# inferenceengine/shadernn

Measured on NVIDIA B200. Metric: frames/sec, higher is better.
Workload: dtype f32 (split-fp16 hi+lo storage for activations and weights, 3 fp16 MMAs per product, fp32 accumulate)

## Files before the change

### include/snnb.h

```cpp
#ifndef SNNB_H_
#define SNNB_H_

#include <stddef.h>
#include <stdint.h>

#ifdef __cplusplus
extern "C" {
#endif

#define SNNB_VERSION 100

typedef struct snnb_context snnb_context;
typedef struct snnb_tensor snnb_tensor;
typedef struct snnb_weights snnb_weights;
typedef struct snnb_model snnb_model;
typedef struct snnb_timer snnb_timer;

enum { SNNB_ACT_NONE = 0, SNNB_ACT_RELU = 1, SNNB_ACT_RELU6 = 2, SNNB_ACT_TANH = 3, SNNB_ACT_SIGMOID = 4, SNNB_ACT_LEAKY_RELU = 5, SNNB_ACT_SILU = 6, SNNB_ACT_SOFTMAX = 7 };
enum { SNNB_PAD_NONE = 0, SNNB_PAD_CONSTANT = 1, SNNB_PAD_REPLICATE = 2, SNNB_PAD_REFLECT = 3 };
enum { SNNB_ALGO_AUTO = 0, SNNB_ALGO_SIMT = 1, SNNB_ALGO_TCGEN05 = 2, SNNB_ALGO_TCGEN05_STREAMK = 3 };
enum { SNNB_PRECISION_FP32X3 = 0, SNNB_PRECISION_FP16W = 1, SNNB_PRECISION_FP16 = 2 };

int snnb_context_create(int device, snnb_context** out);
int snnb_context_destroy(snnb_context* ctx);
// ... 49 lines not shown
int snnb_subpixel_launch(snnb_context* ctx, int r, const snnb_tensor* in, snnb_tensor* out);

int snnb_timer_create(snnb_context* ctx, snnb_timer** out);
int snnb_timer_start(snnb_timer* t);
int snnb_timer_stop(snnb_timer* t);
int snnb_timer_elapsed_ms(snnb_timer* t, float* ms);
int snnb_timer_destroy(snnb_timer* t);

typedef struct snnb_graph snnb_graph;
int snnb_graph_capture_begin(snnb_context* ctx);
int snnb_graph_capture_end(snnb_context* ctx, snnb_graph** out);
int snnb_graph_launch(snnb_graph* g);
int snnb_graph_destroy(snnb_graph* g);

typedef struct {
    int batch;
    int input_width;
    int input_height;
    int conv_algo;
    int use_cuda_graph;
    int fuse;
    int precision;
} snnb_model_options;

int snnb_model_load_json(snnb_context* ctx, const char* json_path, const snnb_model_options* opt, snnb_model** out);
int snnb_model_destroy(snnb_model* m);
int snnb_model_num_layers(const snnb_model* m);
int snnb_model_layer_info(const snnb_model* m, int i, char* name, int name_cap, char* type, int type_cap, int* n, int* h, int* w, int* c);
int snnb_model_num_inputs(const snnb_model* m);
int snnb_model_num_outputs(const snnb_model* m);
int snnb_model_input_dims(const snnb_model* m, int idx, int* n, int* h, int* w, int* c);
int snnb_model_output_dims(const snnb_model* m, int idx, int* n, int* h, int* w, int* c);
int snnb_model_run(snnb_model* m, const float* host_input_nhwc, float* host_output, size_t out_capacity, int* classes_1based);
int snnb_model_submit(snnb_model* m, const float* host_input_nhwc, float* host_output, size_t out_capacity, int* classes_1based, int* ticket);
int snnb_model_submit_u8(snnb_model* m, const uint8_t* host_input_nhwc_u8, const float* mean4, const float* norm4, float* host_output, size_t out_capacity,
                         int* classes_1based, int* ticket);
typedef struct {
    const uint8_t* input_u8;
    int src_height, src_width;
    int linear_filter;
    float mean4[4], norm4[4];
    float* output_f32;
    size_t output_capacity;
    uint8_t* output_u8;
    float out_scale, out_offset;
    int* classes_1based;
} snnb_image_io;
int snnb_model_submit_image(snnb_model* m, const snnb_image_io* io, int* ticket);
int snnb_model_wait(snnb_model* m, int ticket);
int snnb_model_set_input(snnb_model* m, int idx, const float* host_input_nhwc);
int snnb_model_forward(snnb_model* m);
int snnb_model_get_output(snnb_model* m, int idx, float* host_output, size_t out_capacity);
int snnb_model_layer_output(snnb_model* m, int layer, float* host_nhwc, size_t capacity);
int snnb_model_dump_outputs(snnb_model* m, const char* dir);
int snnb_model_time_layers(snnb_model* m, float* times_ms, int capacity);
int snnb_model_layer_kernel(const snnb_model* m, int layer, char* name, int name_cap);
int snnb_model_launches_per_forward(const snnb_model* m);
int snnb_model_get_boxes(snnb_model* m, int n, float* rows6, int max_rows, int* count);
int snnb_model_weight_arena(snnb_model* m, void** device_ptr, size_t* bytes);

typedef struct snnb_comm snnb_comm;
int snnb_nccl_unique_id(unsigned char id128[128]);
int snnb_nccl_comm_create(snnb_context* ctx, int rank, int world_size, const unsigned char id128[128], snnb_comm** out);
int snnb_nccl_comm_destroy(snnb_comm* comm);
int snnb_bcast_weights(snnb_model* m, snnb_comm* comm, int root);

typedef struct snnb_layer_json snnb_layer_json;
int snnb_layer_json_number(const snnb_layer_json* layer, const char* key, double* out);
int snnb_layer_json_string(const snnb_layer_json* layer, const char* key, char* buf, int cap);
int snnb_layer_json_numbers(const snnb_layer_json* layer, const char* path, const double** data, size_t* count);
typedef struct {
    void* user;
    int (*output_dims)(void* user, int num_inputs, const int* in_hwc, int* out_hwc);
    int (*run)(void* user, snnb_context* ctx, int num_inputs, const snnb_tensor* const* inputs, snnb_tensor* output);
    void (*destroy)(void* user);
} snnb_layer_impl;
typedef int (*snnb_layer_creator)(void* registry_user, const snnb_layer_json* layer, snnb_layer_impl* out);
int snnb_register_layer(const char* type_name, snnb_layer_creator creator, void* registry_user);
int snnb_unregister_layer(const char* type_name);
int snnb_tensor_planes(const snnb_tensor* t, void** hi, void** lo, int* cp);
int snnb_debug_streamk_schedule(int tiles, int num_kb, int sms, int* rows, int capacity);
int snnb_debug_feed_plan(int k, int stride, int pad_x, int ic, int out[5]);
int snnb_debug_kblock_schedule(int ksize, int cblocks, int icp, int sc_cblocks, int tiles, int ksplit, int sms, int* rows, int capacity);

#ifdef __cplusplus
}
#endif
#endif
```

### shadernn_b200/_lib.py

```python
import ctypes as C
import os

HERE = os.path.dirname(os.path.abspath(__file__))
LIB_PATH = os.path.join(HERE, "libsnn_b200.so")

c_float_p = C.POINTER(C.c_float)
c_int_p = C.POINTER(C.c_int)
vp = C.c_void_p


class ConvDesc(C.Structure):
    _fields_ = [
        ("in_channels", C.c_int),
        ("out_channels", C.c_int),
        ("kernel", C.c_int),
        ("stride", C.c_int),
        ("pad_x", C.c_int),
        ("pad_y", C.c_int),
        ("pad_mode", C.c_int),
        ("activation", C.c_int),
        ("leaky_alpha", C.c_float),
        ("algo", C.c_int),
    ]

# ... 30 lines not shown
SIGNATURES = {
    "snnb_version": (C.c_int, []),
    "snnb_last_error": (C.c_char_p, []),
    "snnb_context_create": (C.c_int, [C.c_int, C.POINTER(vp)]),
    "snnb_context_destroy": (C.c_int, [vp]),
    "snnb_sync": (C.c_int, [vp]),
    "snnb_context_stream": (vp, [vp]),
    "snnb_launch_count": (C.c_uint64, [vp]),
    "snnb_context_set_precision": (C.c_int, [vp, C.c_int]),
    "snnb_tensor_alloc": (C.c_int, [vp, C.c_int, C.c_int, C.c_int, C.c_int, C.POINTER(vp)]),
    "snnb_tensor_free": (C.c_int, [vp]),
    "snnb_tensor_dims": (C.c_int, [vp, c_int_p, c_int_p, c_int_p, c_int_p]),
    "snnb_tensor_upload_nhwc": (C.c_int, [vp, vp, vp]),
    "snnb_tensor_download_nhwc": (C.c_int, [vp, vp, vp]),
    "snnb_tensor_upload_c4hw4": (C.c_int, [vp, vp, vp]),
    "snnb_tensor_download_c4hw4": (C.c_int, [vp, vp, vp]),
    "snnb_tensor_dump": (C.c_int, [vp, vp, C.c_char_p]),
    "snnb_weights_pack_conv2d": (C.c_int, [vp, C.POINTER(ConvDesc), vp, vp, vp, vp, vp, vp, C.POINTER(vp)]),
    "snnb_weights_pack_depthwise": (C.c_int, [vp, C.POINTER(ConvDesc), vp, vp, vp, vp, vp, vp, C.POINTER(vp)]),
    "snnb_weights_pack_dense": (C.c_int, [vp, C.c_int, C.c_int, vp, vp, C.POINTER(vp)]),
    "snnb_weights_pack_channels": (C.c_int, [vp, C.c_int, vp, vp, vp, vp, C.POINTER(vp)]),
    "snnb_weights_free": (C.c_int, [vp]),
    "snnb_conv2d_launch": (C.c_int, [vp, C.POINTER(ConvDesc), vp, vp, vp, vp]),
    "snnb_depthwise_launch": (C.c_int, [vp, C.POINTER(ConvDesc), vp, vp, vp]),
    "snnb_maxpool_launch": (C.c_int, [vp, C.c_int, C.c_int, vp, vp]),
    "snnb_avgpool_launch": (C.c_int, [vp, C.c_int, C.c_int, vp, vp]),
    "snnb_add_launch": (C.c_int, [vp, C.c_int, C.c_float, vp, vp, vp]),
    "snnb_batchnorm_launch": (C.c_int, [vp, vp, C.c_int, C.c_float, vp, vp]),
    "snnb_activation_launch": (C.c_int, [vp, C.c_int, C.c_float, vp, vp]),
    "snnb_dense_launch": (C.c_int, [vp, vp, C.c_int, C.c_float, vp, vp]),
    "snnb_softmax_launch": (C.c_int, [vp, vp, vp]),
    "snnb_argmax1": (C.c_int, [vp, vp, c_int_p]),
    "snnb_flatten_launch": (C.c_int, [vp, vp, vp]),
    "snnb_concat_launch": (C.c_int, [vp, vp, vp, vp]),
    "snnb_upsample_launch": (C.c_int, [vp, C.c_float, C.c_int, vp, vp]),
    "snnb_pad_launch": (C.c_int, [vp, C.c_int, C.c_int, C.c_int, vp, vp]),
    "snnb_instancenorm_launch": (C.c_int, [vp, vp, C.c_int, C.c_float, vp, vp]),
    "snnb_subpixel_launch": (C.c_int, [vp, C.c_int, vp, vp]),
    "snnb_timer_create": (C.c_int, [vp, C.POINTER(vp)]),
    "snnb_timer_start": (C.c_int, [vp]),
    "snnb_timer_stop": (C.c_int, [vp]),
    "snnb_timer_elapsed_ms": (C.c_int, [vp, c_float_p]),
    "snnb_timer_destroy": (C.c_int, [vp]),
    "snnb_model_load_json": (C.c_int, [vp, C.c_char_p, C.POINTER(ModelOptions), C.POINTER(vp)]),
    "snnb_model_destroy": (C.c_int, [vp]),
    "snnb_model_num_layers": (C.c_int, [vp]),
    "snnb_model_layer_info": (C.c_int, [vp, C.c_int, C.c_char_p, C.c_int, C.c_char_p, C.c_int, c_int_p, c_int_p, c_int_p, c_int_p]),
    "snnb_model_num_inputs": (C.c_int, [vp]),
    "snnb_model_num_outputs": (C.c_int, [vp]),
    "snnb_model_input_dims": (C.c_int, [vp, C.c_int, c_int_p, c_int_p, c_int_p, c_int_p]),
    "snnb_model_output_dims": (C.c_int, [vp, C.c_int, c_int_p, c_int_p, c_int_p, c_int_p]),
    "snnb_model_run": (C.c_int, [vp, vp, vp, C.c_size_t, vp]),
    "snnb_graph_capture_begin": (C.c_int, [vp]),
    "snnb_graph_capture_end": (C.c_int, [vp, C.POINTER(C.c_void_p)]),
    "snnb_graph_launch": (C.c_int, [vp]),
    "snnb_graph_destroy": (C.c_int, [vp]),
    "snnb_model_submit": (C.c_int, [vp, vp, vp, C.c_size_t, vp, c_int_p]),
    "snnb_model_submit_u8": (C.c_int, [vp, vp, vp, vp, vp, C.c_size_t, vp, c_int_p]),
    "snnb_model_submit_image": (C.c_int, [vp, C.POINTER(ImageIO), c_int_p]),
    "snnb_model_wait": (C.c_int, [vp, C.c_int]),
    "snnb_model_set_input": (C.c_int, [vp, C.c_int, vp]),
    "snnb_model_forward": (C.c_int, [vp]),
    "snnb_model_get_output": (C.c_int, [vp, C.c_int, vp, C.c_size_t]),
    "snnb_model_layer_output": (C.c_int, [vp, C.c_int, vp, C.c_size_t]),
    "snnb_model_dump_outputs": (C.c_int, [vp, C.c_char_p]),
    "snnb_model_time_layers": (C.c_int, [vp, c_float_p, C.c_int]),
    "snnb_model_launches_per_forward": (C.c_int, [vp]),
    "snnb_model_layer_kernel": (C.c_int, [vp, C.c_int, C.c_char_p, C.c_int]),
    "snnb_model_get_boxes": (C.c_int, [vp, C.c_int, c_float_p, C.c_int, c_int_p]),
    "snnb_model_weight_arena": (C.c_int, [vp, C.POINTER(vp), C.POINTER(C.c_size_t)]),
    "snnb_nccl_unique_id": (C.c_int, [C.c_char_p]),
    "snnb_nccl_comm_create": (C.c_int, [vp, C.c_int, C.c_int, C.c_char_p, C.POINTER(vp)]),
    "snnb_nccl_comm_destroy": (C.c_int, [vp]),
    "snnb_bcast_weights": (C.c_int, [vp, vp, C.c_int]),
    "snnb_register_layer": (C.c_int, [C.c_char_p, vp, vp]),
    "snnb_unregister_layer": (C.c_int, [C.c_char_p]),
    "snnb_layer_json_number": (C.c_int, [vp, C.c_char_p, C.POINTER(C.c_double)]),
    "snnb_layer_json_string": (C.c_int, [vp, C.c_char_p, C.c_char_p, C.c_int]),
    "snnb_layer_json_numbers": (C.c_int, [vp, C.c_char_p, C.POINTER(C.POINTER(C.c_double)), C.POINTER(C.c_size_t)]),
    "snnb_tensor_planes": (C.c_int, [vp, C.POINTER(vp), C.POINTER(vp), c_int_p]),
    "snnb_debug_streamk_schedule": (C.c_int, [C.c_int, C.c_int, C.c_int, c_int_p, C.c_int]),
    "snnb_debug_feed_plan": (C.c_int, [C.c_int, C.c_int, C.c_int, C.c_int, c_int_p]),
    "snnb_debug_kblock_schedule": (C.c_int, [C.c_int] * 7 + [c_int_p, C.c_int]),
}

_lib = None


class SnnbError(RuntimeError):
    pass


def lib():
    global _lib
    if _lib is None:
        if not os.path.exists(LIB_PATH):
            raise SnnbError(
                "%s is missing — build it with `python -m shadernn_b200._build` (or __graft_entry__.build()). "
                "shadernn_b200 has no CPU or PyTorch fallback." % LIB_PATH)
        l = C.CDLL(LIB_PATH)
        for name, (res, args) in SIGNATURES.items():
            fn = getattr(l, name)
            fn.restype = res
            fn.argtypes = args
        _lib = l
    return _lib


def check(rc, what=""):
    if rc != 0:
        msg = lib().snnb_last_error()
        raise SnnbError("%s failed (status %d): %s" % (what or "snnb call", rc, msg.decode("utf-8", "replace") if msg else "?"))
```

### shadernn_b200/csrc/capi.cpp

```cpp
#include <cstdarg>
#include <cstdlib>
#include <cstring>
#include <memory>

#include "snnb_internal.h"

namespace snnb {

static thread_local char g_err[1024] = "";
void set_error(const char* fmt, ...) {
    va_list ap;
    va_start(ap, fmt);
    vsnprintf(g_err, sizeof(g_err), fmt, ap);
    va_end(ap);
}
const char* get_error() { return g_err; }

bool pdl_enabled() {
    static const bool on = getenv("SNNB_NO_PDL") == nullptr;
    return on;
}

int ensure_stage(snnb_context* ctx, size_t bytes) {
    if (ctx->stage_dev_bytes < bytes) {
// ... 41 lines not shown
    t->feed_lo = t->lo ? t->feed_hi + plane : nullptr;
    t->feed_h = feed_h, t->feed_w = feed_w, t->feed_py = py, t->feed_px = px;
    return 0;
}

}

using namespace snnb;

#define CHECK_DIMS_EQ(a, b, what) SNNB_REQUIRE((a)->n == (b)->n && (a)->h == (b)->h && (a)->w == (b)->w && (a)->c == (b)->c, what ": tensor dims differ")

extern "C" {

int snnb_version(void) { return SNNB_VERSION; }
int snnb_context_set_precision(snnb_context* ctx, int precision) {
    SNNB_REQUIRE(ctx && (precision == SNNB_PRECISION_FP32X3 || precision == SNNB_PRECISION_FP16W), "snnb_context_set_precision: FP32X3 or FP16W (FP16 storage is a model option)");
    ctx->precision = precision;
    return 0;
}
const char* snnb_last_error(void) { return get_error(); }

int snnb_context_create(int device, snnb_context** out) {
    SNNB_REQUIRE(out, "snnb_context_create: null out");
    int count = 0;
    cudaError_t e = cudaGetDeviceCount(&count);
    if (e != cudaSuccess || count == 0) {
        set_error("snnb_context_create: no CUDA device available (%s). This library has no CPU fallback.", cudaGetErrorString(e));
        return 1;
    }
    SNNB_REQUIRE(device >= 0 && device < count, "snnb_context_create: device %d out of range (%d devices)", device, count);
    SNNB_CUDA_OK(cudaSetDevice(device));
    cudaDeviceProp prop;
    SNNB_CUDA_OK(cudaGetDeviceProperties(&prop, device));
    SNNB_REQUIRE(prop.major == 10, "snnb_context_create: device %d is sm_%d%d; this library is built for sm_100a (B200) only", device, prop.major, prop.minor);
    auto ctx      = std::make_unique<snnb_context>();
    ctx->device   = device;
    ctx->sm_count = prop.multiProcessorCount;
    SNNB_CUDA_OK(cudaStreamCreateWithFlags(&ctx->stream, cudaStreamNonBlocking));
    *out = ctx.release();
    return 0;
}

int snnb_context_destroy(snnb_context* ctx) {
    if (!ctx) return 0;
    cudaSetDevice(ctx->device);
    cudaStreamSynchronize(ctx->stream);
    if (ctx->stage_dev) cudaFree(ctx->stage_dev);
    if (ctx->stage_host) cudaFreeHost(ctx->stage_host);
    for (void* b : ctx->scratch_blocks) cudaFree(b);
    cudaStreamDestroy(ctx->stream);
    delete ctx;
    return 0;
}

int snnb_sync(snnb_context* ctx) {
    SNNB_REQUIRE(ctx, "snnb_sync: null context");
    SNNB_CUDA_OK(cudaStreamSynchronize(ctx->stream));
    return 0;
}
void* snnb_context_stream(snnb_context* ctx) { return ctx ? (void*) ctx->stream : nullptr; }
uint64_t snnb_launch_count(snnb_context* ctx) { return ctx ? ctx->launches : 0; }

int snnb_tensor_alloc(snnb_context* ctx, int n, int h, int w, int c, snnb_tensor** out) { return tensor_alloc(ctx, n, h, w, c, out); }
int snnb_tensor_free(snnb_tensor* t) {
    if (!t) return 0;
    if (t->owns && t->hi) cudaFree(t->hi);
    if (t->feed_hi) cudaFree(t->feed_hi);
    delete t;
    return 0;
}
int snnb_debug_feed_plan(int k, int stride, int pad_x, int ic, int out[5]) {
    FeedPlan fp;
    if (!out || !make_feed_plan(k, stride, pad_x, ic, fp)) return 0;
    out[0] = fp.px, out[1] = fp.d, out[2] = fp.nch, out[3] = fp.ksteps, out[4] = fp.rows_per_panel;
    return 1;
}
int snnb_debug_streamk_schedule(int tiles, int num_kb, int sms, int* rows, int capacity) {
    SNNB_REQUIRE(rows || capacity == 0, "snnb_debug_streamk_schedule: null buffer");
    return streamk_schedule(tiles, num_kb, sms, rows, capacity);
}
int snnb_debug_kblock_schedule(int ksize, int cblocks, int icp, int sc_cblocks, int tiles, int ksplit, int sms, int* rows, int capacity) {
    SNNB_REQUIRE(rows || capacity == 0, "snnb_debug_kblock_schedule: null buffer");
    return kblock_schedule(ksize, cblocks, icp, sc_cblocks, tiles, ksplit, sms, rows, capacity);
}
int snnb_tensor_planes(const snnb_tensor* t, void** hi, void** lo, int* cp) {
    SNNB_REQUIRE(t && hi && lo && cp, "snnb_tensor_planes: null argument");
    *hi = t->hi, *lo = t->lo, *cp = t->cp;
    return 0;
}
int snnb_tensor_dims(const snnb_tensor* t, int* n, int* h, int* w, int* c) {
    SNNB_REQUIRE(t, "snnb_tensor_dims: null tensor");
    if (n) *n = t->n;
    if (h) *h = t->h;
    if (w) *w = t->w;
    if (c) *c = t->c;
    return 0;
}
int snnb_tensor_upload_nhwc(snnb_context* ctx, snnb_tensor* t, const float* host) {
    SNNB_REQUIRE(ctx && t && host, "snnb_tensor_upload_nhwc: null argument");
    const size_t bytes = t->pixels() * t->c * sizeof(float);
    if (ensure_stage(ctx, bytes)) return 1;
    SNNB_CUDA_OK(cudaMemcpyAsync(ctx->stage_dev, host, bytes, cudaMemcpyHostToDevice, ctx->stream));
    if (launch_split_f32(ctx, ctx->stage_dev, t)) return 1;
    SNNB_CUDA_OK(cudaStreamSynchronize(ctx->stream));
    return 0;
}
int snnb_tensor_download_nhwc(snnb_context* ctx, const snnb_tensor* t, float* host) {
    SNNB_REQUIRE(ctx && t && host, "snnb_tensor_download_nhwc: null argument");
    const size_t bytes = t->pixels() * t->c * sizeof(float);
    if (ensure_stage(ctx, bytes)) return 1;
    if (launch_merge_f32(ctx, t, ctx->stage_dev)) return 1;
    SNNB_CUDA_OK(cudaMemcpyAsync(host, ctx->stage_dev, bytes, cudaMemcpyDeviceToHost, ctx->stream));
    SNNB_CUDA_OK(cudaStreamSynchronize(ctx->stream));
    return 0;
}

static void c4_to_nhwc(const float* c4, int N, int H, int W, int C, float* nhwc) {
    const int D = (C + 3) / 4;
    for (int n = 0; n < N; ++n)
        for (int y = 0; y < H; ++y)
            for (int x = 0; x < W; ++x)
                for (int c = 0; c < C; ++c)
                    nhwc[(((size_t) n * H + y) * W + x) * C + c] = c4[((((size_t) n * D + c / 4) * H + y) * W + x) * 4 + (c % 4)];
}
static void nhwc_to_c4(const float* nhwc, int N, int H, int W, int C, float* c4) {
    const int D = (C + 3) / 4;
    memset(c4, 0, sizeof(float) * (size_t) N * D * H * W * 4);
    for (int n = 0; n < N; ++n)
        for (int y = 0; y < H; ++y)
            for (int x = 0; x < W; ++x)
                for (int c = 0; c < C; ++c)
                    c4[((((size_t) n * D + c / 4) * H + y) * W + x) * 4 + (c % 4)] = nhwc[(((size_t) n * H + y) * W + x) * C + c];
}
int snnb_tensor_upload_c4hw4(snnb_context* ctx, snnb_tensor* t, const float* host_c4) {
    SNNB_REQUIRE(ctx && t && host_c4, "snnb_tensor_upload_c4hw4: null argument");
    std::vector<float> tmp(t->pixels() * t->c);
    c4_to_nhwc(host_c4, t->n, t->h, t->w, t->c, tmp.data());
    return snnb_tensor_upload_nhwc(ctx, t, tmp.data());
}
int snnb_tensor_download_c4hw4(snnb_context* ctx, const snnb_tensor* t, float* host_c4) {
    SNNB_REQUIRE(ctx && t && host_c4, "snnb_tensor_download_c4hw4: null argument");
    std::vector<float> tmp(t->pixels() * t->c);
    if (snnb_tensor_download_nhwc(ctx, t, tmp.data())) return 1;
    nhwc_to_c4(tmp.data(), t->n, t->h, t->w, t->c, host_c4);
    return 0;
}
int snnb_tensor_dump(snnb_context* ctx, const snnb_tensor* t, const char* path) {
    SNNB_REQUIRE(ctx && t && path, "snnb_tensor_dump: null argument");
    const int D = (t->c + 3) / 4;
    std::vector<float> c4((size_t) t->n * D * t->h * t->w * 4);
    if (snnb_tensor_download_c4hw4(ctx, t, c4.data())) return 1;
    for (int n = 0; n < t->n; ++n) {
        std::string p = path;
        if (t->n > 1) p += ".n" + std::to_string(n);
        FILE* f = fopen(p.c_str(), "wb");
        SNNB_REQUIRE(f, "snnb_tensor_dump: cannot open %s", p.c_str());
        char header[32];
        memset(header, 0, sizeof(header));
        snprintf(header, sizeof(header), "%d %d %d %d", t->w, t->h, D, t->c);
        fwrite(header, 1, sizeof(header), f);
        fwrite(c4.data() + (size_t) n * D * t->h * t->w * 4, sizeof(float), (size_t) D * t->h * t->w * 4, f);
        fclose(f);
    }
    return 0;
}

// ... 244 lines not shown
```

### shadernn_b200/csrc/engine/core.cpp

```cpp
#include <algorithm>
#include <cstring>
#include <unordered_map>
#include <unordered_set>

#include "engine.h"

using namespace snnb;

namespace snn {

using namespace dp;

MixedInferenceCore::~MixedInferenceCore() {
    if (ctx) {
        cudaSetDevice(ctx->device);
        cudaStreamSynchronize(ctx->stream);
    }
    if (cuGraphExec) cudaGraphExecDestroy(cuGraphExec);
    if (cuGraph) cudaGraphDestroy(cuGraph);
    for (auto* t : ownedTensors) snnb_tensor_free(t);
    if (arena) cudaFree(arena);
    if (scratchArena) cudaFree(scratchArena);
    if (ioStage) cudaFree(ioStage);
    if (argmaxDev) cudaFree(argmaxDev);
    if (yoloDev) cudaFree(yoloDev);
    if (yoloHost) cudaFreeHost(yoloHost);
    for (auto& sl : slots) {
        if (sl.yoloDev) cudaFree(sl.yoloDev);
        if (sl.yoloHost) cudaFreeHost(sl.yoloHost);
        if (sl.stageIn) cudaFree(sl.stageIn);
        if (sl.stageResize) cudaFree(sl.stageResize);
        if (sl.stageOut) cudaFree(sl.stageOut);
        if (sl.smallHost) cudaFreeHost(sl.smallHost);
        if (sl.argmax) cudaFree(sl.argmax);
        if (sl.h2dDone) cudaEventDestroy(sl.h2dDone);
        if (sl.stageFree) cudaEventDestroy(sl.stageFree);
        if (sl.resultReady) cudaEventDestroy(sl.resultReady);
    }
    if (copyStream) cudaStreamDestroy(copyStream);
}

std::unique_ptr<MixedInferenceCore> MixedInferenceCore::create(snnb_context* ctx, const std::string& modelFileName, const ShaderGenOptions& options,
                                                               std::string& err) {
    std::unique_ptr<MixedInferenceCore> core(new MixedInferenceCore());
    core->ctx     = ctx;
    core->options = options;
    try {
        core->layers = loadFromJsonModel(modelFileName);
        core->graph  = generateInferenceGraph(core->layers, options);
    } catch (std::exception& e) {
        err = e.what();
        return nullptr;
    }
    if (!core->init(err)) return nullptr;
    return core;
}

static bool allZeroPadding(const PaddingSpec& p) {
    uint32_t o[4];
    p.offsets(3, true, o);
    const bool keyword_same = !(p.t == "valid" || p.t == "none" || (!p.t.empty() && std::all_of(p.t.begin(), p.t.end(), ::isdigit)));
    return !keyword_same && o[0] == 0 && o[1] == 0 && o[2] == 0 && o[3] == 0;
}

bool MixedInferenceCore::init(std::string& err) {
    const int N = (int) options.batch;
    const bool twoPlanes = options.precision != SNNB_PRECISION_FP16;
    std::unordered_map<GenericModelLayer*, int> order;
    for (size_t i = 0; i < graph.sorted.size(); ++i) order[graph.sorted[i]] = (int) i;

    for (auto* L : graph.sorted) {
        if (L->isInputLayer) inputLayers.push_back(L);
        if (L->nextLayers.empty()) outputLayers.push_back(L);
        if (L->typeName == "YOLO") yolo = static_cast<YOLOLayer*>(L);
    }
    std::stable_sort(inputLayers.begin(), inputLayers.end(), [](GenericModelLayer* a, GenericModelLayer* b) {
        return static_cast<InputLayerLayer*>(a)->_desc.inputIndex < static_cast<InputLayerLayer*>(b)->_desc.inputIndex;
    });
    if (inputLayers.empty()) {
        err = "model has no InputLayer";
        return false;
    }

    std::unordered_map<GenericModelLayer*, GenericModelLayer*> alias;
    const bool shortcutFold = options.fuse && options.convAlgo != SNNB_ALGO_SIMT && getenv("SNNB_NO_SHORTCUT_FOLD") == nullptr;
    auto foldable = [&](GenericModelLayer* c2, GenericModelLayer* ds) {
        if (c2 == ds || c2->typeName != "Conv2D" || ds->typeName != "Conv2D" || c2->fusedAway || ds->fusedAway) return false;
        auto* cc = static_cast<Conv2DLayer*>(c2);
        auto* dc = static_cast<Conv2DLayer*>(ds);
        if (c2->nextLayers.size() != 1 || ds->nextLayers.size() != 1 || c2->prevLayers.size() != 1 || ds->prevLayers.size() != 1) return false;
        if (cc->_desc.activation.id != SNNB_ACT_NONE || dc->_desc.activation.id != SNNB_ACT_NONE || cc->residual || cc->fusedAct >= 0 || cc->shortcut ||
            dc->shortcut || dc->foldedInto)
            return false;
        const int dsMode = padModeId(dc->_desc.padding.mode);
        if (cc->_desc.stride != 1 || dc->_desc.kernelSize != 1 || !(dsMode == SNNB_PAD_NONE || dsMode == SNNB_PAD_CONSTANT)) return false;
        GenericModelLayer* x = ds->prevLayers[0];
        if (order[x] >= order[c2]) return false;
        const Dims &dc2 = graph.outputDims[order[c2]], &dds = graph.outputDims[order[ds]];
        if (dc2.width != dds.width || dc2.height != dds.height || dc2.depth != dds.depth || graph.outputDims[order[x]].depth != ds->numInputPlanes) return false;
        auto stand_in = [&](GenericModelLayer* X) {
            snnb_tensor t;
            const Dims& d = graph.outputDims[order[X]];
            t.n = N, t.h = (int) d.height, t.w = (int) d.width, t.c = (int) d.depth, t.cp = round_up(t.c, 8);
            t.hi = reinterpret_cast<__half*>(1), t.lo = twoPlanes ? t.hi : nullptr;
            return t;
        };
        const snnb_tensor in = stand_in(c2->prevLayers[0]), sc = stand_in(x), out = stand_in(c2);
        snnb_weights probe;
        probe.w_hi = probe.w_lo = probe.w_row_hi = probe.w_row_lo = reinterpret_cast<__half*>(1);
        uint32_t offs[4];
        cc->_desc.padding.offsets((int) cc->_desc.kernelSize, true, offs);
        ConvArgs a;
        a.in = &in, a.residual = nullptr, a.out = const_cast<snnb_tensor*>(&out), a.w = &probe;
        a.k = (int) cc->_desc.kernelSize, a.stride = 1;
        a.pad_x = a.k == 1 ? 0 : (int) offs[0], a.pad_y = a.k == 1 ? 0 : (int) offs[2], a.pad_mode = padModeId(cc->_desc.padding.mode);
        probe.row_stride = 1, probe.row_pad = a.pad_x;
        a.act = SNNB_ACT_NONE, a.alpha = 0.0f, a.precision = options.precision;
        a.shortcut = &sc, a.sc_stride = (int) dc->_desc.stride;
        return conv2d_umma_fold_supported(ctx, a);
    };
    if (options.fuse) {
        for (auto* L : graph.sorted) {
            if (L->typeName == "Pad" && L->nextLayers.size() == 1 && L->prevLayers.size() == 1) {
                auto* pad  = static_cast<PadLayer*>(L);
                auto* next = L->nextLayers[0];
                PaddingSpec* np = nullptr;
                if (next->typeName == "Conv2D" && static_cast<Conv2DLayer*>(next)->_desc.kernelSize > 1) np = &static_cast<Conv2DLayer*>(next)->_desc.padding;
                if (next->typeName == "SeparableConv2D" && pad->mode == "constant") np = &static_cast<SeparableConv2DLayer*>(next)->_desc.padding;
                if (np && allZeroPadding(*np)) {
                    uint32_t o[4];
                    pad->padding.offsets(0, false, o);
                    np->t = std::to_string(o[0]), np->b = std::to_string(o[1]), np->l = std::to_string(o[2]), np->r = std::to_string(o[3]);
                    np->mode       = pad->mode;
                    L->fusedAway   = true;
                    alias[L]       = L->prevLayers[0];
                }
            }
            if (shortcutFold && L->typeName == "Add" && L->prevLayers.size() == 2) {
                auto* add = static_cast<AddLayer*>(L);
                for (int o = 0; o < 2; ++o) {
                    GenericModelLayer* c2 = L->prevLayers[o];
                    GenericModelLayer* ds = L->prevLayers[1 - o];
                    if (!foldable(c2, ds)) continue;
                    auto* cc       = static_cast<Conv2DLayer*>(c2);
                    cc->fusedAct   = add->activation.id;
                    cc->fusedAlpha = add->activation.alpha;
                    cc->shortcut   = static_cast<Conv2DLayer*>(ds);
                    cc->shortcut->foldedInto = cc;
                    ds->fusedAway  = true;
                    L->fusedAway   = true;
                    alias[c2]      = L;
                    break;
                }
            }
            if (L->typeName == "Add" && L->prevLayers.size() == 2 && !L->fusedAway) {
                auto* add = static_cast<AddLayer*>(L);
                GenericModelLayer* a = L->prevLayers[0];
                GenericModelLayer* b = L->prevLayers[1];
                auto fusable = [&](GenericModelLayer* c, GenericModelLayer* other) {
                    if (c->typeName != "Conv2D" || c->nextLayers.size() != 1 || c->fusedAway) return false;
                    auto* conv = static_cast<Conv2DLayer*>(c);
                    if (conv->_desc.activation.id != SNNB_ACT_NONE || conv->residual || conv->fusedAct >= 0) return false;
                    return order[other] < order[c] && c != other;
                };
                GenericModelLayer* conv = nullptr;
                GenericModelLayer* other = nullptr;
                if (fusable(b, a))
                    conv = b, other = a;
                else if (fusable(a, b))
                    conv = a, other = b;
                if (conv) {
                    conv->fusedAct   = add->activation.id;
                    conv->fusedAlpha = add->activation.alpha;
                    conv->prevLayers.push_back(other);
                    L->fusedAway     = true;
                    alias[conv]      = L;
                }
            }
            if (L->typeName == "Dense" && L->prevLayers.size() == 1) {
                GenericModelLayer* f = L->prevLayers[0];
                GenericModelLayer* pool = (f->typeName == "Flatten" && f->prevLayers.size() == 1 && f->nextLayers.size() == 1 &&
                                           static_cast<FlattenLayer*>(f)->activation.id == SNNB_ACT_NONE)
                                              ? f->prevLayers[0]
                                              : f;
                auto dimsOf = [&](GenericModelLayer* x) { return graph.outputDims[order[x]]; };
                if (pool->typeName == "AveragePooling2D" && static_cast<PoolingLayer*>(pool)->isAvg && pool->nextLayers.size() == 1 && pool->prevLayers.size() == 1 &&
                    !pool->fusedAway && dimsOf(pool).width * dimsOf(pool).height == 1 && static_cast<DenseLayer*>(L)->units <= 256 &&
                    dimsOf(pool->prevLayers[0]).width * dimsOf(pool->prevLayers[0]).height >= 4 && dimsOf(pool->prevLayers[0]).depth <= 4096 &&
                    static_cast<PoolingLayer*>(pool)->_desc.kernelSize >= dimsOf(pool->prevLayers[0]).width &&
                    static_cast<PoolingLayer*>(pool)->_desc.kernelSize >= dimsOf(pool->prevLayers[0]).height) {
                    static_cast<DenseLayer*>(L)->gapSource = pool->prevLayers[0];
                    pool->fusedAway = true;
                }
            }
            if (L->typeName == "Flatten" && L->inputDims.size() == 1 && L->inputDims[0].width * L->inputDims[0].height == 1 &&
                static_cast<FlattenLayer*>(L)->activation.id == SNNB_ACT_NONE) {
                L->fusedAway = true;
                alias[L]     = L->prevLayers[0];
            }
        }
    }

    std::unordered_map<GenericModelLayer*, snnb_tensor*> outOf;
    auto resolve = [&](GenericModelLayer* L) -> GenericModelLayer* {
        std::unordered_set<GenericModelLayer*> seen;
        while (alias.count(L) && !seen.count(L)) {
            seen.insert(L);
            L = alias[L];
        }
        return L;
    };
    for (size_t i = 0; i < graph.sorted.size(); ++i) {
        GenericModelLayer* L = graph.sorted[i];
        if (L->typeName == "YOLO") continue;
        GenericModelLayer* owner = resolve(L);
        if (owner != L && !(L->typeName == "Conv2D")) continue;
        if (L->typeName == "Conv2D" && static_cast<Conv2DLayer*>(L)->foldedInto) continue;
        if (outOf.count(owner)) continue;
        const Dims& d = graph.outputDims[order[owner]];
        snnb_tensor* t = nullptr;
        if (tensor_alloc(ctx, N, (int) d.height, (int) d.width, (int) d.depth, &t, twoPlanes)) {
            err = get_error();
            return false;
        }
        ownedTensors.push_back(t);
        outOf[owner] = t;
    }
    for (auto* L : graph.sorted) {
        if (L->typeName == "YOLO") {
            for (auto* p : L->prevLayers) L->inputs.push_back(outOf.at(resolve(p)));
            continue;
        }
        GenericModelLayer* owner = resolve(L);
        L->output                = outOf.count(owner) ? outOf[owner] : nullptr;
        if (L->fusedAway) continue;
        size_t nin = L->prevLayers.size();
        if (L->typeName == "Conv2D" && static_cast<Conv2DLayer*>(L)->fusedAct >= 0 && !static_cast<Conv2DLayer*>(L)->shortcut) {
            nin -= 1;
            L->residual = outOf.at(resolve(L->prevLayers.back()));
        }
        for (size_t k = 0; k < nin; ++k) L->inputs.push_back(outOf.at(resolve(L->prevLayers[k])));
        if (L->typeName == "Conv2D") {
            auto* cl  = static_cast<Conv2DLayer*>(L);
            cl->algo = options.convAlgo;
            if (cl->shortcut) cl->shortcutIn = outOf.at(resolve(cl->shortcut->prevLayers[0]));
            int ph = 0, pw = 0;
            snnb_weights probe_w;
            probe_w.w_hi = probe_w.w_lo = reinterpret_cast<__half*>(1);
            probe_w.w_row_hi = probe_w.w_row_lo = reinterpret_cast<__half*>(1);
            probe_w.row_stride = (int) cl->_desc.stride, probe_w.row_pad = 0;
            std::swap(cl->weights, probe_w);
            const bool prepad = cl->wantsPrepad(L->inputs[0], L->output, options.convAlgo, ph, pw);
            std::swap(cl->weights, probe_w);
            if (prepad) {
                if (tensor_alloc(ctx, N, ph, pw, L->inputs[0]->c, &cl->prepadded, twoPlanes)) {
                    err = get_error();
                    return false;
                }
                ownedTensors.push_back(cl->prepadded);
            }
            {
                static const bool noFeed = getenv("SNNB_NO_FEED") != nullptr;
                GenericModelLayer* src   = resolve(L->prevLayers[0]);
                snnb_tensor* in          = L->inputs[0];
                const int mode           = padModeId(cl->_desc.padding.mode);
                uint32_t offs[4];
                cl->_desc.padding.offsets((int) cl->_desc.kernelSize, true, offs);
                const int k = (int) cl->_desc.kernelSize, padX = (int) offs[0], padY = (int) offs[2];
                FeedPlan fp;
                if (!noFeed && !prepad && src->isInputLayer && !in->feed_hi && options.convAlgo != SNNB_ALGO_SIMT && !L->residual && !cl->shortcut && L->output->c <= 64 &&
                    (mode == SNNB_PAD_NONE || mode == SNNB_PAD_CONSTANT) && make_feed_plan(k, (int) cl->_desc.stride, padX, in->c, fp)) {
                    const int tilesX = (L->output->w + 127) / 128;
                    const int needW  = 2 * (tilesX * 128 - 1) + 2 * fp.nch;
                    const int needH  = 2 * (L->output->h - 1) + k - padY + padY;
                    const int feedW  = (std::max(in->w + fp.px, needW) + 1) & ~1;
                    const int feedH  = std::max(in->h + padY, needH);
                    if (tensor_alloc_feed(in, feedH, feedW, padY, fp.px)) {
                        err = get_error();
                        return false;
                    }
                    cl->feedInput = true;
                }
            }
        }
        if (L->typeName == "Dense") {
            auto* dl = static_cast<DenseLayer*>(L);
            if (L->inputs[0]->h * L->inputs[0]->w != 1) {
                if (tensor_alloc(ctx, N, 1, 1, (int) dl->numInputPlanes, &dl->flat, twoPlanes)) {
                    err = get_error();
                    return false;
                }
                ownedTensors.push_back(dl->flat);
            }
            if ((uint32_t) (L->inputs[0]->h * L->inputs[0]->w * L->inputs[0]->c) != dl->numInputPlanes) {
                err = L->name + ": Dense expects " + std::to_string(dl->numInputPlanes) + " inputs, graph provides " +
                      std::to_string(L->inputs[0]->h * L->inputs[0]->w * L->inputs[0]->c);
                return false;
            }
        }
        if ((L->typeName == "Add" || L->typeName == "Concatenate") && L->inputs.size() != 2) {
            err = L->name + ": expects exactly two inputs";
            return false;
        }
        auto dimsStr = [](const snnb_tensor* t) { return std::to_string(t->h) + "x" + std::to_string(t->w) + "x" + std::to_string(t->c); };
        if (L->typeName == "Conv2D" || L->typeName == "SeparableConv2D" || L->typeName == "BatchNormalization" || L->typeName == "InstanceNorm") {
            if (L->inputs.empty() || !L->output) {
                err = L->name + ": layer has no input";
                return false;
            }
            if ((uint32_t) L->inputs[0]->c != L->numInputPlanes) {
                err = L->name + ": inputPlanes " + std::to_string(L->numInputPlanes) + " but the producing layer has " + std::to_string(L->inputs[0]->c) + " channels";
                return false;
            }
            const uint32_t wantOut = (L->typeName == "Conv2D") ? L->numOutputPlanes : L->numInputPlanes;
            if ((uint32_t) L->output->c != wantOut) {
                err = L->name + ": output tensor has " + std::to_string(L->output->c) + " channels, weights are packed for " + std::to_string(wantOut);
                return false;
            }
        }
        if (L->typeName == "Add") {
            for (auto* in : L->inputs)
                if (in->h != L->output->h || in->w != L->output->w || in->c != L->output->c) {
                    err = L->name + ": Add operand " + dimsStr(in) + " does not match the output " + dimsStr(L->output);
                    return false;
                }
        }
        if (L->typeName == "Conv2D" && L->residual &&
            (L->residual->h != L->output->h || L->residual->w != L->output->w || L->residual->c != L->output->c)) {
            err = L->name + ": fused Add operand " + dimsStr(L->residual) + " does not match the output " + dimsStr(L->output);
            return false;
        }
        if (L->typeName == "Concatenate") {
            if (L->inputs[0]->h != L->inputs[1]->h || L->inputs[0]->w != L->inputs[1]->w || L->inputs[0]->c + L->inputs[1]->c != L->output->c ||
                L->inputs[0]->h != L->output->h || L->inputs[0]->w != L->output->w) {
                err = L->name + ": Concatenate operands " + dimsStr(L->inputs[0]) + " and " + dimsStr(L->inputs[1]) + " do not stack into " + dimsStr(L->output);
                return false;
            }
        }
    }

    for (auto* in : inputLayers) {
        snnb_tensor* t = in->output;
        if (!t || !t->feed_hi || getenv("SNNB_NO_FEED_ONLY")) continue;
        bool only = true;
        int readers = 0;
        for (auto* L : graph.sorted) {
            if (L->fusedAway || L->isInputLayer) continue;
            const bool reads = std::find(L->inputs.begin(), L->inputs.end(), t) != L->inputs.end() || L->residual == t ||
                               (L->typeName == "Conv2D" && static_cast<Conv2DLayer*>(L)->shortcutIn == t);
            if (!reads) continue;
            ++readers;
            only = only && L->typeName == "Conv2D" && static_cast<Conv2DLayer*>(L)->feedInput && L->inputs.size() >= 1 && L->inputs[0] == t && L->residual != t &&
                   std::count(L->inputs.begin(), L->inputs.end(), t) == 1;
        }
        for (auto* o : outputLayers) only = only && o->output != t;
        t->feed_only = only && readers > 0;
    }

    std::vector<std::pair<GenericModelLayer*, PackedHost>> packed;
    size_t total = 0, scratchTotal = 0;
    for (auto* L : graph.sorted) {
        PackedHost p;
        try {
            L->packWeights(p);
// ... 239 lines not shown
            sl.stageResizeBytes = inBytes;
        }
        stage = sl.stageResize;
    }
    if (sl.everUsed) SNNB_CUDA_OK(cudaStreamWaitEvent(copyStream, sl.stageFree, 0));
    SNNB_CUDA_OK(cudaMemcpyAsync(stage, hostInput, inBytes, cudaMemcpyHostToDevice, copyStream));
    SNNB_CUDA_OK(cudaEventRecord(sl.h2dDone, copyStream));
    SNNB_CUDA_OK(cudaStreamWaitEvent(ctx->stream, sl.h2dDone, 0));
    if (resize) {
        if (launch_resize_u8(ctx, reinterpret_cast<const uint8_t*>(stage), io->src_height, io->src_width, in, mean, norm, io->linear_filter != 0)) return 1;
    } else if (u8 ? launch_split_u8(ctx, reinterpret_cast<const uint8_t*>(sl.stageIn), in, mean, norm) : launch_split_f32(ctx, sl.stageIn, in)) {
        return 1;
    }
    SNNB_CUDA_OK(cudaEventRecord(sl.stageFree, ctx->stream));
    if (forward()) return 1;
    sl.userOut = nullptr, sl.userClasses = nullptr, sl.userFloats = 0;
    static const bool noSmall = getenv("SNNB_NO_SMALL_RESULT") != nullptr;
    const bool small = !noSmall && isClassifier && !(io && io->output_u8) && (hostOutput || classes1) &&
                       outFloats * sizeof(float) + options.batch * sizeof(int) <= SMALL_RESULT_BYTES;
    if (small) {
        float* vals = static_cast<float*>(sl.smallDev);
        int* cls    = reinterpret_cast<int*>(static_cast<char*>(sl.smallDev) + outFloats * sizeof(float));
        if (launch_result_small(ctx, out, hostOutput ? vals : nullptr, classes1 ? cls : nullptr)) return 1;
        sl.userOut = hostOutput, sl.userClasses = classes1, sl.userFloats = outFloats;
        hostOutput = nullptr, classes1 = nullptr;
    }
    if (hostOutput) {
        if (launch_merge_f32(ctx, out, sl.stageOut)) return 1;
        SNNB_CUDA_OK(cudaMemcpyAsync(hostOutput, sl.stageOut, outFloats * sizeof(float), cudaMemcpyDeviceToHost, ctx->stream));
    }
    if (io && io->output_u8) {
        if (launch_merge_u8(ctx, out, reinterpret_cast<uint8_t*>(sl.stageOut), io->out_scale, io->out_offset)) return 1;
        SNNB_CUDA_OK(cudaMemcpyAsync(io->output_u8, sl.stageOut, outFloats, cudaMemcpyDeviceToHost, ctx->stream));
    }
    sl.classesHost = nullptr;
    if (classes1 && isClassifier) {
        if (launch_argmax(ctx, out, sl.argmax)) return 1;
        SNNB_CUDA_OK(cudaMemcpyAsync(classes1, sl.argmax, sizeof(int) * options.batch, cudaMemcpyDeviceToHost, ctx->stream));
        sl.classesHost = classes1;
    }
    if (yolo && decodeYolo(sl.yoloDev, sl.yoloHost, false)) return 1;
    SNNB_CUDA_OK(cudaEventRecord(sl.resultReady, ctx->stream));
    sl.busy = sl.everUsed = true;
    *ticket = nextTicket++;
    return 0;
}

int MixedInferenceCore::wait(int ticket) {
    SNNB_REQUIRE(ticket >= 0 && ticket < nextTicket && ticket >= nextTicket - 2, "wait: ticket %d is not in flight", ticket);
    Slot& sl = slots[ticket & 1];
    SNNB_REQUIRE(sl.busy, "wait: ticket %d was already waited for", ticket);
    SNNB_CUDA_OK(cudaEventSynchronize(sl.resultReady));
    if (sl.userOut) std::memcpy(sl.userOut, sl.smallHost, sl.userFloats * sizeof(float));
    if (sl.userClasses) {
        const int* cls = reinterpret_cast<const int*>(static_cast<const char*>(sl.smallHost) + sl.userFloats * sizeof(float));
        for (uint32_t i = 0; i < options.batch; ++i) sl.userClasses[i] = cls[i] + 1;
    }
    sl.userOut = nullptr, sl.userClasses = nullptr;
    if (sl.classesHost)
        for (uint32_t i = 0; i < options.batch; ++i) sl.classesHost[i] += 1;
    sl.busy = false;
    if (yolo) {
        const int rc = yolo->finishDecode(sl.yoloHost, sl.yoloDev, boxes);
        SNNB_REQUIRE(rc >= 0, "wait: corrupt detection candidate list");
        return rc;
    }
    return 0;
}

int MixedInferenceCore::layerOutput(int layerId, float* host, size_t capacityFloats) {
    SNNB_REQUIRE(layerId >= 0 && layerId < (int) layers.size() && host, "layerOutput: bad argument");
    GenericModelLayer* L = layers[layerId].get();
    SNNB_REQUIRE(!(L->typeName == "Conv2D" && static_cast<Conv2DLayer*>(L)->foldedInto),
                 "layerOutput: layer %d (%s) was fused into the K loop of the convolution it is added to; load the model with fuse=0 to observe it", layerId,
                 L->name.c_str());
    SNNB_REQUIRE(L->output, "layerOutput: layer %d (%s) has no device tensor", layerId, L->name.c_str());
    SNNB_REQUIRE(!(L->typeName == "Conv2D" && static_cast<Conv2DLayer*>(L)->fusedAct >= 0),
                 "layerOutput: layer %d (%s) was fused into its Add; load the model with fuse=0 to observe it", layerId, L->name.c_str());
    SNNB_REQUIRE(!(L->fusedAway && L->typeName == "AveragePooling2D"),
                 "layerOutput: layer %d (%s) was fused into the classifier head (pool + Dense in one launch); load the model with fuse=0 to observe it", layerId,
                 L->name.c_str());
    const size_t floats = L->output->pixels() * L->output->c;
    SNNB_REQUIRE(capacityFloats >= floats, "layerOutput: buffer too small (%zu < %zu floats)", capacityFloats, floats);
    return snnb_tensor_download_nhwc(ctx, L->output, host);
}

int MixedInferenceCore::timeLayers(std::vector<float>& ms) {
    ms.assign(layers.size(), 0.0f);
    std::vector<cudaEvent_t> ev(graph.sorted.size() + 1);
    for (auto& e : ev) SNNB_CUDA_OK(cudaEventCreate(&e));
    ExecOptions eo;
    eo.convAlgo = options.convAlgo, eo.precision = options.precision;
    SNNB_CUDA_OK(cudaEventRecord(ev[0], ctx->stream));
    layerKernels.assign(layers.size(), std::string());
    for (size_t i = 0; i < graph.sorted.size(); ++i) {
        GenericModelLayer* L = graph.sorted[i];
        if (!(L->fusedAway || L->isInputLayer || L->typeName == "YOLO")) {
            ctx->last_kernel = nullptr;
            if (int rc = L->run(ctx, eo)) return rc;
            layerKernels[L->layerId] = ctx->last_kernel ? ctx->last_kernel : (L->typeName + " kernels");
        }
        SNNB_CUDA_OK(cudaEventRecord(ev[i + 1], ctx->stream));
    }
    SNNB_CUDA_OK(cudaStreamSynchronize(ctx->stream));
    for (size_t i = 0; i < graph.sorted.size(); ++i) {
        float t = 0;
        SNNB_CUDA_OK(cudaEventElapsedTime(&t, ev[i], ev[i + 1]));
        ms[graph.sorted[i]->layerId] = t;
    }
    for (auto& e : ev) cudaEventDestroy(e);
    return 0;
}

int MixedInferenceCore::dumpOutputs(const std::string& dir) {
    for (auto& l : layers) {
        if (!l->output || l->fusedAway) continue;
        SNNB_REQUIRE(!(l->typeName == "Conv2D" && l->fusedAct >= 0), "dumpOutputs: %s was fused into its Add; load the model with fuse=0 to dump every layer", l->name.c_str());
        std::string path = dir + "/" + l->name + " pass[0].dump";
        if (snnb_tensor_dump(ctx, l->output, path.c_str())) return 1;
    }
    return 0;
}

}
```

### shadernn_b200/csrc/engine/engine.h

```cpp
#pragma once

#include <algorithm>
#include <map>
#include <memory>
#include <string>
#include <vector>

#include "../snnb_internal.h"
#include "json.h"

namespace snn {

struct SNNModelOutputBoxes {
    std::vector<std::vector<float>> rows;
};

namespace dp {

class ModelParser {
public:
    explicit ModelParser(const std::string& fileName);
    ~ModelParser();
    int getLayerCount() const;
    std::string getLayerName(int layerId) const;
    int getNumInbound(int layerId) const;
    std::vector<int> getInboundLayerId(int layerId) const;
    int getInputPlanes(int layerId) const;
    int getOutputPlanes(int layerId) const;
    bool isInputRange01() const;
    const json::Value& layer(int layerId) const;
    bool isBinWeight() const { return binFile != nullptr; }
    void readBin(float* dst, size_t count);
    const std::string& fileName() const { return _fileName; }

private:
    std::string _fileName;
    json::ValuePtr _root;
    FILE* binFile = nullptr;
};

int padModeId(const std::string& mode);
struct PaddingSpec {
    std::string t = "valid", b = "valid", l = "valid", r = "valid";
    std::string mode;
    void parse(const json::Value& layerObj, bool readMode);
    void offsets(int kernelSize, bool evenKernelTopLeftMinusOne, uint32_t (&offs)[4]) const;
    bool validLike() const { return t == "0" || t == "valid" || t == "none"; }
};

struct Dims {
    uint32_t width = 0, height = 0, depth = 0;
};

struct ActivationSpec {
    int id      = SNNB_ACT_NONE;
    float alpha = 0.0f;
    static int fromString(const std::string& s);
};

struct ExecOptions;

class GenericModelLayer {
public:
    virtual ~GenericModelLayer() {}
    std::string name;
    std::string typeName;
    int layerId = -1;
    std::vector<GenericModelLayer*> prevLayers, nextLayers;
    std::vector<Dims> inputDims;
    uint32_t numInputPlanes = 0, numOutputPlanes = 0;
    bool isInputLayer = false;

    virtual void getOutputDims(uint32_t& width, uint32_t& height, uint32_t& depth) const;
    struct Transform { float scaleW = 1, scaleH = 1, transW = 0, transH = 0; };
    virtual Transform getOutputScaleDimAdjustment() const { return Transform(); }

    virtual void packWeights(snnb::PackedHost&) {}
    snnb_weights weights;
    std::vector<snnb_tensor*> inputs;
    snnb_tensor* output = nullptr;
    virtual int run(snnb_context* ctx, const ExecOptions& opt) = 0;
    bool fusedAway          = false;
    snnb_tensor* residual   = nullptr;
    int fusedAct            = -1;
    float fusedAlpha        = 0.0f;
    float* scratch          = nullptr;
    size_t scratchBytes() const { return _scratchBytes; }

protected:
    size_t _scratchBytes = 0;
};

class PluginLayer : public GenericModelLayer {
public:
    snnb_layer_impl impl {};
    ~PluginLayer() override {
        if (impl.destroy) impl.destroy(impl.user);
    }
    void getOutputDims(uint32_t& w, uint32_t& h, uint32_t& d) const override;
    int run(snnb_context* ctx, const ExecOptions& opt) override;
};

typedef GenericModelLayer* (*LayerCreator)(ModelParser&, int);
void initLayerRegisty();
void registerLayer(const std::string& layerName, LayerCreator creator);
GenericModelLayer* createLayerInstance(std::string layerName, ModelParser& parser, int i);

struct InputLayerDesc {
    uint32_t inputWidth = 0, inputHeight = 0, inputChannels = 0, inputIndex = 0;
    void parse(ModelParser& parser, int layerId);
};
class InputLayerLayer : public GenericModelLayer {
public:
    InputLayerDesc _desc;
    void getOutputDims(uint32_t& w, uint32_t& h, uint32_t& d) const override;
    int run(snnb_context*, const ExecOptions&) override { return 0; }
};

struct GenericConvDesc {
    uint32_t kernelSize = 1, stride = 1;
    PaddingSpec padding;
    ActivationSpec activation;
    std::string activationName;
    std::vector<float> weights;
    std::vector<float> biases;
    bool useBatchNormalization = false;
    std::map<std::string, std::vector<float>> batchNormalization;
};
struct Conv2DDesc : GenericConvDesc {
    void parse(ModelParser& parser, int layerId);
};
class Conv2DLayer : public GenericModelLayer {
public:
    Conv2DDesc _desc;
    int algo = SNNB_ALGO_AUTO;
    snnb_tensor* prepadded = nullptr;
    bool feedInput = false;
    Conv2DLayer* shortcut    = nullptr;
    Conv2DLayer* foldedInto  = nullptr;
    snnb_tensor* shortcutIn  = nullptr;
    bool wantsPrepad(const snnb_tensor* in, const snnb_tensor* out, int convAlgo, int& ph, int& pw) const;
    Transform getOutputScaleDimAdjustment() const override;
    void getOutputDims(uint32_t& w, uint32_t& h, uint32_t& d) const override;
    void packWeights(snnb::PackedHost& p) override;
    int run(snnb_context* ctx, const ExecOptions& opt) override;
};
struct SeparableConv2DDesc : GenericConvDesc {
    void parse(ModelParser& parser, int layerId);
};
class SeparableConv2DLayer : public GenericModelLayer {
public:
    SeparableConv2DDesc _desc;
    void getOutputDims(uint32_t& w, uint32_t& h, uint32_t& d) const override;
    void packWeights(snnb::PackedHost& p) override;
    int run(snnb_context* ctx, const ExecOptions& opt) override;
};
struct PoolDesc {
    uint32_t kernelSize = 1, stride = 1;
    PaddingSpec padding;
    void parseMax(ModelParser& parser, int layerId);
    void parseAvg(ModelParser& parser, int layerId);
};
class PoolingLayer : public GenericModelLayer {
public:
    PoolDesc _desc;
    bool isAvg = false;
    Transform getOutputScaleDimAdjustment() const override;
    int run(snnb_context* ctx, const ExecOptions& opt) override;
};
class AdaptiveAvgPool2dLayer : public GenericModelLayer {
public:
    uint32_t poolSize = 1;
    void getOutputDims(uint32_t& w, uint32_t& h, uint32_t& d) const override;
    int run(snnb_context* ctx, const ExecOptions& opt) override;
};
class AddLayer : public GenericModelLayer {
public:
    ActivationSpec activation;
    int run(snnb_context* ctx, const ExecOptions& opt) override;
};
class BatchNormalizationLayer : public GenericModelLayer {
public:
    std::map<std::string, std::vector<float>> batchNormalization;
    ActivationSpec activation;
    void packWeights(snnb::PackedHost& p) override;
    int run(snnb_context* ctx, const ExecOptions& opt) override;
};
class InstanceNormLayer : public GenericModelLayer {
public:
    std::vector<float> gamma, beta;
    ActivationSpec activation;
    void packWeights(snnb::PackedHost& p) override;
    int run(snnb_context* ctx, const ExecOptions& opt) override;
    void setScratch() { _scratchBytes = 0; }
    void computeScratch(int n) { _scratchBytes = snnb::instnorm_scratch_floats(n, snnb::round_up((int) numOutputPlanes, 8)) * sizeof(float); }
};
class ActivationLayer : public GenericModelLayer {
public:
    ActivationSpec activation;
    int run(snnb_context* ctx, const ExecOptions& opt) override;
};
class DenseLayer : public GenericModelLayer {
public:
    std::vector<float> kernel;
    std::vector<float> biases;
    ActivationSpec activation;
    uint32_t units = 0;
    void getOutputDims(uint32_t& w, uint32_t& h, uint32_t& d) const override;
    void packWeights(snnb::PackedHost& p) override;
    int run(snnb_context* ctx, const ExecOptions& opt) override;
    snnb_tensor* flat = nullptr;
    GenericModelLayer* gapSource = nullptr;
};
class FlattenLayer : public GenericModelLayer {
public:
    ActivationSpec activation;
    void getOutputDims(uint32_t& w, uint32_t& h, uint32_t& d) const override;
    int run(snnb_context* ctx, const ExecOptions& opt) override;
};
class ConcatenateLayer : public GenericModelLayer {
public:
    void getOutputDims(uint32_t& w, uint32_t& h, uint32_t& d) const override;
    int run(snnb_context* ctx, const ExecOptions& opt) override;
};
class UpSampling2DLayer : public GenericModelLayer {
public:
    float scale = 1.0f;
    std::string interpolationType = "nearest";
    Transform getOutputScaleDimAdjustment() const override { return Transform {scale, scale, 0.0f, 0.0f}; }
    int run(snnb_context* ctx, const ExecOptions& opt) override;
};
class PadLayer : public GenericModelLayer {
public:
    PaddingSpec padding;
    std::string mode = "constant";
    Transform getOutputScaleDimAdjustment() const override;
    int run(snnb_context* ctx, const ExecOptions& opt) override;
};
class SubpixelLayer : public GenericModelLayer {
public:
    uint32_t kernelSize = 2;
    void getOutputDims(uint32_t& w, uint32_t& h, uint32_t& d) const override;
    int run(snnb_context* ctx, const ExecOptions& opt) override;
};
class YOLOLayer : public GenericModelLayer {
public:
    void getOutputDims(uint32_t& w, uint32_t& h, uint32_t& d) const override;
    int run(snnb_context*, const ExecOptions&) override { return 0; }
    int decode(snnb_context* ctx, std::vector<SNNModelOutputBoxes>& perImage);
    static constexpr int YOLO_HEAD_ROWS = 2048;
    int maxCand() const { return inputs.size() < 2 ? 0 : inputs[0]->n * (inputs[0]->h * inputs[0]->w + inputs[1]->h * inputs[1]->w) * 3; }
    size_t candidateBytes() const { return 32 + (size_t) maxCand() * 8 * sizeof(float); }
    size_t headBytes() const { return 32 + (size_t) std::min(maxCand(), YOLO_HEAD_ROWS) * 8 * sizeof(float); }
    int enqueueCandidates(snnb_context* ctx, void* devBuf);
    int finishDecode(const void* hostBuf, const void* devBuf, std::vector<SNNModelOutputBoxes>& perImage) const;
};

struct ShaderGenOptions {
    uint32_t desiredInputWidth = 0, desiredInputHeight = 0;
    uint32_t batch             = 1;
    int convAlgo               = SNNB_ALGO_AUTO;
    bool fuse                  = false;
    bool useCudaGraph          = false;
    int precision              = SNNB_PRECISION_FP32X3;
};
struct ExecOptions {
    int convAlgo  = SNNB_ALGO_AUTO;
    int precision = SNNB_PRECISION_FP32X3;
};

std::vector<std::shared_ptr<GenericModelLayer>> loadFromJsonModel(const std::string& fileName);
struct InferenceGraph {
    std::vector<GenericModelLayer*> sorted;
    std::vector<Dims> outputDims;
};
InferenceGraph generateInferenceGraph(const std::vector<std::shared_ptr<GenericModelLayer>>& layers, const ShaderGenOptions& options);

}

class MixedInferenceCore {
public:
    ~MixedInferenceCore();
    static std::unique_ptr<MixedInferenceCore> create(snnb_context* ctx, const std::string& modelFileName, const dp::ShaderGenOptions& options,
                                                      std::string& err);
    int forward();
    int setInput(int idx, const float* hostNHWC);
    int getOutput(int idx, float* host, size_t capacityFloats);
    int run(const float* hostInput, float* hostOutput, size_t capacityFloats, int* classes1);
    int submit(const float* hostInput, float* hostOutput, size_t capacityFloats, int* classes1, int* ticket);
    int submitU8(const uint8_t* hostInput, const float mean[4], const float norm[4], float* hostOutput, size_t capacityFloats, int* classes1, int* ticket);
    int submitImpl(const void* hostInput, bool u8, const float* mean, const float* norm, float* hostOutput, size_t capacityFloats, int* classes1, int* ticket,
                   const snnb_image_io* io = nullptr);
    int submitImage(const snnb_image_io& io, int* ticket);
    int wait(int ticket);
    int layerOutput(int layerId, float* host, size_t capacityFloats);
    int timeLayers(std::vector<float>& ms);
    int dumpOutputs(const std::string& dir);

    snnb_context* ctx = nullptr;
    dp::ShaderGenOptions options;
    std::vector<std::shared_ptr<dp::GenericModelLayer>> layers;
    dp::InferenceGraph graph;
    std::vector<dp::GenericModelLayer*> inputLayers, outputLayers;
    std::vector<SNNModelOutputBoxes> boxes;
    void* arena       = nullptr;
    size_t arenaBytes = 0;
    int launchesPerForward = 0;
    bool isClassifier = false;
    std::vector<std::string> layerKernels;

private:
    bool init(std::string& err);
    int enqueueForward(bool countOnly);
    std::vector<snnb_tensor*> ownedTensors;
    void* scratchArena = nullptr;
    cudaGraph_t cuGraph         = nullptr;
    cudaGraphExec_t cuGraphExec = nullptr;
    float* ioStage   = nullptr;
    size_t ioStageBytes = 0;
    int* argmaxDev   = nullptr;
    dp::YOLOLayer* yolo = nullptr;
    void* yoloDev  = nullptr;
    void* yoloHost = nullptr;
    int decodeYolo(void* dev, void* host, bool sync);
    static constexpr size_t SMALL_RESULT_BYTES = 64 * 1024;
    struct Slot {
        void* stageResize = nullptr;
        size_t stageResizeBytes = 0;
        float* stageIn = nullptr;
        float* stageOut = nullptr;
        int* argmax = nullptr;
        cudaEvent_t h2dDone = nullptr, stageFree = nullptr, resultReady = nullptr;
        int* classesHost = nullptr;
        void* smallHost = nullptr;
        void* smallDev  = nullptr;
        float* userOut = nullptr;
        int* userClasses = nullptr;
        size_t userFloats = 0;
        void* yoloDev = nullptr;
        void* yoloHost = nullptr;
        bool busy = false, everUsed = false;
    } slots[2];
    cudaStream_t copyStream = nullptr;
    int nextTicket = 0;
    int ensureStreaming();
};

}
```

### shadernn_b200/csrc/engine/layers.cpp

```cpp
#include <algorithm>
#include <cmath>

#include <cstring>
#include <thread>

#include "engine.h"

using namespace snnb;

namespace snn {
namespace dp {

void GenericModelLayer::getOutputDims(uint32_t& width, uint32_t& height, uint32_t& depth) const {
    width = height = depth = 0U;
    float accSW = 0, accSH = 0, accTW = 0, accTH = 0;
    const Transform t = getOutputScaleDimAdjustment();
    for (auto& dim : inputDims) {
        accSW  = std::max(accSW, t.scaleW * dim.width);
        accTW  = std::max(accTW, t.transW);
        accSH  = std::max(accSH, t.scaleH * dim.height);
        accTH  = std::max(accTH, t.transH);
        width  = (uint32_t) (accSW + accTW);
        height = (uint32_t) (accSH + accTH);
        depth  = std::max(depth, dim.depth);
    }
}

void InputLayerLayer::getOutputDims(uint32_t& w, uint32_t& h, uint32_t& d) const {
    w = inputDims.empty() ? _desc.inputWidth : inputDims[0].width;
    h = inputDims.empty() ? _desc.inputHeight : inputDims[0].height;
    d = _desc.inputChannels;
}

GenericModelLayer::Transform Conv2DLayer::getOutputScaleDimAdjustment() const {
    uint32_t offset[4];
    _desc.padding.offsets((int) _desc.kernelSize, true, offset);
    float scale       = 1 / static_cast<float>(_desc.stride);
    float translation = 0.0f;
    if (_desc.kernelSize % 2 != 0) {
        translation = 1 + (static_cast<float>(offset[0] + offset[1]) - static_cast<float>(_desc.kernelSize)) / static_cast<float>(_desc.stride);
    } else {
        translation = 1 + (static_cast<float>(offset[0] + offset[1] - 1) - static_cast<float>(_desc.kernelSize)) / static_cast<float>(_desc.stride);
    }
    return Transform {scale, scale, translation, translation};
}
void Conv2DLayer::getOutputDims(uint32_t& w, uint32_t& h, uint32_t& d) const {
    GenericModelLayer::getOutputDims(w, h, d);
    d = numOutputPlanes;
}
int padModeId(const std::string& m) {
    if (m == "constant") return SNNB_PAD_CONSTANT;
    if (m == "replicate") return SNNB_PAD_REPLICATE;
    if (m == "reflect") return SNNB_PAD_REFLECT;
    return SNNB_PAD_NONE;
}
static const float* bnv(const std::map<std::string, std::vector<float>>& bn, const char* key) {
    auto it = bn.find(key);
    return (it == bn.end() || it->second.empty()) ? nullptr : it->second.data();
}
void Conv2DLayer::packWeights(PackedHost& p) {
    if (foldedInto) return;
    const auto& bn = _desc.batchNormalization;
    const bool use = _desc.useBatchNormalization;
    pack_conv2d_host((int) numInputPlanes, (int) numOutputPlanes, (int) _desc.kernelSize, _desc.weights.data(), _desc.biases.empty() ? nullptr : _desc.biases.data(),
                     use ? bnv(bn, "gamma") : nullptr, use ? bnv(bn, "beta") : nullptr, use ? bnv(bn, "movingMean") : nullptr,
                     use ? bnv(bn, "movingVariance") : nullptr, p);
    {
        uint32_t offs[4];
        _desc.padding.offsets((int) _desc.kernelSize, true, offs);
        const int mode = padModeId(_desc.padding.mode);
        if (mode == SNNB_PAD_NONE || mode == SNNB_PAD_CONSTANT) {
            pack_rowwin_host(p, (int) _desc.stride, _desc.kernelSize == 1 ? 0 : (int) offs[0]);
            if (feedInput) pack_feed_host(p, (int) _desc.stride, _desc.kernelSize == 1 ? 0 : (int) offs[0]);
        } else {
            pack_rowwin_host(p, (int) _desc.stride, 0);
        }
    }
    if (shortcut) {
        const auto& sd = shortcut->_desc;
        const bool sbn = sd.useBatchNormalization;
        pack_shortcut_host((int) shortcut->numInputPlanes, sd.weights.data(), sd.biases.empty() ? nullptr : sd.biases.data(),
                           sbn ? bnv(sd.batchNormalization, "gamma") : nullptr, sbn ? bnv(sd.batchNormalization, "beta") : nullptr,
                           sbn ? bnv(sd.batchNormalization, "movingMean") : nullptr, sbn ? bnv(sd.batchNormalization, "movingVariance") : nullptr, p);
        std::vector<float>().swap(shortcut->_desc.weights);
    }
    std::vector<float>().swap(_desc.weights);
}
bool Conv2DLayer::wantsPrepad(const snnb_tensor* in, const snnb_tensor* out, int convAlgo, int& ph, int& pw) const {
    const int mode = padModeId(_desc.padding.mode);
    if (!(mode == SNNB_PAD_REPLICATE || mode == SNNB_PAD_REFLECT) || _desc.kernelSize <= 1 || convAlgo == SNNB_ALGO_SIMT) return false;
    ConvArgs probe {in, nullptr, const_cast<snnb_tensor*>(out), &weights, (int) _desc.kernelSize, (int) _desc.stride, 0, 0, SNNB_PAD_CONSTANT, 0, 0.0f};
    if (!conv2d_umma_supported(probe)) return false;
    ph = (out->h - 1) * (int) _desc.stride + (int) _desc.kernelSize;
    pw = (out->w - 1) * (int) _desc.stride + (int) _desc.kernelSize;
    return true;
}

int Conv2DLayer::run(snnb_context* ctx, const ExecOptions& opt) {
    uint32_t offs[4];
    _desc.padding.offsets((int) _desc.kernelSize, true, offs);
    if (prepadded) {
        if (launch_pad(ctx, inputs[0], prepadded, (int) offs[0], (int) offs[2], padModeId(_desc.padding.mode))) return 1;
        ConvArgs a {prepadded, residual, output, &weights, (int) _desc.kernelSize, (int) _desc.stride, 0, 0, SNNB_PAD_CONSTANT,
                    fusedAct >= 0 ? fusedAct : _desc.activation.id, fusedAct >= 0 ? fusedAlpha : _desc.activation.alpha};
        a.precision = opt.precision;
        return launch_conv2d_umma(ctx, a);
    }
    ConvArgs a;
    a.in = inputs[0], a.residual = residual, a.out = output, a.w = &weights;
    a.k = (int) _desc.kernelSize, a.stride = (int) _desc.stride;
    a.pad_x = _desc.kernelSize == 1 ? 0 : (int) offs[0];
    a.pad_y = _desc.kernelSize == 1 ? 0 : (int) offs[2];
    a.pad_mode = padModeId(_desc.padding.mode);
    a.act      = fusedAct >= 0 ? fusedAct : _desc.activation.id;
    a.alpha    = fusedAct >= 0 ? fusedAlpha : _desc.activation.alpha;
    a.precision = opt.precision;
    a.shortcut = shortcutIn, a.sc_stride = shortcut ? (int) shortcut->_desc.stride : 1;
    const int want = algo != SNNB_ALGO_AUTO ? algo : opt.convAlgo;
    if (want != SNNB_ALGO_SIMT && conv2d_umma_supported(a)) return launch_conv2d_umma(ctx, a);
    if (shortcut) {
        set_error("%s: a folded projection shortcut runs on the tensor-core kernel only; load the model with fuse=0 for another algorithm", name.c_str());
        return 2;
    }
    if (want == SNNB_ALGO_TCGEN05) {
        set_error("%s: tcgen05 path requested but unsupported for this shape", name.c_str());
        return 2;
    }
    return launch_conv2d_simt(ctx, a);
}

void SeparableConv2DLayer::getOutputDims(uint32_t& width, uint32_t& height, uint32_t& depth) const {
    uint32_t po[4];
    _desc.padding.offsets((int) _desc.kernelSize, true, po);
    width = height = depth = 0;
    for (auto& dim : inputDims) {
        width  = (dim.width - _desc.kernelSize + po[0] + po[2]) / _desc.stride + 1;
        height = (dim.height - _desc.kernelSize + po[1] + po[3]) / _desc.stride + 1;
        depth  = dim.depth;
        break;
    }
}
void SeparableConv2DLayer::packWeights(PackedHost& p) {
    const auto& bn = _desc.batchNormalization;
    const bool use = _desc.useBatchNormalization;
    pack_depthwise_host((int) numInputPlanes, (int) _desc.kernelSize, _desc.weights.data(), _desc.biases.empty() ? nullptr : _desc.biases.data(),
                        use ? bnv(bn, "gamma") : nullptr, use ? bnv(bn, "beta") : nullptr, use ? bnv(bn, "movingMean") : nullptr,
                        use ? bnv(bn, "movingVariance") : nullptr, p);
}
int SeparableConv2DLayer::run(snnb_context* ctx, const ExecOptions&) {
    uint32_t offs[4];
    _desc.padding.offsets((int) _desc.kernelSize, true, offs);
    ConvArgs a;
    a.in = inputs[0], a.residual = nullptr, a.out = output, a.w = &weights;
    a.k = (int) _desc.kernelSize, a.stride = (int) _desc.stride;
    a.pad_x = (int) offs[0], a.pad_y = (int) offs[2];
    a.pad_mode = SNNB_PAD_CONSTANT, a.act = _desc.activation.id, a.alpha = _desc.activation.alpha;
    return launch_depthwise(ctx, a);
}

GenericModelLayer::Transform PoolingLayer::getOutputScaleDimAdjustment() const {
    float scale = 1.0f / _desc.stride, translation;
    if (_desc.padding.validLike())
        translation = 1.0f - (static_cast<float>(_desc.kernelSize) / static_cast<float>(_desc.stride));
    else
        translation = 1.0f - 1.0f / static_cast<float>(_desc.stride);
    return Transform {scale, scale, translation, translation};
}
int PoolingLayer::run(snnb_context* ctx, const ExecOptions&) { return launch_pool(ctx, inputs[0], output, (int) _desc.kernelSize, (int) _desc.stride, isAvg); }

void AdaptiveAvgPool2dLayer::getOutputDims(uint32_t& w, uint32_t& h, uint32_t& d) const {
    w = h = poolSize;
    d     = inputDims.empty() ? numOutputPlanes : inputDims[0].depth;
}
int AdaptiveAvgPool2dLayer::run(snnb_context* ctx, const ExecOptions&) {
    const snnb_tensor* in = inputs[0];
    if (in->h % (int) poolSize || in->w % (int) poolSize || in->h / (int) poolSize != in->w / (int) poolSize) {
        set_error("%s: AdaptiveAvgPool2d needs H and W divisible by pool (%d x %d -> %u)", name.c_str(), in->h, in->w, poolSize);
        return 2;
    }
    const int k = in->h / (int) poolSize;
    return launch_pool(ctx, in, output, k, k, true);
}

int AddLayer::run(snnb_context* ctx, const ExecOptions&) { return launch_add(ctx, inputs[0], inputs[1], output, activation.id, activation.alpha); }
void BatchNormalizationLayer::packWeights(PackedHost& p) {
    pack_channels_host((int) numOutputPlanes, bnv(batchNormalization, "gamma"), bnv(batchNormalization, "beta"), bnv(batchNormalization, "movingMean"),
                       bnv(batchNormalization, "movingVariance"), p);
}
int BatchNormalizationLayer::run(snnb_context* ctx, const ExecOptions&) { return launch_batchnorm(ctx, inputs[0], output, &weights, activation.id, activation.alpha); }
void InstanceNormLayer::packWeights(PackedHost& p) { pack_channels_host((int) numOutputPlanes, gamma.data(), beta.data(), nullptr, nullptr, p); }
int InstanceNormLayer::run(snnb_context* ctx, const ExecOptions&) {
    return launch_instancenorm(ctx, inputs[0], output, &weights, activation.id, activation.alpha, scratch);
}
int ActivationLayer::run(snnb_context* ctx, const ExecOptions&) { return launch_activation(ctx, inputs[0], output, activation.id, activation.alpha); }

void DenseLayer::getOutputDims(uint32_t& w, uint32_t& h, uint32_t& d) const {
    w = h = 1;
    d     = units;
}
void DenseLayer::packWeights(PackedHost& p) {
    pack_conv2d_host((int) numInputPlanes, (int) units, 1, kernel.data(), biases.empty() ? nullptr : biases.data(), nullptr, nullptr, nullptr, nullptr, p);
    p.kind = 3;
    std::vector<float>().swap(kernel);
}
// ... 229 lines not shown
```

### shadernn_b200/csrc/kernels_umma.cu

```cuda
#include <cuda.h>

#include <algorithm>
#include <vector>
#include <cstdlib>

#include "snnb_internal.h"

namespace snnb {

constexpr int UM_BLOCK_M     = 128;
constexpr int UM_BLOCK_K     = 64;
constexpr int UM_MAX_N       = 128;
constexpr int UM_MAX_N2      = 256;
constexpr int UM_STAGES      = 3;
constexpr int UM_A_BYTES     = UM_BLOCK_M * 128;
constexpr int UM_B_BYTES     = UM_MAX_N * 128;
constexpr int UM_STAGE_BYTES = 2 * UM_A_BYTES + 2 * UM_B_BYTES;
constexpr int UM_EPI_WARPS   = 8;
constexpr int UM_THREADS     = 64 + 32 * UM_EPI_WARPS;
constexpr int UM_ACC_COLS    = 2 * UM_MAX_N;
constexpr int UM_TMEM_COLS   = 2 * UM_ACC_COLS;
constexpr int UM_STG_BYTES   = 2 * UM_BLOCK_M * 128;
constexpr int UM_SCHED_SLOTS = 8;
constexpr int UM_SMEM_BYTES  = UM_STAGES * UM_STAGE_BYTES + UM_STG_BYTES + 1024  + 320 ;
// ... 97 lines not shown
    asm volatile("cp.async.bulk.tensor.4d.shared::cluster.global.mbarrier::complete_tx::bytes [%0], [%1, {%3, %4, %5, %6}], [%2];" ::"r"(dst), "l"(m),
                 "r"(bar), "r"(c0), "r"(c1), "r"(c2), "r"(c3)
                 : "memory");
}
__device__ __forceinline__ void tma_load_2d(uint32_t dst, const CUtensorMap* m, uint32_t bar, int c0, int c1) {
    asm volatile("cp.async.bulk.tensor.2d.shared::cluster.global.mbarrier::complete_tx::bytes [%0], [%1, {%3, %4}], [%2];" ::"r"(dst), "l"(m), "r"(bar),
                 "r"(c0), "r"(c1)
                 : "memory");
}

__device__ __forceinline__ void tmem_alloc(uint32_t slot_smem, uint32_t cols) {
    asm volatile("tcgen05.alloc.cta_group::1.sync.aligned.shared::cta.b32 [%0], %1;" ::"r"(slot_smem), "r"(cols) : "memory");
    asm volatile("tcgen05.relinquish_alloc_permit.cta_group::1.sync.aligned;" ::: "memory");
}
__device__ __forceinline__ void tmem_dealloc(uint32_t taddr, uint32_t cols) {
    asm volatile("tcgen05.dealloc.cta_group::1.sync.aligned.b32 %0, %1;" ::"r"(taddr), "r"(cols) : "memory");
}
__device__ __forceinline__ void umma_f16(uint32_t d_tmem, uint64_t a_desc, uint64_t b_desc, uint32_t idesc, uint32_t accumulate) {
    asm volatile(
        "{\n\t.reg .pred p;\n\t"
        "setp.ne.b32 p, %4, 0;\n\t"
        "tcgen05.mma.cta_group::1.kind::f16 [%0], %1, %2, %3, p;\n\t}" ::"r"(d_tmem),
        "l"(a_desc), "l"(b_desc), "r"(idesc), "r"(accumulate)
        : "memory");
}
__device__ __forceinline__ void umma_commit(uint32_t bar) {
    asm volatile("tcgen05.commit.cta_group::1.mbarrier::arrive::one.shared::cluster.b64 [%0];" ::"r"(bar) : "memory");
}
__device__ __forceinline__ void tmem_ld16(uint32_t taddr, uint32_t (&r)[16]) {
    asm volatile("tcgen05.ld.sync.aligned.32x32b.x16.b32 {%0, %1, %2, %3, %4, %5, %6, %7, %8, %9, %10, %11, %12, %13, %14, %15}, [%16];"
                 : "=r"(r[0]), "=r"(r[1]), "=r"(r[2]), "=r"(r[3]), "=r"(r[4]), "=r"(r[5]), "=r"(r[6]), "=r"(r[7]), "=r"(r[8]), "=r"(r[9]), "=r"(r[10]),
                   "=r"(r[11]), "=r"(r[12]), "=r"(r[13]), "=r"(r[14]), "=r"(r[15])
                 : "r"(taddr)
                 : "memory");
}
__device__ __forceinline__ void tmem_ld_wait() { asm volatile("tcgen05.wait::ld.sync.aligned;" ::: "memory"); }

__device__ __forceinline__ void tma_store_4d(const CUtensorMap* m, uint32_t src, int c0, int c1, int c2, int c3) {
    asm volatile("cp.async.bulk.tensor.4d.global.shared::cta.bulk_group [%0, {%2, %3, %4, %5}], [%1];" ::"l"(m), "r"(src), "r"(c0), "r"(c1), "r"(c2), "r"(c3)
                 : "memory");
}
__device__ __forceinline__ void bulk_load_1d(uint32_t dst, const void* src, uint32_t bytes, uint32_t bar) {
    asm volatile("cp.async.bulk.shared::cluster.global.mbarrier::complete_tx::bytes [%0], [%1], %2, [%3];" ::"r"(dst), "l"(src), "r"(bytes), "r"(bar) : "memory");
}
__device__ __forceinline__ void bulk_commit() { asm volatile("cp.async.bulk.commit_group;" ::: "memory"); }
__device__ __forceinline__ void bulk_wait_read0() { asm volatile("cp.async.bulk.wait_group.read 0;" ::: "memory"); }
__device__ __forceinline__ void bulk_wait_read1() { asm volatile("cp.async.bulk.wait_group.read 1;" ::: "memory"); }
__device__ __forceinline__ void fence_async_smem() { asm volatile("fence.proxy.async.shared::cta;" ::: "memory"); }
__device__ __forceinline__ void named_bar_sync(int id, int threads) { asm volatile("bar.sync %0, %1;" ::"r"(id), "r"(threads) : "memory"); }

__device__ __forceinline__ uint64_t make_smem_desc(uint32_t saddr) {
    return (uint64_t) ((saddr >> 4) & 0x3FFFu) | (1ull << 16) | (64ull << 32) | (1ull << 46) | (2ull << 61);
}
__device__ __forceinline__ uint64_t make_smem_desc_sbo(uint32_t saddr, uint32_t sbo_bytes) {
    return (uint64_t) ((saddr >> 4) & 0x3FFFu) | (1ull << 16) | ((uint64_t) (sbo_bytes >> 4) << 32) | (1ull << 46) | (2ull << 61);
}
__device__ __forceinline__ uint32_t make_idesc(int M, int N) {
    return (1u << 4) | (0u << 7) | (0u << 10) | ((uint32_t) (N >> 3) << 17) | ((uint32_t) (M >> 4) << 24);
}

__device__ __noinline__ float umma_act(float v, int act, float alpha) {
    switch (act) {
    case SNNB_ACT_RELU: return fmaxf(v, 0.0f);
    case SNNB_ACT_RELU6: return fminf(fmaxf(v, 0.0f), 6.0f);
    case SNNB_ACT_TANH: return tanhf(v);
    case SNNB_ACT_SIGMOID: return 1.0f / (1.0f + expf(-v));
    case SNNB_ACT_LEAKY_RELU: return fmaxf(v, v * alpha);
    case SNNB_ACT_SILU: return v * 1.0f / (1.0f + expf(-v));
    default: return v;
    }
}
__device__ __forceinline__ float2 um_h2f(uint32_t u) { return __half22float2(*reinterpret_cast<const __half2*>(&u)); }
__device__ __forceinline__ uint32_t um_f2h(float a, float b) {
    uint32_t h;
    asm("cvt.rn.satfinite.f16x2.f32 %0, %1, %2;" : "=r"(h) : "f"(b), "f"(a));
    return h;
}
__device__ __forceinline__ void um_split2(float a, float b, uint32_t& h, uint32_t& l) {
    h               = um_f2h(a, b);
    const float2 hf = um_h2f(h);
    l               = um_f2h(a - hf.x, b - hf.y);
}

struct EpiArgs {
    const CUtensorMap *o_hi64, *o_lo64, *o_hiT, *o_loT;
    const CUtensorMap *r_hi64, *r_lo64, *r_hiT, *r_loT;
    const float* bias;
    int n_blk, OC, act, has_res, rows_box;
    int has_lo;
    float alpha;
    uint32_t stg;
    uint32_t res_bar;
    uint32_t tmem_empty;
    int bar_id;
    const float* part_src;
    int part_splits;
    long long* trace;
    int trace_seq;
    bool no_store = false;
    bool two_stagings = false;
};

__device__ __forceinline__ void epilogue_residual_load(const EpiArgs& e, int sl, int oc0, int c1, int c2, int c3, bool leader) {
    if (!leader) return;
    const int w          = min(64, e.n_blk - sl * 64);
    const bool sw        = w == 64;
    const uint32_t pitch = sw ? 128u : (uint32_t) w * 2u;
    if (elect_one()) {
        bulk_wait_read0();
        mbar_expect_tx(e.res_bar, (e.has_lo ? 2u : 1u) * (uint32_t) e.rows_box * pitch);
        tma_load_4d(e.stg, sw ? e.r_hi64 : e.r_hiT, e.res_bar, oc0 + sl * 64, c1, c2, c3);
        if (e.has_lo) tma_load_4d(e.stg + UM_BLOCK_M * 128, sw ? e.r_lo64 : e.r_loT, e.res_bar, oc0 + sl * 64, c1, c2, c3);
    }
    __syncwarp();
}

template <int NWARPS, int TERMS>
__device__ __forceinline__ void epilogue_tile(const EpiArgs& e, uint32_t taddr, int oc0, int c1, int c2, int c3, int row, int half, bool leader, int lane,
                                              uint32_t& res_phase) {
    constexpr int MAXC  = NWARPS == 8 ? 2 : 4;
    const bool fast_act = e.act == SNNB_ACT_NONE || e.act == SNNB_ACT_RELU || e.act == SNNB_ACT_RELU6 || e.act == SNNB_ACT_LEAKY_RELU;
    const float slope   = (e.act == SNNB_ACT_RELU || e.act == SNNB_ACT_RELU6) ? 0.0f : (e.act == SNNB_ACT_LEAKY_RELU ? e.alpha : 1.0f);
    const float hi_clip = e.act == SNNB_ACT_RELU6 ? 6.0f : __int_as_float(0x7f800000);
    const int nslabs    = (e.n_blk + 63) >> 6;
#define EPI_STAMP(k)                                                                                      \
    do {                                                                                                  \
        if (e.trace && leader && lane == 0 && blockIdx.x == 0 && tseq < 16) e.trace[4 * 256 + 64 + 8 * tseq + (k)] = clock64(); \
    } while (0)
    for (int sl = 0; sl < nslabs; ++sl) {
        const int tseq     = e.trace_seq * nslabs + sl;
        EPI_STAMP(0);
        const int w        = min(64, e.n_blk - sl * 64);
        const bool sw      = w == 64;
        const uint32_t pitch = sw ? 128u : (uint32_t) w * 2u;
        const uint32_t srow  = e.stg + (uint32_t) row * pitch;
        const uint32_t xr    = sw ? (uint32_t) (row & 7) : 0u;
        const int slab_oc    = oc0 + sl * 64;
        if (e.has_res && sl > 0) epilogue_residual_load(e, sl, oc0, c1, c2, c3, leader);
        bool res_ready = false;
#pragma unroll
        for (int k0 = 0; k0 < MAXC; k0 += 2) {
            uint32_t oh[2][8], ol[2][8];
            uint32_t r[2][16], r2[2][16];
#pragma unroll
            for (int kk = 0; kk < 2; ++kk) {
                const int ci = NWARPS == 8 ? half + 2 * (k0 + kk) : k0 + kk;
                if (ci < (w >> 4)) {
                    const int c = sl * 64 + ci * 16;
                    if (e.part_src) {
                        float4 t[4][4];
#pragma unroll
                        for (int sp = 0; sp < 4; ++sp) {
                            const float4* src = reinterpret_cast<const float4*>(e.part_src + (size_t) sp * UM_BLOCK_M * e.n_blk) + (size_t) (c >> 4) * 4 * UM_BLOCK_M + row;
#pragma unroll
                            for (int j4 = 0; j4 < 4; ++j4)
                                t[sp][j4] = sp < e.part_splits ? __ldcg(src + j4 * UM_BLOCK_M) : make_float4(0.f, 0.f, 0.f, 0.f);
                        }
                        float a16[16];
#pragma unroll
                        for (int j4 = 0; j4 < 4; ++j4) {
                            a16[4 * j4] = t[0][j4].x, a16[4 * j4 + 1] = t[0][j4].y, a16[4 * j4 + 2] = t[0][j4].z, a16[4 * j4 + 3] = t[0][j4].w;
#pragma unroll
                            for (int sp = 1; sp < 4; ++sp)
                                if (sp < e.part_splits) a16[4 * j4] += t[sp][j4].x, a16[4 * j4 + 1] += t[sp][j4].y, a16[4 * j4 + 2] += t[sp][j4].z, a16[4 * j4 + 3] += t[sp][j4].w;
                        }
#pragma unroll
                        for (int j = 0; j < 16; ++j) r[kk][j] = __float_as_uint(a16[j]), r2[kk][j] = 0u;
                    } else {
                        tmem_ld16(taddr + (uint32_t) c, r[kk]);
                        if (TERMS == 3) {
                            tmem_ld16(taddr + (uint32_t) (e.n_blk + c), r2[kk]);
                        } else {
#pragma unroll
                            for (int j = 0; j < 16; ++j) r2[kk][j] = 0u;
                        }
                    }
                }
            }
            if (!e.part_src) tmem_ld_wait();
#pragma unroll
            for (int kk = 0; kk < 2; ++kk) {
                const int k = k0 + kk, ci = NWARPS == 8 ? half + 2 * k : k;
                if (ci < (w >> 4)) {
                    const int c = sl * 64 + ci * 16;
                    float v[16];
#pragma unroll
                    for (int j4 = 0; j4 < 4; ++j4) {
                        const float4 b = __ldg(reinterpret_cast<const float4*>(e.bias + oc0 + c) + j4);
                        v[4 * j4 + 0] = (__uint_as_float(r[kk][4 * j4 + 0]) + __uint_as_float(r2[kk][4 * j4 + 0])) + b.x;
                        v[4 * j4 + 1] = (__uint_as_float(r[kk][4 * j4 + 1]) + __uint_as_float(r2[kk][4 * j4 + 1])) + b.y;
                        v[4 * j4 + 2] = (__uint_as_float(r[kk][4 * j4 + 2]) + __uint_as_float(r2[kk][4 * j4 + 2])) + b.z;
                        v[4 * j4 + 3] = (__uint_as_float(r[kk][4 * j4 + 3]) + __uint_as_float(r2[kk][4 * j4 + 3])) + b.w;
                    }
                    if (e.has_res) {
                        if (!res_ready) {
                            mbar_wait(e.res_bar, res_phase);
                            res_ready = true;
                        }
#pragma unroll
                        for (int g = 0; g < 2; ++g) {
                            const uint32_t a = srow + ((((uint32_t) (ci * 2 + g)) ^ xr) << 4);
                            uint32_t hh[4], ll[4];
                            asm volatile("ld.shared.v4.b32 {%0, %1, %2, %3}, [%4];" : "=r"(hh[0]), "=r"(hh[1]), "=r"(hh[2]), "=r"(hh[3]) : "r"(a));
                            if (e.has_lo) {
                                asm volatile("ld.shared.v4.b32 {%0, %1, %2, %3}, [%4];" : "=r"(ll[0]), "=r"(ll[1]), "=r"(ll[2]), "=r"(ll[3]) : "r"(a + UM_BLOCK_M * 128));
                            } else {
                                ll[0] = ll[1] = ll[2] = ll[3] = 0u;
                            }
#pragma unroll
                            for (int j = 0; j < 4; ++j) {
                                const float2 rh = um_h2f(hh[j]), rl = um_h2f(ll[j]);
                                v[g * 8 + 2 * j] += rh.x + rl.x;
                                v[g * 8 + 2 * j + 1] += rh.y + rl.y;
                            }
                        }
                    }
                    if (e.act == SNNB_ACT_RELU) {
#pragma unroll
                        for (int j = 0; j < 16; ++j) v[j] = fmaxf(v[j], 0.0f);
                    } else if (e.act == SNNB_ACT_NONE) {
                    } else if (e.act == SNNB_ACT_RELU6) {
#pragma unroll
                        for (int j = 0; j < 16; ++j) v[j] = fminf(fmaxf(v[j], 0.0f), 6.0f);
                    } else if (fast_act) {
#pragma unroll
                        for (int j = 0; j < 16; ++j) v[j] = fminf(fmaxf(v[j], v[j] * slope), hi_clip);
                    } else {
#pragma unroll
                        for (int j = 0; j < 16; ++j) v[j] = (oc0 + c + j < e.OC) ? umma_act(v[j], e.act, e.alpha) : 0.0f;
                    }
#pragma unroll
                    for (int j = 0; j < 8; ++j) um_split2(v[2 * j], v[2 * j + 1], oh[kk][j], ol[kk][j]);
                }
            }
            if (k0 + 2 >= MAXC) {
                EPI_STAMP(1);
                if (e.has_res && !res_ready) mbar_wait(e.res_bar, res_phase);
                if (e.has_res) res_phase ^= 1u;
                if (sl == nslabs - 1 && !e.part_src) {
                    tc_fence_before();
                    __syncwarp();
                    if (lane == 0) mbar_arrive(e.tmem_empty);
                }
            }
            if (k0 == 0) {
                if (!e.has_res) {
                    if (leader) {
                        if (elect_one()) {
                            if (e.two_stagings) bulk_wait_read1();
                            else bulk_wait_read0();
                        }
                        __syncwarp();
                    }
                    EPI_STAMP(2);
                    named_bar_sync(e.bar_id, NWARPS * 32);
                }
                EPI_STAMP(3);
            }
#pragma unroll
            for (int kk = 0; kk < 2; ++kk) {
                const int k = k0 + kk, ci = NWARPS == 8 ? half + 2 * k : k;
                if (ci < (w >> 4)) {
#pragma unroll
                    for (int g = 0; g < 2; ++g) {
                        const uint32_t a = srow + ((((uint32_t) (ci * 2 + g)) ^ xr) << 4);
                        asm volatile("st.shared.v4.b32 [%0], {%1, %2, %3, %4};" ::"r"(a), "r"(oh[kk][4 * g]), "r"(oh[kk][4 * g + 1]), "r"(oh[kk][4 * g + 2]), "r"(oh[kk][4 * g + 3])
                                     : "memory");
                        if (e.has_lo)
                            asm volatile("st.shared.v4.b32 [%0], {%1, %2, %3, %4};" ::"r"(a + UM_BLOCK_M * 128), "r"(ol[kk][4 * g]), "r"(ol[kk][4 * g + 1]), "r"(ol[kk][4 * g + 2]),
                                         "r"(ol[kk][4 * g + 3])
                                         : "memory");
                    }
                }
            }
        }
        EPI_STAMP(4);
        fence_async_smem();
        EPI_STAMP(5);
        named_bar_sync(e.bar_id, NWARPS * 32);
        EPI_STAMP(6);
        if (leader) {
            if (!e.no_store && elect_one()) {
                tma_store_4d(sw ? e.o_hi64 : e.o_hiT, e.stg, slab_oc, c1, c2, c3);
                if (e.has_lo) tma_store_4d(sw ? e.o_lo64 : e.o_loT, e.stg + UM_BLOCK_M * 128, slab_oc, c1, c2, c3);
                bulk_commit();
            }
            __syncwarp();
        }
        EPI_STAMP(7);
    }
#undef EPI_STAMP
}
template <int NWARPS, int TERMS>
__device__ __forceinline__ void epilogue_dump_partial(const EpiArgs& e, uint32_t taddr, float* dst, int row, int half, int lane) {
    for (int c = (NWARPS == 8 ? half : 0) * 16; c < e.n_blk; c += (NWARPS == 8 ? 32 : 16)) {
        uint32_t r[16], r2[16];
        tmem_ld16(taddr + (uint32_t) c, r);
        if (TERMS == 3) {
            tmem_ld16(taddr + (uint32_t) (e.n_blk + c), r2);
        } else {
#pragma unroll
            for (int j = 0; j < 16; ++j) r2[j] = 0u;
        }
        tmem_ld_wait();
        float4* d = reinterpret_cast<float4*>(dst) + (size_t) (c >> 4) * 4 * UM_BLOCK_M + row;
#pragma unroll
        for (int j4 = 0; j4 < 4; ++j4)
            d[j4 * UM_BLOCK_M] = make_float4(__uint_as_float(r[4 * j4]) + __uint_as_float(r2[4 * j4]), __uint_as_float(r[4 * j4 + 1]) + __uint_as_float(r2[4 * j4 + 1]),
                                __uint_as_float(r[4 * j4 + 2]) + __uint_as_float(r2[4 * j4 + 2]), __uint_as_float(r[4 * j4 + 3]) + __uint_as_float(r2[4 * j4 + 3]));
    }
    tc_fence_before();
    __syncwarp();
    if (lane == 0) mbar_arrive(e.tmem_empty);
// ... 465 lines not shown
                tc_fence_before();
                __syncwarp();
                if (lane == 0) mbar_arrive(e.tmem_empty);
                continue;
            }
            if (wi.pieces > 1) {
                float* tile_parts = p.partials + (size_t) wi.slot * (SK ? 4 : p.ksplit) * (UM_BLOCK_M * p.n_blk);
                epilogue_dump_partial<UM_EPI_WARPS, EPI_TERMS>(e, taddr, tile_parts + (size_t) wi.piece * (UM_BLOCK_M * p.n_blk), row, half, lane);
                __threadfence();
                named_bar_sync(1, UM_EPI_WARPS * 32);
                if (warp == 2 && lane == 0) {
                    const int old  = atomicAdd(p.counters + wi.slot, 1);
                    const int last = old == wi.pieces - 1;
                    if (last) p.counters[wi.slot] = 0;
                    asm volatile("st.shared.b32 [%0], %1;" ::"r"(last_flag), "r"(last) : "memory");
                }
                named_bar_sync(1, UM_EPI_WARPS * 32);
                int last;
                asm volatile("ld.shared.b32 %0, [%1];" : "=r"(last) : "r"(last_flag) : "memory");
                if (!last) continue;
                __threadfence();
                e.part_src = tile_parts, e.part_splits = wi.pieces;
                if (p.has_res) epilogue_residual_load(e, 0, oc_idx * p.n_blk, bx * p.tw, by * p.th, bn * p.tn, leader);
            }
            if (SPLIT_EPI)
                epilogue_tile<UM_EPI_WARPS / 2, EPI_TERMS>(e, taddr, oc_idx * p.n_blk, bx * p.tw, by * p.th, bn * p.tn, row, 0, leader, lane, res_phase);
            else
                epilogue_tile<UM_EPI_WARPS, EPI_TERMS>(e, taddr, oc_idx * p.n_blk, bx * p.tw, by * p.th, bn * p.tn, row, half, leader, lane, res_phase);
            e.part_src = nullptr;
            if (leader) UM_TRACE(4, it);
        }
        epilogue_drain(leader);
    }

    if (warp == 0) UM_TRACE(5, 2);
    tc_fence_before();
    __syncthreads();
    if (warp == 0) UM_TRACE(5, 3);
    if (p.trace && threadIdx.x == 0) {
        unsigned long long g;
        asm volatile("mov.u64 %0, %%globaltimer;" : "=l"(g));
        atomicMax(reinterpret_cast<unsigned long long*>(p.trace) + 5 * 256 + 9, g);
        if (blockIdx.x == 0) p.trace[5 * 256 + 11] = (long long) g;
    }
    if (warp == 1) {
        tc_fence_after();
        tmem_dealloc(tmem_base, UM_TMEM_COLS);
    }
}

constexpr int RW_MAX_STAGES    = 16;
constexpr int RW_EPI_WARPS     = 8;
constexpr int RW_THREADS       = 64 + 32 * RW_EPI_WARPS;
constexpr int RW_MAX_N         = 64;
constexpr int RW_BOXW          = 144;
constexpr int RW_ARR_BYTES     = RW_BOXW * 16;
constexpr int RW_SMEM_BYTES    = 227 * 1024;
constexpr int RW_BAR_BYTES     = 512;
constexpr int RW_B_MAX_BYTES   = RW_SMEM_BYTES - 1024 - RW_BAR_BYTES - UM_STG_BYTES - 4 * 4 * RW_ARR_BYTES;

struct RowWinParams {
    __half* out_hi;
    __half* out_lo;
    const float* bias;
    int N, OH, OW, OC, OCp, n_blk, ocr;
    int kh, stride, pad_y;
    int tiles_x;
    int parities, dmin[2];
    int ksteps, panels, ks_parity[8], ks_erel[8];
    int act;
    float alpha;
    long long* trace;
    int ablate;
    const __half* feed_hi;
    const __half* feed_lo;
    int feed_h, feed_w, feed_py;
    uint32_t feed_seg_bytes;
    int stages;
    uint32_t stage_bytes, lo_off, b_bytes;
    int rows_per_stage;
    uint32_t row_bytes;
    int stg_bufs;
    int feed_prows;
};

__device__ __forceinline__ uint64_t make_window_desc(uint32_t saddr) { return (uint64_t) ((saddr >> 4) & 0x3FFFu) | (1ull << 16) | (8ull << 32) | (1ull << 46); }

template <int TERMS, int FKS>
__global__ void __launch_bounds__(RW_THREADS, 1)
conv_rowwin_kernel(const __grid_constant__ CUtensorMap tmA_hi0, const __grid_constant__ CUtensorMap tmA_hi1, const __grid_constant__ CUtensorMap tmA_lo0,
                   const __grid_constant__ CUtensorMap tmA_lo1, const __grid_constant__ CUtensorMap tmB_hi, const __grid_constant__ CUtensorMap tmB_lo,
                   const __grid_constant__ CUtensorMap tmO_hi, const __grid_constant__ CUtensorMap tmO_lo, const RowWinParams p) {
    extern __shared__ uint8_t smem_raw[];
    const uint32_t smem_base = (smem_u32(smem_raw) + 1023u) & ~1023u;
    const uint32_t sB = smem_base;
    const uint32_t stg      = smem_base + p.b_bytes;
    const uint32_t sA0      = stg + (uint32_t) p.stg_bufs * UM_STG_BYTES;
    const uint32_t bar_base = sA0 + (uint32_t) p.stages * p.stage_bytes;
    const int RW_STAGES     = p.stages;
    auto full_bar       = [&](int s) { return bar_base + 8u * s; };
    auto empty_bar      = [&](int s) { return bar_base + 8u * (RW_MAX_STAGES + s); };
    auto tmem_full_bar  = [&](int a) { return bar_base + 8u * (2 * RW_MAX_STAGES + a); };
    auto tmem_empty_bar = [&](int a) { return bar_base + 8u * (2 * RW_MAX_STAGES + 2 + a); };
    const uint32_t b_bar     = bar_base + 8u * (2 * RW_MAX_STAGES + 4);
    const uint32_t tmem_slot = bar_base + 8u * (2 * RW_MAX_STAGES + 5);

    const int warp = threadIdx.x >> 5, lane = threadIdx.x & 31;
    pdl_trigger();
    if (warp == 0 && lane == 0) {
        tma_prefetch_desc(&tmA_hi0);
        tma_prefetch_desc(&tmA_lo0);
        tma_prefetch_desc(&tmB_hi);
        tma_prefetch_desc(&tmB_lo);
        for (int s = 0; s < RW_STAGES; ++s) {
            mbar_init(full_bar(s), 1);
            mbar_init(empty_bar(s), 1);
        }
        for (int a = 0; a < 2; ++a) {
            mbar_init(tmem_full_bar(a), 1);
            mbar_init(tmem_empty_bar(a), RW_EPI_WARPS);
        }
        mbar_init(b_bar, 1);
        fence_barrier_init();
    }
    if (warp == 1) tmem_alloc(tmem_slot, 4 * RW_MAX_N);
    tc_fence_before();
    __syncthreads();
    tc_fence_after();
    uint32_t tmem_base;
    asm volatile("ld.shared.b32 %0, [%1];" : "=r"(tmem_base) : "r"(tmem_slot));
    pdl_wait();
    if (warp == 0) UM_TRACE(5, 0);
    if (p.trace && threadIdx.x == 0) {
        unsigned long long g;
        asm volatile("mov.u64 %0, %%globaltimer;" : "=l"(g));
        atomicMin(reinterpret_cast<unsigned long long*>(p.trace) + 5 * 256 + 8, g);
        if (blockIdx.x == 0) p.trace[5 * 256 + 10] = (long long) g;
    }

    const int total_tiles = p.N * p.OH * p.tiles_x;

    if (warp == 0) {
        {
            if (elect_one()) {
                const int vrows = FKS > 0 ? p.feed_prows : p.kh * p.panels;
                mbar_expect_tx(b_bar, (TERMS == 3 ? 2u : 1u) * (uint32_t) vrows * (uint32_t) p.n_blk * 128u);
                for (int v = 0; v < vrows; ++v) {
                    if (TERMS == 3) {
                        tma_load_2d(sB + (2 * v) * p.n_blk * 128, &tmB_hi, b_bar, 0, v * p.ocr);
                        tma_load_2d(sB + (2 * v + 1) * p.n_blk * 128, &tmB_lo, b_bar, 0, v * p.ocr);
                    } else {
                        tma_load_2d(sB + v * p.n_blk * 128, &tmB_hi, b_bar, 0, v * p.ocr);
                    }
                }
            }
            __syncwarp();
            int stage = 0;
            uint32_t phase = 0;
            const uint32_t tx_bytes = (TERMS == 1 ? 1u : 2u) * (p.feed_seg_bytes ? p.feed_seg_bytes : (uint32_t) p.parities * RW_ARR_BYTES);
            if constexpr (FKS > 0) {
                const uint32_t seg  = p.feed_seg_bytes;
                const size_t pitch  = (size_t) p.feed_w * 4;
                const int per_image = p.OH * p.tiles_x;
                int rem = (int) blockIdx.x % per_image, n = (int) blockIdx.x / per_image;
                uint32_t sA = sA0;
                for (int tile = blockIdx.x; tile < total_tiles; tile += gridDim.x) {
                    const int oy = p.tiles_x == 1 ? rem : rem / p.tiles_x, xt = p.tiles_x == 1 ? 0 : rem % p.tiles_x;
                    const size_t off = (((size_t) n * p.feed_h + (oy * 2 - p.pad_y + p.feed_py)) * p.feed_w + 2 * xt * UM_BLOCK_M) * 4;
                    const __half* src_hi = p.feed_hi + off;
                    const __half* src_lo = p.feed_lo + off;
                    for (int ky0 = 0; ky0 < p.kh; ky0 += p.rows_per_stage) {
                        const int rows = min(p.rows_per_stage, p.kh - ky0);
                        mbar_wait(empty_bar(stage), phase ^ 1u);
                        if (elect_one()) {
                            if (p.ablate & 2) {
                                mbar_arrive(full_bar(stage));
                            } else {
                                mbar_expect_tx(full_bar(stage), tx_bytes * (uint32_t) rows);
                                const __half* sh = src_hi;
                                const __half* sl = src_lo;
                                uint32_t dst     = sA;
                                for (int r = 0; r < rows; ++r, dst += p.row_bytes, sh += pitch, sl += pitch) {
                                    bulk_load_1d(dst, sh, seg, full_bar(stage));
                                    if (TERMS >= 2) bulk_load_1d(dst + RW_ARR_BYTES, sl, seg, full_bar(stage));
                                }
                            }
                        }
                        __syncwarp();
                        src_hi += pitch * rows, src_lo += pitch * rows;
                        sA += p.stage_bytes;
                        if (++stage == RW_STAGES) stage = 0, phase ^= 1u, sA = sA0;
                    }
                    rem += (int) gridDim.x;
                    while (rem >= per_image) rem -= per_image, ++n;
                }
            } else
            for (int tile = blockIdx.x; tile < total_tiles; tile += gridDim.x) {
                const int xt = tile % p.tiles_x, oy = (tile / p.tiles_x) % p.OH, n = tile / (p.tiles_x * p.OH);
                const int ox0 = xt * UM_BLOCK_M;
                for (int ky = 0; ky < p.kh; ++ky) {
                    const int iy = oy * p.stride - p.pad_y + ky;
                    mbar_wait(empty_bar(stage), phase ^ 1u);
                    if (elect_one()) {
                        const uint32_t sA = sA0 + stage * p.stage_bytes;
                        if (p.ablate & 2) {
                            mbar_arrive(full_bar(stage));
                        } else {
                            mbar_expect_tx(full_bar(stage), tx_bytes);
                            tma_load_4d(sA, &tmA_hi0, full_bar(stage), 0, ox0 + p.dmin[0], iy, n);
                            if (TERMS >= 2) tma_load_4d(sA + p.lo_off, &tmA_lo0, full_bar(stage), 0, ox0 + p.dmin[0], iy, n);
                            if (p.parities == 2) {
                                tma_load_4d(sA + RW_ARR_BYTES, &tmA_hi1, full_bar(stage), 0, ox0 + p.dmin[1], iy, n);
                                if (TERMS >= 2) tma_load_4d(sA + p.lo_off + RW_ARR_BYTES, &tmA_lo1, full_bar(stage), 0, ox0 + p.dmin[1], iy, n);
                            }
                        }
                    }
                    __syncwarp();
                    if (++stage == RW_STAGES) stage = 0, phase ^= 1u;
                }
            }
        }
    } else if (warp == 1) {
        mbar_wait(b_bar, 0);
        const uint32_t idesc_cat = TERMS == 3 ? make_idesc(UM_BLOCK_M, 2 * p.n_blk) : make_idesc(UM_BLOCK_M, p.n_blk);
        const uint32_t idesc     = make_idesc(UM_BLOCK_M, p.n_blk);
        if (elect_one()) {
            uint32_t koff[8];
#pragma unroll
            for (int q = 0; q < 8; ++q) koff[q] = q < p.ksteps ? (((uint32_t) p.ks_parity[q] * RW_ARR_BYTES + (uint32_t) p.ks_erel[q] * 16u) >> 4) : 0u;
            const uint64_t wdesc0 = make_window_desc(sA0), bdesc0 = make_smem_desc(sB);
            const uint32_t b_panel = (uint32_t) ((TERMS == 3 ? 2 : 1) * p.n_blk * 128) >> 4;
            const uint32_t b_ky    = b_panel * (uint32_t) p.panels;
            const int last_q      = p.ksteps - 1;
            const uint32_t koff_last = ((uint32_t) p.ks_parity[last_q] * RW_ARR_BYTES + (uint32_t) p.ks_erel[last_q] * 16u) >> 4;
            int stage = 0, it = 0, tr = 0;
            uint32_t phase = 0;
            bool ready     = false;
            const bool no_mma = (p.ablate & 4) != 0;
            const uint64_t lo_off16 = (uint64_t) (p.lo_off >> 4);
            if constexpr (FKS > 0) {
                constexpr uint32_t LO16 = RW_ARR_BYTES >> 4;
                constexpr int RPP       = FKS == 1 ? 4 : (FKS == 2 ? 2 : 1);
                const uint32_t stage16  = p.stage_bytes >> 4, row16 = p.row_bytes >> 4;
                const bool tracing      = p.trace != nullptr && blockIdx.x == 0;
                uint64_t a_cur = wdesc0;
                for (int tile = blockIdx.x; tile < total_tiles; tile += gridDim.x, ++it) {
                    const int acc = it & 1;
                    mbar_wait(tmem_empty_bar(acc), ((uint32_t) (it >> 1) & 1u) ^ 1u);
                    tc_fence_after();
                    const uint32_t d_tmem = tmem_base + (uint32_t) (acc * 2 * RW_MAX_N);
                    uint64_t b_cat = bdesc0;
                    int b_sub      = 0;
                    for (int ky0 = 0; ky0 < p.kh; ky0 += p.rows_per_stage) {
                        const int rows = min(p.rows_per_stage, p.kh - ky0);
                        if (!ready) mbar_wait(full_bar(stage), phase);
                        tc_fence_after();
                        if (tracing && tr < 256) p.trace[1 * 256 + tr] = clock64();
                        if (!no_mma) {
                            umma_f16(d_tmem, a_cur, b_cat, idesc_cat, ky0 > 0 ? 1u : 0u);
                            if (TERMS >= 2) umma_f16(d_tmem, a_cur + LO16, b_cat, idesc, 1u);
                        }
                        const int cur        = stage;
                        const bool wrap      = stage == RW_STAGES - 1;
                        uint64_t a_row       = a_cur;
                        phase ^= wrap ? 1u : 0u;
                        stage = wrap ? 0 : stage + 1;
                        a_cur = wrap ? wdesc0 : a_cur + stage16;
                        ready = mbar_test_wait(full_bar(stage), phase);
                        for (int r = 0; r < rows; ++r, a_row += row16) {
                            const uint64_t b_now = b_cat;
                            if (++b_sub == RPP) b_sub = 0, b_cat += b_panel - (RPP - 1) * (8 / RPP);
                            else b_cat += 8 / RPP;
                            if (no_mma) continue;
#pragma unroll
                            for (int q = 0; q < FKS; ++q) {
                                if (r == 0 && q == 0) continue;
                                umma_f16(d_tmem, a_row + 2u * q, b_now + 2u * q, idesc_cat, 1u);
                                if (TERMS >= 2) umma_f16(d_tmem, a_row + LO16 + 2u * q, b_now + 2u * q, idesc, 1u);
                            }
                        }
                        umma_commit(empty_bar(cur));
                        if (ky0 + rows == p.kh) umma_commit(tmem_full_bar(acc));
                        if (tracing && tr < 256) p.trace[2 * 256 + tr] = clock64();
                        ++tr;
                    }
                }
            } else
            for (int tile = blockIdx.x; tile < total_tiles; tile += gridDim.x, ++it) {
                const int acc = it & 1;
                const uint32_t acc_phase = (uint32_t) (it >> 1) & 1u;
                mbar_wait(tmem_empty_bar(acc), acc_phase ^ 1u);
                tc_fence_after();
                const uint32_t d_tmem = tmem_base + (uint32_t) (acc * 2 * RW_MAX_N);
                uint64_t b_cat = bdesc0;
                for (int ky = 0; ky < p.kh; ++ky, b_cat += b_ky) {
                    if (!ready) mbar_wait(full_bar(stage), phase);
                    tc_fence_after();
                    UM_TRACE(1, tr);
                    const uint64_t a0 = wdesc0 + (uint64_t) ((uint32_t) stage * (p.stage_bytes >> 4));
#pragma unroll
                    for (int q = 0; q < 8; ++q) {
                        if (q < last_q && !no_mma) {
                            const uint64_t bq = b_cat + (uint64_t) ((q >> 2) * b_panel + 2u * (q & 3));
                            umma_f16(d_tmem, a0 + koff[q], bq, idesc_cat, (ky > 0 || q > 0) ? 1u : 0u);
                            if (TERMS >= 2) umma_f16(d_tmem, a0 + lo_off16 + koff[q], bq, idesc, 1u);
                        }
                    }
                    const uint64_t b_last = b_cat + (uint64_t) ((last_q >> 2) * b_panel + 2u * (last_q & 3));
                    const int cur = stage;
                    phase ^= (stage == RW_STAGES - 1) ? 1u : 0u;
                    stage = stage == RW_STAGES - 1 ? 0 : stage + 1;
                    ready = mbar_test_wait(full_bar(stage), phase);
                    if (!no_mma) {
                        umma_f16(d_tmem, a0 + koff_last, b_last, idesc_cat, (ky > 0 || last_q > 0) ? 1u : 0u);
                        if (TERMS >= 2) umma_f16(d_tmem, a0 + lo_off16 + koff_last, b_last, idesc, 1u);
                    }
                    umma_commit(empty_bar(cur));
                    if (ky == p.kh - 1) umma_commit(tmem_full_bar(acc));
                    UM_TRACE(2, tr);
                    ++tr;
                }
            }
        }
        __syncwarp();
    } else {
        const int q    = warp & 3;
        const int half = (warp - 2) >> 2;
        const int row  = q * 32 + lane;
        EpiArgs e;
        e.o_hi64 = &tmO_hi, e.o_lo64 = &tmO_lo, e.o_hiT = &tmO_hi, e.o_loT = &tmO_lo;
        e.r_hi64 = e.r_lo64 = e.r_hiT = e.r_loT = &tmO_hi;
        e.bias = p.bias, e.n_blk = p.n_blk, e.OC = p.OC, e.act = p.act, e.has_res = 0, e.rows_box = UM_BLOCK_M, e.alpha = p.alpha;
        e.has_lo = TERMS >= 2;
        e.stg = stg, e.res_bar = 0, e.bar_id = 1;
        e.part_src = nullptr, e.part_splits = 0;
        e.no_store = (p.ablate & 8) != 0;
        e.two_stagings = p.stg_bufs == 2;
        uint32_t res_phase = 0;
        int it = 0;
        for (int tile = blockIdx.x; tile < total_tiles; tile += gridDim.x, ++it) {
            const int acc = it & 1;
            const uint32_t acc_phase = (uint32_t) (it >> 1) & 1u;
            const int xt = tile % p.tiles_x, oy = (tile / p.tiles_x) % p.OH, n = tile / (p.tiles_x * p.OH);
            mbar_wait(tmem_full_bar(acc), acc_phase);
            tc_fence_after();
            if (warp == 2) UM_TRACE(3, it);
            e.tmem_empty = tmem_empty_bar(acc);
            e.trace = p.trace, e.trace_seq = it;
            const uint32_t taddr = tmem_base + ((uint32_t) (q * 32) << 16) + (uint32_t) (acc * 2 * RW_MAX_N);
            if (p.ablate & 1) {
                tc_fence_before();
                __syncwarp();
                if (lane == 0) mbar_arrive(e.tmem_empty);
                continue;
            }
            e.stg = stg + (uint32_t) ((it & 1) & (p.stg_bufs - 1)) * UM_STG_BYTES;
            epilogue_tile<RW_EPI_WARPS, TERMS>(e, taddr, 0, xt * UM_BLOCK_M, oy, n, row, half, warp == 2, lane, res_phase);
            if (warp == 2) UM_TRACE(4, it);
        }
        epilogue_drain(warp == 2);
    }

    tc_fence_before();
    __syncthreads();
    if (warp == 0) UM_TRACE(5, 3);
    if (p.trace && threadIdx.x == 0) {
        unsigned long long g;
        asm volatile("mov.u64 %0, %%globaltimer;" : "=l"(g));
        atomicMax(reinterpret_cast<unsigned long long*>(p.trace) + 5 * 256 + 9, g);
        if (blockIdx.x == 0) p.trace[5 * 256 + 11] = (long long) g;
    }
    if (warp == 1) {
        tc_fence_after();
        tmem_dealloc(tmem_base, 4 * RW_MAX_N);
    }
}

static bool trace_enabled() {
    static const bool on = getenv("SNNB_UMMA_TRACE") != nullptr;
    return on;
}
static int trace_begin(snnb_context* ctx, long long** out) {
    static long long* d_trace = nullptr;
    if (!d_trace) SNNB_CUDA_OK(cudaMalloc(&d_trace, 6 * 256 * sizeof(long long)));
    SNNB_CUDA_OK(cudaMemsetAsync(d_trace, 0, 6 * 256 * sizeof(long long), ctx->stream));
    const long long big = 0x7fffffffffffffffLL;
    SNNB_CUDA_OK(cudaMemcpyAsync(d_trace + 5 * 256 + 8, &big, sizeof(big), cudaMemcpyHostToDevice, ctx->stream));
    SNNB_CUDA_OK(cudaStreamSynchronize(ctx->stream));
    *out = d_trace;
    return 0;
}
static int trace_end(snnb_context* ctx, const long long* d_trace, const char* header) {
    std::vector<long long> h(6 * 256);
    SNNB_CUDA_OK(cudaStreamSynchronize(ctx->stream));
    SNNB_CUDA_OK(cudaMemcpy(h.data(), d_trace, h.size() * sizeof(long long), cudaMemcpyDeviceToHost));
    const long long t0 = h[5 * 256];
    fprintf(stderr, "TRACE %s\n", header);
    fprintf(stderr, "  wallclock_ns   all-CTA span %lld | CTA0 entry +%lld exit +%lld\n", h[5 * 256 + 9] - h[5 * 256 + 8], h[5 * 256 + 10] - h[5 * 256 + 8],
            h[5 * 256 + 11] - h[5 * 256 + 8]);
    fprintf(stderr, "  epi_phases (start, +phase1, +wait_read, +barA, +STS, +fence, +barB, +store) per slab:");
    for (int sq = 0; sq < 16 && h[4 * 256 + 64 + 8 * sq]; ++sq) {
        fprintf(stderr, " [");
        for (int k = 1; k < 8; ++k) fprintf(stderr, "%lld ", h[4 * 256 + 64 + 8 * sq + k] ? h[4 * 256 + 64 + 8 * sq + k] - h[4 * 256 + 64 + 8 * sq] : -1);
        fprintf(stderr, "]");
    }
    fprintf(stderr, "\n");
    h[4 * 256 + 64] = 0;
    h[5 * 256 + 4]  = 0;
    const char* names[6] = {"prod_got_empty", "mma_got_full", "mma_issued", "epi_got_full", "epi_done", "entry_setup_proddone_alldone"};
    for (int r = 0; r < 6; ++r) {
        fprintf(stderr, "  %-14s", names[r]);
        for (int i = 0; i < 256 && (h[r * 256 + i] || (r == 5 && i == 0)); ++i) fprintf(stderr, " %lld", h[r * 256 + i] - t0);
        fprintf(stderr, "\n");
    }
    return 0;
}

typedef CUresult (*EncodeTiledFn)(CUtensorMap*, CUtensorMapDataType, cuuint32_t, void*, const cuuint64_t*, const cuuint64_t*, const cuuint32_t*,
                                  const cuuint32_t*, CUtensorMapInterleave, CUtensorMapSwizzle, CUtensorMapL2promotion, CUtensorMapFloatOOBfill);

static EncodeTiledFn get_encode(snnb_context* ctx) {
    if (!ctx->tmap_encode_fn) {
        void* fn = nullptr;
        cudaDriverEntryPointQueryResult qres;
        if (cudaGetDriverEntryPoint("cuTensorMapEncodeTiled", &fn, cudaEnableDefault, &qres) != cudaSuccess || qres != cudaDriverEntryPointSuccess) return nullptr;
        ctx->tmap_encode_fn = fn;
    }
    return reinterpret_cast<EncodeTiledFn>(ctx->tmap_encode_fn);
}

static int encode_nhwc_box_maps(EncodeTiledFn encode, const snnb_tensor* t, int width, int tw, int th, int tn, bool swizzle128, CUtensorMap (&maps)[2]) {
    const cuuint64_t dims[4]    = {(cuuint64_t) t->cp, (cuuint64_t) t->w, (cuuint64_t) t->h, (cuuint64_t) t->n};
    const cuuint64_t strides[3] = {(cuuint64_t) t->cp * 2, (cuuint64_t) t->w * t->cp * 2, (cuuint64_t) t->h * t->w * t->cp * 2};
    const cuuint32_t box[4]     = {(cuuint32_t) width, (cuuint32_t) tw, (cuuint32_t) th, (cuuint32_t) tn};
    const cuuint32_t estr[4]    = {1, 1, 1, 1};
    __half* planes[2]    = {t->hi, t->lo ? t->lo : t->hi};
    for (int i = 0; i < 2; ++i) {
        CUresult r = encode(&maps[i], CU_TENSOR_MAP_DATA_TYPE_FLOAT16, 4, planes[i], dims, strides, box, estr, CU_TENSOR_MAP_INTERLEAVE_NONE,
                            swizzle128 ? CU_TENSOR_MAP_SWIZZLE_128B : CU_TENSOR_MAP_SWIZZLE_NONE, CU_TENSOR_MAP_L2_PROMOTION_L2_128B,
                            CU_TENSOR_MAP_FLOAT_OOB_FILL_NONE);
        SNNB_REQUIRE(r == CUDA_SUCCESS, "cuTensorMapEncodeTiled(out/residual) failed: %d (cp %d w %d h %d n %d box %d %d %d %d)", (int) r, t->cp, t->w, t->h, t->n,
                     width, tw, th, tn);
    }
// ... 18 lines not shown
            if (eff > best.eff + 1e-9 || (eff > best.eff - 1e-9 && tw > best.tw)) {
                best.tw = tw, best.th = th, best.tn = tn, best.tiles_x = tx, best.tiles_y = ty, best.tiles_n = tnn, best.eff = eff;
            }
        }
    }
    return best;
}

static bool streamk_split(long long tiles, int num_kb, int sms, int& dp, long long& units, int& ctas) {
    dp    = (int) (tiles / sms) * sms;
    units = (tiles - dp) * num_kb;
    const int umin = (num_kb + 2) / 3;
    if (units < umin) return false;
    ctas = (int) std::min<long long>(sms, units / umin);
    return true;
}

struct OcPlan {
    int n_blk = 0, tiles_oc = 0, ksplit = 1, kb_per_split = 0;
    double cost = 1e300;
    int sk = 0, sk_dp = 0, sk_ctas = 0;
    long long sk_units = 0;
};
static double mma_clk(int n) { return std::max(48.0, n * 0.5); }
static OcPlan plan_oc_ksplit(int OC, int m_tiles, int rows_used, int tile_w, int num_kb, int sm_count, int terms, bool halo = false, bool stream_k = false) {
    OcPlan best;
    double best_cost = 1e300;
    static const int no_split = getenv("SNNB_NO_SPLITK") != nullptr;
    const int max_n = terms == 3 ? UM_MAX_N : UM_MAX_N2;
    const int t_min = (OC + max_n - 1) / max_n, t_max = (OC + 15) / 16;
    for (int t = t_min; t <= t_max; ++t) {
        const int blk = std::min(max_n, round_up((OC + t - 1) / t, 16));
        if (blk * t < OC) continue;
        const double ingest  = tile_w < 8 ? 58.0 : 72.0;
        const double a_bytes = (terms == 1 ? 1.0 : 2.0) * rows_used * 128.0, b_bytes = (terms == 3 ? 2.0 : 1.0) * blk * 128;
        const double mma     = terms == 3 ? 4.0 * (mma_clk(2 * blk) + mma_clk(blk)) : 4.0 * terms * mma_clk(blk);
        const double kb_cost = halo ? mma + 125.0 : std::max((a_bytes + b_bytes) / (ingest * 1.05), mma + 45.0);
        for (int sp = 1; sp <= ((no_split || halo) ? 1 : 4); ++sp) {
            if (sp > 1 && (num_kb < 8 * sp)) break;
            const int kbps          = (num_kb + sp - 1) / sp;
            if ((sp - 1) * kbps >= num_kb) continue;
            const long long items = (long long) m_tiles * t * sp;
            const long long rounds = (items + sm_count - 1) / sm_count;
            const double cost      = (double) rounds * (kbps * kb_cost + 7000.0 + (sp > 1 ? 9000.0 : 0.0));
            if (cost < best_cost * (sp > 1 ? 0.93 : 1.0) - 1e-9)
                best_cost = cost, best.cost = cost, best.n_blk = blk, best.tiles_oc = t, best.ksplit = sp, best.kb_per_split = kbps, best.sk = 0;
        }
        static const int env_sk = getenv("SNNB_SK") != nullptr;
        const long long tiles = (long long) m_tiles * t;
        if ((stream_k || env_sk) && !no_split && !halo && num_kb >= 6 && tiles % sm_count != 0) {
            int dp = 0, ctas = 0;
            long long units = 0;
            if (streamk_split(tiles, num_kb, sm_count, dp, units, ctas)) {
                const double u    = std::ceil((double) units / ctas);
                const double cost = (double) (dp / sm_count) * (num_kb * kb_cost + 7000.0) + u * kb_cost + 7000.0 + 4000.0;
                if (cost < best_cost * 0.95 - 1e-9)
                    best_cost = cost, best.cost = cost, best.n_blk = blk, best.tiles_oc = t, best.ksplit = 1, best.kb_per_split = num_kb, best.sk = 1, best.sk_dp = dp,
                    best.sk_ctas = ctas, best.sk_units = units;
            }
        }
        if (blk <= 16) break;
    }
    return best;
}

static int ensure_splitk_scratch(snnb_context* ctx, size_t partial_bytes, size_t n_counters) {
    if (partial_bytes > ctx->splitk_bytes) {
        void* pnew = nullptr;
        SNNB_CUDA_OK(cudaMalloc(&pnew, partial_bytes));
        ctx->scratch_blocks.push_back(pnew);
        ctx->splitk_partials = static_cast<float*>(pnew), ctx->splitk_bytes = partial_bytes;
    }
    if (n_counters > ctx->splitk_counter_n) {
        void* pnew = nullptr;
        SNNB_CUDA_OK(cudaMalloc(&pnew, n_counters * sizeof(int)));
        SNNB_CUDA_OK(cudaMemset(pnew, 0, n_counters * sizeof(int)));
        ctx->scratch_blocks.push_back(pnew);
        ctx->splitk_counters = static_cast<int*>(pnew), ctx->splitk_counter_n = n_counters;
    }
    return 0;
}

static int conv_terms(const snnb_context* ctx, const ConvArgs& a) {
    if (!a.in->lo || !a.out->lo) return 1;
    const int prec = a.precision >= 0 ? a.precision : ctx->precision;
    return prec == SNNB_PRECISION_FP16W ? 2 : (prec == SNNB_PRECISION_FP16 ? 1 : 3);
}

static bool feed_usable(const ConvArgs& a, FeedPlan& fp);
static bool rowwin_supported(const ConvArgs& a) {
    RowPlan rp;
    if (!(a.in->cp == 8 && a.w && a.w->w_row_hi && a.w->w_row_lo && a.w->row_stride == a.stride && a.w->row_pad == a.pad_x && a.out->c <= RW_MAX_N &&
          a.residual == nullptr && make_row_plan(a.k, a.stride, a.pad_x, rp) && 128 + rp.span <= RW_BOXW))
        return false;
    FeedPlan fp;
    const int wrows = feed_usable(a, fp) ? (a.k + fp.rows_per_panel - 1) / fp.rows_per_panel : a.k * ((rp.ksteps + 3) / 4);
    return wrows * 2 * round_up(a.out->c, 16) * 128 <= RW_B_MAX_BYTES;
}

bool conv2d_umma_supported(const ConvArgs& a) {
    if (!a.w || !a.w->w_hi || !a.w->w_lo) return false;
    if (!(a.pad_mode == SNNB_PAD_NONE || a.pad_mode == SNNB_PAD_CONSTANT)) return false;
    if (rowwin_supported(a)) return true;
    if (!(a.stride == 1 || a.stride == 2)) return false;
    if (a.in->c < 16) return false;
    if (a.k < 1 || a.k > 11) return false;
    if (a.pad_x > 127 || a.pad_y > 127) return false;
    return true;
}

static bool halo_plan(const snnb_context* ctx, const ConvArgs& a, int cblocks, int terms, double plain_cost, OcPlan& hp) {
    static const bool no_halo = getenv("SNNB_NO_HALO") != nullptr;
    if (no_halo || a.k != 3 || a.stride != 1 || a.pad_x > 1 || a.pad_y > 1) return false;
    const int hx = (a.out->w + HL_TW - 1) / HL_TW, hy = (a.out->h + HL_TH - 1) / HL_TH;
    hp = plan_oc_ksplit(a.out->c, hx * hy * a.out->n, UM_BLOCK_M, HL_TW, 9 * cblocks, ctx->sm_count, terms, true);
    return hp.n_blk > 0 && hp.cost < plain_cost;
}

bool conv2d_umma_fold_supported(const snnb_context* ctx, const ConvArgs& a) {
    if (!a.shortcut || a.residual || !conv2d_umma_supported(a) || rowwin_supported(a)) return false;
    if (!(a.sc_stride == 1 || a.sc_stride == 2) || a.shortcut->n != a.out->n || !a.shortcut->lo != !a.in->lo) return false;
    const TilePlan tp = plan_tiles(a.out->n, a.out->h, a.out->w, a.stride);
    if (tp.tw <= 0) return false;
    const int cblocks = (a.in->c + UM_BLOCK_K - 1) / UM_BLOCK_K, terms = conv_terms(ctx, a);
    const OcPlan op   = plan_oc_ksplit(a.out->c, tp.tiles_x * tp.tiles_y * tp.tiles_n, tp.tw * tp.th * tp.tn, tp.tw, a.k * a.k * cblocks, ctx->sm_count, terms, false,
                                       a.stream_k);
    OcPlan hp;
    return op.n_blk > 0 && !halo_plan(ctx, a, cblocks, terms, op.cost, hp);
}

enum { ATTR_UMMA = 1u, ATTR_ROWWIN = 2u, ATTR_DW1 = 4u, ATTR_DW2 = 8u };

typedef void (*RowWinKernel)(const CUtensorMap, const CUtensorMap, const CUtensorMap, const CUtensorMap, const CUtensorMap, const CUtensorMap, const CUtensorMap,
                             const CUtensorMap, const RowWinParams);
template <int TERMS> static RowWinKernel rowwin_kernel_fks(int fks) {
    switch (fks) {
    case 1: return conv_rowwin_kernel<TERMS, 1>;
    case 2: return conv_rowwin_kernel<TERMS, 2>;
    case 3: return conv_rowwin_kernel<TERMS, 3>;
    case 4: return conv_rowwin_kernel<TERMS, 4>;
    default: return conv_rowwin_kernel<TERMS, 0>;
    }
}
static RowWinKernel rowwin_kernel_of(int terms, int fks) { return terms == 3 ? rowwin_kernel_fks<3>(fks) : (terms == 2 ? rowwin_kernel_fks<2>(fks) : rowwin_kernel_fks<1>(fks)); }

static bool feed_usable(const ConvArgs& a, FeedPlan& fp) {
    const snnb_tensor* in = a.in;
    if (!in->feed_hi || !a.w->w_feed_hi || !a.w->w_feed_lo || a.w->feed_pad != a.pad_x) return false;
    if (!make_feed_plan(a.k, a.stride, a.pad_x, in->c, fp) || fp.px != in->feed_px || in->feed_py != a.pad_y) return false;
    const int tiles_x = (a.out->w + UM_BLOCK_M - 1) / UM_BLOCK_M;
    return in->feed_w >= 2 * (tiles_x * UM_BLOCK_M - 1) + 2 * fp.nch && in->feed_h >= 2 * (a.out->h - 1) + a.k &&
           (254 + 2 * fp.nch) * 8 <= RW_ARR_BYTES;
}

static int launch_conv2d_rowwin(snnb_context* ctx, const ConvArgs& a, EncodeTiledFn encode) {
    const snnb_tensor* in = a.in;
    snnb_tensor* out      = a.out;
    RowPlan rp;
    SNNB_REQUIRE(make_row_plan(a.k, a.stride, a.pad_x, rp), "launch_conv2d_rowwin: no row plan");
    FeedPlan fp;
    const bool feed = feed_usable(a, fp);
    SNNB_REQUIRE(feed || !in->feed_only, "launch_conv2d_rowwin: the input tensor only exists as a stem feed, which this launch cannot read");
    if (feed) {
        rp.parities = 1, rp.ksteps = fp.ksteps;
        for (int q = 0; q < fp.ksteps; ++q) rp.ks_parity[q] = 0, rp.ks_erel[q] = 2 * q;
    }
    ctx->last_kernel = feed ? "conv_rowwin_kernel<feed>" : "conv_rowwin_kernel";
    RowWinParams p;
    p.out_hi = out->hi, p.out_lo = out->lo, p.bias = a.w->bias;
    p.N = out->n, p.OH = out->h, p.OW = out->w, p.OC = out->c, p.OCp = out->cp;
    p.n_blk = round_up(out->c, 16), p.ocr = a.w->ocr;
    p.kh = a.k, p.stride = a.stride, p.pad_y = a.pad_y;
    p.tiles_x  = (out->w + UM_BLOCK_M - 1) / UM_BLOCK_M;
    p.parities = rp.parities, p.dmin[0] = rp.dmin[0], p.dmin[1] = rp.dmin[1];
    p.ksteps   = rp.ksteps, p.panels = (rp.ksteps + 3) / 4;
    for (int q = 0; q < 8; ++q) p.ks_parity[q] = q < rp.ksteps ? rp.ks_parity[q] : 0, p.ks_erel[q] = q < rp.ksteps ? rp.ks_erel[q] : 0;
    p.act = a.act, p.alpha = a.alpha;
    static const int rw_ablate = getenv("SNNB_UMMA_ABLATE") ? atoi(getenv("SNNB_UMMA_ABLATE")) : 0;
    p.ablate                   = rw_ablate;
    p.feed_hi = in->feed_hi, p.feed_lo = in->feed_lo, p.feed_h = in->feed_h, p.feed_w = in->feed_w, p.feed_py = in->feed_py;
    p.feed_seg_bytes = feed ? (uint32_t) (254 + 2 * fp.nch) * 8u : 0u;
    const int terms = conv_terms(ctx, a);
    p.lo_off      = (uint32_t) p.parities * RW_ARR_BYTES;
    p.row_bytes   = (terms == 1 ? 1u : 2u) * p.lo_off;
    static const int one_row = getenv("SNNB_FEED_ONE_ROW") != nullptr;
    p.rows_per_stage = (feed && !one_row) ? (a.k + (a.k + 3) / 4 - 1) / ((a.k + 3) / 4) : 1;
    p.stage_bytes    = (uint32_t) p.rows_per_stage * p.row_bytes;
    p.feed_prows  = feed ? (a.k + fp.rows_per_panel - 1) / fp.rows_per_panel : 0;
    p.b_bytes     = (uint32_t) round_up((terms == 3 ? 2 : 1) * (feed ? p.feed_prows : a.k * p.panels) * p.n_blk * 128, 1024);
    static const int one_stg = getenv("SNNB_ROWWIN_ONE_STAGING") != nullptr;
    const int ring_room      = RW_SMEM_BYTES - 1024 - RW_BAR_BYTES - (int) p.b_bytes;
    p.stg_bufs    = (!one_stg && (ring_room - 2 * UM_STG_BYTES) / (int) p.stage_bytes >= 2) ? 2 : 1;
    p.stages      = std::min(RW_MAX_STAGES, (ring_room - p.stg_bufs * UM_STG_BYTES) / (int) p.stage_bytes);
    SNNB_REQUIRE(p.stages >= 2, "launch_conv2d_rowwin: weight panels of %u bytes leave no room for the activation ring", p.b_bytes);

    CUtensorMap tmA[4], tmB[2];
    for (int plane = 0; plane < 2; ++plane)
        for (int par = 0; par < 2; ++par) {
            const int pp = par < rp.parities ? par : 0;
            __half* base = ((plane && in->lo) ? in->lo : in->hi) + (size_t) pp * 8;
            const int wp        = (in->w - pp + a.stride - 1) / a.stride;
            const cuuint64_t dims[4]    = {8, (cuuint64_t) (wp > 0 ? wp : 1), (cuuint64_t) in->h, (cuuint64_t) in->n};
            const cuuint64_t strides[3] = {(cuuint64_t) a.stride * 16, (cuuint64_t) in->w * 16, (cuuint64_t) in->h * in->w * 16};
            const cuuint32_t box[4]     = {8, (cuuint32_t) RW_BOXW, 1, 1};
            const cuuint32_t estr[4]    = {1, 1, 1, 1};
            CUresult r = encode(&tmA[plane * 2 + par], CU_TENSOR_MAP_DATA_TYPE_FLOAT16, 4, base, dims, strides, box, estr, CU_TENSOR_MAP_INTERLEAVE_NONE,
                                CU_TENSOR_MAP_SWIZZLE_NONE, CU_TENSOR_MAP_L2_PROMOTION_L2_128B, CU_TENSOR_MAP_FLOAT_OOB_FILL_NONE);
            SNNB_REQUIRE(r == CUDA_SUCCESS, "cuTensorMapEncodeTiled(A, rowwin) failed: %d", (int) r);
        }
    {
        const cuuint64_t dims[2]    = {64, (cuuint64_t) (feed ? (a.k + fp.rows_per_panel - 1) / fp.rows_per_panel : a.k * p.panels) * a.w->ocr};
        const cuuint64_t strides[1] = {128};
        const cuuint32_t box[2]     = {64, (cuuint32_t) p.n_blk};
        const cuuint32_t estr[2]    = {1, 1};
        void* planes[2] = {(void*) (feed ? a.w->w_feed_hi : a.w->w_row_hi), (void*) (feed ? a.w->w_feed_lo : a.w->w_row_lo)};
        for (int i = 0; i < 2; ++i) {
            CUresult r = encode(&tmB[i], CU_TENSOR_MAP_DATA_TYPE_FLOAT16, 2, planes[i], dims, strides, box, estr,
                                CU_TENSOR_MAP_INTERLEAVE_NONE, CU_TENSOR_MAP_SWIZZLE_128B, CU_TENSOR_MAP_L2_PROMOTION_L2_256B, CU_TENSOR_MAP_FLOAT_OOB_FILL_NONE);
            SNNB_REQUIRE(r == CUDA_SUCCESS, "cuTensorMapEncodeTiled(B, rowwin) failed: %d", (int) r);
        }
    }
    CUtensorMap tmO[2];
    if (encode_nhwc_box_maps(encode, out, p.n_blk, UM_BLOCK_M, 1, 1, p.n_blk == 64, tmO)) return 2;
    if (!(ctx->func_attr_mask & ATTR_ROWWIN)) {
        for (int t = 1; t <= 3; ++t)
            for (int f = 0; f <= 4; ++f) SNNB_CUDA_OK(cudaFuncSetAttribute(rowwin_kernel_of(t, f), cudaFuncAttributeMaxDynamicSharedMemorySize, RW_SMEM_BYTES));
        ctx->func_attr_mask |= ATTR_ROWWIN;
    }
    const int total_tiles = p.N * p.OH * p.tiles_x;
    const int grid        = std::min(total_tiles, ctx->sm_count);
    p.trace = nullptr;
    if (trace_enabled() && trace_begin(ctx, &p.trace)) return 1;
    auto* kern = rowwin_kernel_of(terms, feed ? fp.ksteps : 0);
    const cudaError_t le = launch_k_pdl(kern, dim3(grid), dim3(RW_THREADS), RW_SMEM_BYTES, ctx->stream, tmA[0], tmA[1], tmA[2], tmA[3], tmB[0], tmB[1], tmO[0], tmO[1], p);
    if (p.trace) {
        char hdr[256];
        snprintf(hdr, sizeof hdr, "rowwin%s k%d s%d IC%d OC%d out %dx%dx%d n_blk %d tiles %d grid %d kh %d ksteps %d terms %d", feed ? "<feed>" : "", a.k, a.stride, a.in->c,
                 a.out->c, a.out->n, a.out->h, a.out->w, p.n_blk, total_tiles, grid, p.kh, p.ksteps, terms);
        if (trace_end(ctx, p.trace, hdr)) return 1;
    }
    cudaError_t e = le != cudaSuccess ? le : cudaGetLastError();
    if (e != cudaSuccess) {
        set_error("conv_rowwin_kernel launch failed: %s", cudaGetErrorString(e));
        return 1;
    }
    ctx->launches++;
    return 0;
}

int launch_conv2d_umma(snnb_context* ctx, const ConvArgs& a) {
    EncodeTiledFn encode = get_encode(ctx);
    SNNB_REQUIRE(encode, "launch_conv2d_umma: cuTensorMapEncodeTiled is unavailable in this driver");
    if (rowwin_supported(a)) {
        SNNB_REQUIRE(!a.shortcut, "launch_conv2d_umma: a folded shortcut needs the plain tensor-core kernel, not the row-window kernel");
        return launch_conv2d_rowwin(ctx, a, encode);
    }
    SNNB_REQUIRE(!a.in->feed_only && !(a.shortcut && a.shortcut->feed_only), "launch_conv2d_umma: the input tensor only exists as a stem feed, which this launch cannot read");
    SNNB_REQUIRE(!(a.shortcut && a.residual), "launch_conv2d_umma: a folded shortcut and a residual operand are exclusive");
    SNNB_REQUIRE(!a.shortcut || ((a.sc_stride == 1 || a.sc_stride == 2) && a.shortcut->n == a.out->n), "launch_conv2d_umma: unsupported shortcut (stride %d)",
                 a.sc_stride);
    const snnb_tensor* in = a.in;
    snnb_tensor* out      = a.out;
    UmmaParams p;
    p.out_hi = out->hi, p.out_lo = out->lo;
    p.res_hi = a.residual ? a.residual->hi : nullptr, p.res_lo = a.residual ? a.residual->lo : nullptr;
    p.has_res = a.residual != nullptr;
    p.bias    = a.w->bias;
    p.N = out->n, p.OH = out->h, p.OW = out->w, p.OC = out->c, p.OCp = out->cp;
    const TilePlan tp = plan_tiles(out->n, out->h, out->w, a.stride);
    SNNB_REQUIRE(tp.tw > 0, "launch_conv2d_umma: no tile plan");
    p.tw = tp.tw, p.th = tp.th, p.tn = tp.tn, p.rows_used = tp.tw * tp.th * tp.tn;
    p.tiles_x = tp.tiles_x, p.tiles_y = tp.tiles_y, p.tiles_n = tp.tiles_n;
    p.ksize = a.k, p.stride = a.stride, p.pad_x = a.pad_x, p.pad_y = a.pad_y;
    p.cblocks = (in->c + UM_BLOCK_K - 1) / UM_BLOCK_K;
    p.sc_cblocks = a.shortcut ? (a.shortcut->c + UM_BLOCK_K - 1) / UM_BLOCK_K : 0, p.sc_stride = a.shortcut ? a.sc_stride : 1;
    const int num_kb = a.k * a.k * p.cblocks + p.sc_cblocks;
    const int terms = conv_terms(ctx, a);
    p.has_lo        = out->lo != nullptr;
    p.b_stages = 0, p.b_stage_bytes = 0;
    OcPlan op       = plan_oc_ksplit(out->c, tp.tiles_x * tp.tiles_y * tp.tiles_n, p.rows_used, tp.tw, num_kb, ctx->sm_count, terms, false, a.stream_k);
    OcPlan hp;
    const bool halo = !a.shortcut && halo_plan(ctx, a, p.cblocks, terms, op.cost, hp);
    if (halo) {
        op              = hp;
        p.b_stage_bytes = (terms == 3 ? 2 : 1) * op.n_blk * 128 <= UM_B_BYTES ? UM_B_BYTES : 2 * UM_B_BYTES;
        p.b_stages      = HL_B_RING_BYTES / p.b_stage_bytes;
        p.tw = HL_TW, p.th = HL_TH, p.tn = 1, p.rows_used = UM_BLOCK_M;
        p.tiles_x = (out->w + HL_TW - 1) / HL_TW, p.tiles_y = (out->h + HL_TH - 1) / HL_TH, p.tiles_n = out->n;
    }
    SNNB_REQUIRE(op.n_blk > 0, "launch_conv2d_umma: no output-channel plan");
    p.n_blk = op.n_blk, p.tiles_oc = op.tiles_oc, p.ksplit = op.ksplit, p.kb_per_split = op.kb_per_split;
    p.sk = halo ? 0 : op.sk, p.sk_dp = op.sk_dp, p.sk_ctas = op.sk_ctas, p.sk_units = op.sk_units;
    p.partials = nullptr, p.counters = nullptr;
    if (!ctx->sched_counter) {
        cudaStreamCaptureStatus cap = cudaStreamCaptureStatusNone;
        SNNB_CUDA_OK(cudaStreamIsCapturing(ctx->stream, &cap));
        SNNB_REQUIRE(cap == cudaStreamCaptureStatusNone, "launch_conv2d_umma: the scheduler counter must be allocated by an eager pass before graph capture");
        void* pnew = nullptr;
        SNNB_CUDA_OK(cudaMalloc(&pnew, 256));
        SNNB_CUDA_OK(cudaMemset(pnew, 0, 256));
        ctx->scratch_blocks.push_back(pnew);
        ctx->sched_counter = static_cast<int*>(pnew);
    }
    p.sched_counter = ctx->sched_counter;
    if (p.ksplit > 1 || p.sk) {
        const size_t tiles = p.sk ? (size_t) p.tiles_x * p.tiles_y * p.tiles_n * p.tiles_oc - p.sk_dp : (size_t) p.tiles_x * p.tiles_y * p.tiles_n * p.tiles_oc;
        cudaStreamCaptureStatus cap = cudaStreamCaptureStatusNone;
        SNNB_CUDA_OK(cudaStreamIsCapturing(ctx->stream, &cap));
        const size_t need = tiles * (p.sk ? 4 : p.ksplit) * UM_BLOCK_M * p.n_blk * sizeof(float);
        SNNB_REQUIRE(cap == cudaStreamCaptureStatusNone || (need <= ctx->splitk_bytes && tiles <= ctx->splitk_counter_n),
                     "launch_conv2d_umma: split-K scratch must be allocated by an eager pass before graph capture");
        if (ensure_splitk_scratch(ctx, need, tiles)) return 1;
        p.partials = ctx->splitk_partials, p.counters = ctx->splitk_counters;
    }
    p.ICp     = round_up(in->c, 8);
    p.act = a.act, p.alpha = a.alpha;
    static const int ablate = getenv("SNNB_UMMA_ABLATE") ? atoi(getenv("SNNB_UMMA_ABLATE")) : 0;
    p.ablate                = ablate;
    const int kp_want = a.k * a.k * p.ICp + (a.shortcut ? round_up(a.shortcut->c, 8) : 0);
    SNNB_REQUIRE(a.w->kp == kp_want, "launch_conv2d_umma: packed weights do not match (kp %d vs %d)", a.w->kp, kp_want);

    auto encode_a = [&](const snnb_tensor* t, int s, int bw, int bh, CUtensorMap (&maps)[2]) {
        const cuuint64_t dims[4]    = {(cuuint64_t) t->c, (cuuint64_t) t->w, (cuuint64_t) t->h, (cuuint64_t) t->n};
        const cuuint64_t strides[3] = {(cuuint64_t) t->cp * 2, (cuuint64_t) t->w * t->cp * 2, (cuuint64_t) t->h * t->w * t->cp * 2};
        const cuuint32_t box[4]     = {(cuuint32_t) UM_BLOCK_K, (cuuint32_t) bw, (cuuint32_t) bh, (cuuint32_t) p.tn};
        const cuuint32_t estr[4]    = {1, (cuuint32_t) s, (cuuint32_t) s, 1};
        __half* planes[2]    = {t->hi, t->lo ? t->lo : t->hi};
        for (int i = 0; i < 2; ++i) {
            CUresult r = encode(&maps[i], CU_TENSOR_MAP_DATA_TYPE_FLOAT16, 4, planes[i], dims, strides, box, estr, CU_TENSOR_MAP_INTERLEAVE_NONE,
                                CU_TENSOR_MAP_SWIZZLE_128B, CU_TENSOR_MAP_L2_PROMOTION_L2_128B, CU_TENSOR_MAP_FLOAT_OOB_FILL_NONE);
            SNNB_REQUIRE(r == CUDA_SUCCESS, "cuTensorMapEncodeTiled(A) failed: %d (dims %d %d %d %d box %u %u %u %u)", (int) r, t->c, t->w, t->h, t->n, box[0],
                         box[1], box[2], box[3]);
        }
        return 0;
    };
    CUtensorMap tmA[2], tmB[2], tmS[2];
    if (encode_a(in, a.stride, halo ? HL_W : p.tw * a.stride, halo ? HL_H : p.th * a.stride, tmA)) return 2;
    if (!a.shortcut) {
        tmS[0] = tmA[0], tmS[1] = tmA[1];
// ... 230 lines not shown
            }
        }
    }
    (void) warp;
}

bool depthwise_tma_supported(const ConvArgs& a) {
    if (!a.in->lo || !a.out->lo) return false;
    const int tw = a.stride == 1 ? 16 : 8, th = a.stride == 1 ? 8 : 4;
    const int tx = (a.out->w + tw - 1) / tw, ty = (a.out->h + th - 1) / th;
    if ((double) a.out->w * a.out->h < 0.5 * (double) tx * tw * ty * th) return false;
    return a.k == 3 && (a.stride == 1 || a.stride == 2) && a.residual == nullptr && a.in->c == a.out->c && a.w->w_f32 != nullptr &&
           a.pad_mode <= SNNB_PAD_CONSTANT;
}

template <int S> static int launch_depthwise_tma_s(snnb_context* ctx, const ConvArgs& a, EncodeTiledFn encode) {
    ctx->last_kernel = "depthwise_tma_kernel";
    using T = DwTile<S>;
    const snnb_tensor* in = a.in;
    snnb_tensor* out      = a.out;
    DwTmaParams p;
    p.out_hi = out->hi, p.out_lo = out->lo;
    p.w = a.w->w_f32, p.bias = a.w->bias;
    p.N = out->n, p.OH = out->h, p.OW = out->w, p.C = out->c, p.Cp = out->cp;
    p.pad_x = a.pad_x, p.pad_y = a.pad_y;
    p.tiles_x = (out->w + T::TW - 1) / T::TW, p.tiles_y = (out->h + T::TH - 1) / T::TH, p.chunks = (out->cp + 63) / 64;
    p.act = a.act, p.alpha = a.alpha;
    CUtensorMap tmI[2];
    {
        const cuuint64_t dims[4]    = {(cuuint64_t) in->c, (cuuint64_t) in->w, (cuuint64_t) in->h, (cuuint64_t) in->n};
        const cuuint64_t strides[3] = {(cuuint64_t) in->cp * 2, (cuuint64_t) in->w * in->cp * 2, (cuuint64_t) in->h * in->w * in->cp * 2};
        const cuuint32_t box[4]     = {64, (cuuint32_t) T::IW, (cuuint32_t) T::IH, 1};
        const cuuint32_t estr[4]    = {1, 1, 1, 1};
        __half* planes[2]    = {in->hi, in->lo};
        for (int i = 0; i < 2; ++i) {
            CUresult r = encode(&tmI[i], CU_TENSOR_MAP_DATA_TYPE_FLOAT16, 4, planes[i], dims, strides, box, estr, CU_TENSOR_MAP_INTERLEAVE_NONE, CU_TENSOR_MAP_SWIZZLE_NONE,
                                CU_TENSOR_MAP_L2_PROMOTION_L2_128B, CU_TENSOR_MAP_FLOAT_OOB_FILL_NONE);
            SNNB_REQUIRE(r == CUDA_SUCCESS, "cuTensorMapEncodeTiled(depthwise input) failed: %d", (int) r);
        }
    }
    const uint32_t attr_bit = S == 1 ? ATTR_DW1 : ATTR_DW2;
    if (!(ctx->func_attr_mask & attr_bit)) {
        SNNB_CUDA_OK(cudaFuncSetAttribute(depthwise_tma_kernel<S>, cudaFuncAttributeMaxDynamicSharedMemorySize, T::SMEM_BYTES));
        ctx->func_attr_mask |= attr_bit;
    }
    const long long total = (long long) p.N * p.tiles_y * p.tiles_x * p.chunks;
    const int grid        = (int) std::min<long long>(total, 2 * ctx->sm_count);
    const cudaError_t le  = launch_k_pdl(depthwise_tma_kernel<S>, dim3(grid), dim3(DW_THREADS), T::SMEM_BYTES, ctx->stream, tmI[0], tmI[1], p);
    cudaError_t e = le != cudaSuccess ? le : cudaGetLastError();
    if (e != cudaSuccess) {
        set_error("depthwise_tma_kernel launch failed: %s", cudaGetErrorString(e));
        return 1;
    }
    ctx->launches++;
    return 0;
}

int launch_depthwise_tma(snnb_context* ctx, const ConvArgs& a) {
    EncodeTiledFn encode = get_encode(ctx);
    SNNB_REQUIRE(encode, "launch_depthwise_tma: cuTensorMapEncodeTiled is unavailable in this driver");
    return a.stride == 1 ? launch_depthwise_tma_s<1>(ctx, a, encode) : launch_depthwise_tma_s<2>(ctx, a, encode);
}

int streamk_schedule(int tiles, int num_kb, int sms, int* rows, int capacity) {
    UmmaParams p {};
    int dp = 0, ctas = 0;
    long long units = 0;
    if (tiles <= 0 || num_kb <= 0 || sms <= 0 || tiles % sms == 0 || !streamk_split(tiles, num_kb, sms, dp, units, ctas)) return -1;
    p.sk = 1, p.sk_dp = dp, p.sk_ctas = ctas, p.sk_units = units, p.ksplit = 1, p.kb_per_split = num_kb;
    const int grid = dp > 0 ? sms : ctas, end = dp + 4 * ctas;
    int n = 0;
    for (int cta = 0; cta < grid; ++cta)
        for (int work = sk_first_work(p, cta, end); work < end; work = sk_next_work(p, work, cta, grid, num_kb, end)) {
            const WorkItem w = decode_work<true>(p, work, tiles, num_kb);
            if (n < capacity) {
                int* r = rows + 6 * (size_t) n;
                r[0] = cta, r[1] = w.tile, r[2] = w.kb0, r[3] = w.kb1, r[4] = w.piece, r[5] = w.pieces;
            }
            ++n;
        }
    return n;
}

int kblock_schedule(int ksize, int cblocks, int icp, int sc_cblocks, int tiles, int ksplit, int sms, int* rows, int capacity) {
    if (ksize < 1 || cblocks < 1 || icp < 8 || sc_cblocks < 0 || tiles < 1 || ksplit < 0 || sms < 1) return -1;
    UmmaParams p {};
    p.ksize = ksize, p.cblocks = cblocks, p.ICp = icp, p.sc_cblocks = sc_cblocks, p.sc_stride = 1;
    const int num_kb = ksize * ksize * cblocks + sc_cblocks;
    std::vector<WorkItem> items;
    if (ksplit > 0) {
        p.ksplit = ksplit, p.kb_per_split = (num_kb + ksplit - 1) / ksplit;
        for (int work = 0; work < tiles * ksplit; ++work) items.push_back(decode_work<false>(p, work, tiles, num_kb));
    } else {
        int dp = 0, ctas = 0;
        long long units = 0;
        if (tiles % sms == 0 || !streamk_split(tiles, num_kb, sms, dp, units, ctas)) return -1;
        p.sk = 1, p.sk_dp = dp, p.sk_ctas = ctas, p.sk_units = units, p.ksplit = 1, p.kb_per_split = num_kb;
        const int grid = dp > 0 ? sms : ctas, end = dp + 4 * ctas;
        for (int cta = 0; cta < grid; ++cta)
            for (int work = sk_first_work(p, cta, end); work < end; work = sk_next_work(p, work, cta, grid, num_kb, end)) items.push_back(decode_work<true>(p, work, tiles, num_kb));
    }
    struct Row {
        int *rows, capacity, ksize, tile, n;
        __host__ __device__ void operator()(int kb, bool sc, int cb, int kx, int ky, int wcol) {
            if (n < capacity) {
                int* r = rows + 6 * (size_t) n;
                r[0] = tile, r[1] = kb, r[2] = sc, r[3] = ky * ksize + kx, r[4] = cb, r[5] = wcol;
            }
            ++n;
        }
    } row {rows, capacity, ksize, 0, 0};
    for (const WorkItem& w : items) {
        row.tile = w.tile;
        for_each_kblock(p, w.kb0, w.kb1, row);
    }
    return row.n;
}

}
```

### shadernn_b200/csrc/snnb_internal.h

```cpp
#pragma once

#include <cuda_runtime.h>
#include <cuda_fp16.h>
#include <cstdint>
#include <cstdio>
#include <string>
#include <utility>
#include <vector>

#include "snnb.h"

namespace snnb {

void set_error(const char* fmt, ...);
const char* get_error();

#define SNNB_CUDA_OK(expr)                                                                              \
    do {                                                                                                \
        cudaError_t _e = (expr);                                                                        \
        if (_e != cudaSuccess) {                                                                        \
            ::snnb::set_error("%s:%d: %s -> %s", __FILE__, __LINE__, #expr, cudaGetErrorString(_e));    \
            return 1;                                                                                   \
        }                                                                                               \
    } while (0)
// ... 41 lines not shown

struct snnb_tensor {
    snnb_context* ctx = nullptr;
    __half* hi = nullptr;
    __half* lo = nullptr;
    int n = 0, h = 0, w = 0, c = 0, cp = 0;
    size_t plane_elems = 0;
    bool owns = true;
    __half* feed_hi = nullptr;
    __half* feed_lo = nullptr;
    int feed_h = 0, feed_w = 0, feed_py = 0, feed_px = 0;
    bool feed_only = false;
    size_t pixels() const { return (size_t) n * h * w; }
};

struct snnb_weights {
    snnb_context* ctx = nullptr;
    int kind = 0;
    int in_ch = 0, out_ch = 0, kernel = 1;
    float* w_f32 = nullptr;
    int ocw = 0;
    __half* w_hi = nullptr;
    __half* w_lo = nullptr;
    int kp = 0, ocr = 0;
    __half* w_row_hi = nullptr;
    __half* w_row_lo = nullptr;
    int row_stride = 0, row_pad = 0;
    __half* w_feed_hi = nullptr;
    __half* w_feed_lo = nullptr;
    int feed_pad = -1;
    float* bias = nullptr;
    float *gamma = nullptr, *beta = nullptr, *mean = nullptr, *var = nullptr;
    void* owned = nullptr;
    size_t bytes = 0;
};

struct snnb_context {
    int device          = 0;
    cudaStream_t stream = nullptr;
    int sm_count        = 148;
    uint64_t launches   = 0;
    float* stage_dev    = nullptr;
    size_t stage_dev_bytes = 0;
    float* stage_host   = nullptr;
    size_t stage_host_bytes = 0;
    void* tmap_encode_fn = nullptr;
    float* splitk_partials = nullptr;
    size_t splitk_bytes    = 0;
    int* splitk_counters   = nullptr;
    size_t splitk_counter_n = 0;
    int* sched_counter      = nullptr;
    uint32_t func_attr_mask = 0;
    const char* last_kernel = nullptr;
    int precision = SNNB_PRECISION_FP32X3;
    std::vector<void*> scratch_blocks;
};

struct snnb_graph {
    snnb_context* ctx     = nullptr;
    cudaGraph_t graph     = nullptr;
    cudaGraphExec_t exec  = nullptr;
};

struct snnb_timer {
    snnb_context* ctx = nullptr;
    cudaEvent_t e0 = nullptr, e1 = nullptr;
};

namespace snnb {

int ensure_stage(snnb_context* ctx, size_t bytes);

struct ConvArgs {
    const snnb_tensor* in;
    const snnb_tensor* residual;
    snnb_tensor* out;
    const snnb_weights* w;
    int k, stride, pad_x, pad_y, pad_mode, act;
    float alpha;
    int precision = -1;
    bool stream_k = false;
    const snnb_tensor* shortcut = nullptr;
    int sc_stride = 1;
};
int launch_conv2d_simt(snnb_context* ctx, const ConvArgs& a);
int launch_conv2d_umma(snnb_context* ctx, const ConvArgs& a);
bool conv2d_umma_supported(const ConvArgs& a);
bool conv2d_umma_fold_supported(const snnb_context* ctx, const ConvArgs& a);
int kblock_schedule(int ksize, int cblocks, int icp, int sc_cblocks, int tiles, int ksplit, int sms, int* rows, int capacity);
int streamk_schedule(int tiles, int num_kb, int sms, int* rows, int capacity);
int launch_depthwise(snnb_context* ctx, const ConvArgs& a);
bool depthwise_tma_supported(const ConvArgs& a);
int launch_depthwise_tma(snnb_context* ctx, const ConvArgs& a);
int launch_pool(snnb_context* ctx, const snnb_tensor* in, snnb_tensor* out, int k, int stride, bool avg);
bool gap_dense_supported(const snnb_tensor* in, const snnb_tensor* out, const snnb_weights* w);
int launch_gap_dense(snnb_context* ctx, const snnb_tensor* in, snnb_tensor* out, const snnb_weights* w, int act, float alpha, bool softmax);
int launch_add(snnb_context* ctx, const snnb_tensor* a, const snnb_tensor* b, snnb_tensor* out, int act, float alpha);
int launch_batchnorm(snnb_context* ctx, const snnb_tensor* in, snnb_tensor* out, const snnb_weights* w, int act, float alpha);
int launch_activation(snnb_context* ctx, const snnb_tensor* in, snnb_tensor* out, int act, float alpha);
int launch_softmax(snnb_context* ctx, const snnb_tensor* in, snnb_tensor* out);
int launch_argmax(snnb_context* ctx, const snnb_tensor* in, int* dev_idx);
int launch_yolo_candidates(snnb_context* ctx, const snnb_tensor* h0, const snnb_tensor* h1, float thresh, int maxc, int* counts, float* cand);
int launch_flatten(snnb_context* ctx, const snnb_tensor* in, snnb_tensor* out);
int launch_concat(snnb_context* ctx, const snnb_tensor* a, const snnb_tensor* b, snnb_tensor* out);
int launch_upsample(snnb_context* ctx, const snnb_tensor* in, snnb_tensor* out, float scale, bool bilinear);
int launch_pad(snnb_context* ctx, const snnb_tensor* in, snnb_tensor* out, int pad_x, int pad_y, int mode);
constexpr int INSTNORM_MAX_CHUNKS = 64;
static inline size_t instnorm_scratch_floats(int n, int cp) { return (size_t) n * cp * 2 + (size_t) n * (cp >> 3) * INSTNORM_MAX_CHUNKS * 16; }
int launch_instancenorm(snnb_context* ctx, const snnb_tensor* in, snnb_tensor* out, const snnb_weights* w, int act, float alpha, float* scratch = nullptr);
int launch_subpixel(snnb_context* ctx, const snnb_tensor* in, snnb_tensor* out, int r);
int launch_split_f32(snnb_context* ctx, const float* dev_nhwc, snnb_tensor* t);
int launch_split_u8(snnb_context* ctx, const uint8_t* dev_nhwc_u8, snnb_tensor* t, const float mean[4], const float norm[4]);
int launch_merge_f32(snnb_context* ctx, const snnb_tensor* t, float* dev_nhwc);
int launch_result_small(snnb_context* ctx, const snnb_tensor* t, float* values, int* idx);
int launch_resize_u8(snnb_context* ctx, const uint8_t* dev_nhwc_u8, int src_h, int src_w, snnb_tensor* t, const float mean[4], const float norm[4], bool linear);
int launch_merge_u8(snnb_context* ctx, const snnb_tensor* t, uint8_t* dev_nhwc_u8, float scale, float offset);

struct RowPlan {
    int parities = 0;
    int dmin[2]  = {0, 0};
    int ntaps[2] = {0, 0};
    int ksteps   = 0;
    int ks_parity[8], ks_erel[8], ks_tap[8][2];
    int span = 0;
};
static inline bool make_row_plan(int k, int stride, int pad_x, RowPlan& rp) {
    if (k < 1 || k > 9 || !(stride == 1 || stride == 2)) return false;
    rp = RowPlan();
    rp.parities = stride;
    for (int par = 0; par < stride; ++par) {
        int js[9], t = 0;
        for (int j = 0; j < k; ++j)
            if ((((j - pad_x) % stride) + stride) % stride == par) js[t++] = j;
        rp.ntaps[par] = t;
        if (!t) continue;
        const int a  = js[0] - pad_x;
        rp.dmin[par] = a >= 0 ? a / stride : -((-a + stride - 1) / stride);
        for (int q = 0; q < (t + 1) / 2; ++q) {
            if (rp.ksteps >= 8) return false;
            rp.ks_parity[rp.ksteps] = par;
            rp.ks_erel[rp.ksteps]   = 2 * q;
            rp.ks_tap[rp.ksteps][0] = js[2 * q];
            rp.ks_tap[rp.ksteps][1] = (2 * q + 1 < t) ? js[2 * q + 1] : -1;
            rp.ksteps++;
        }
        rp.span = rp.span > 2 * ((t + 1) / 2) ? rp.span : 2 * ((t + 1) / 2);
    }
    return rp.ksteps > 0;
}

struct FeedPlan {
    int px = 0, d = 0, nch = 0, ksteps = 0;
    int rows_per_panel = 1;
};
static inline bool make_feed_plan(int k, int stride, int pad_x, int ic, FeedPlan& fp) {
    if (stride != 2 || ic > 4 || k < 2 || k > 9 || pad_x < 0 || pad_x > 8) return false;
    fp.px     = (pad_x + 1) & ~1;
    fp.d      = fp.px - pad_x;
    fp.nch    = ((fp.d + k + 1) / 2 + 1) & ~1;
    fp.ksteps = fp.nch / 2;
    fp.rows_per_panel = fp.ksteps == 1 ? 4 : (fp.ksteps == 2 ? 2 : 1);
    return fp.ksteps <= 4;
}

struct PackedHost {
    std::vector<float> w_f32;
    std::vector<__half> w_hi, w_lo;
    std::vector<__half> w_row_hi, w_row_lo;
    int row_stride = 0, row_pad = 0;
    std::vector<__half> w_feed_hi, w_feed_lo;
    int feed_pad = -1;
// ... 20 lines not shown
```

Before: 61390.

## Fuse stem max-pool into the row-window conv kernel epilogue

Adds a fused path where the stem Conv2D (fed from the input feed) computes its output rows and max-pools them in shared memory before storing only the pooled tensor. The goal is to drop the full-resolution conv output write, the separate pooling kernel launch, and its re-read. It adds a pooled variant of the row-window kernel, a per-CTA row schedule that follows pool window overlap, and debug and dump helpers that recompute the unpooled output on demand. The pool region takes shared memory that was used for staging, which can reduce pipeline stages, and row ordering across CTAs becomes constrained.

```diff
diff --git a/include/snnb.h b/include/snnb.h
--- a/include/snnb.h
+++ b/include/snnb.h
@@ -155,6 +155,7 @@
 int snnb_debug_streamk_schedule(int tiles, int num_kb, int sms, int* rows, int capacity);
 int snnb_debug_feed_plan(int k, int stride, int pad_x, int ic, int out[5]);
 int snnb_debug_kblock_schedule(int ksize, int cblocks, int icp, int sc_cblocks, int tiles, int ksplit, int sms, int* rows, int capacity);
+int snnb_debug_stem_pool_schedule(int N, int OH, int PH, int k, int grid, int* rows, int capacity);
 
 #ifdef __cplusplus
 }
diff --git a/shadernn_b200/_lib.py b/shadernn_b200/_lib.py
--- a/shadernn_b200/_lib.py
+++ b/shadernn_b200/_lib.py
@@ -136,6 +136,7 @@
     "snnb_debug_streamk_schedule": (C.c_int, [C.c_int, C.c_int, C.c_int, c_int_p, C.c_int]),
     "snnb_debug_feed_plan": (C.c_int, [C.c_int, C.c_int, C.c_int, C.c_int, c_int_p]),
     "snnb_debug_kblock_schedule": (C.c_int, [C.c_int] * 7 + [c_int_p, C.c_int]),
+    "snnb_debug_stem_pool_schedule": (C.c_int, [C.c_int] * 5 + [c_int_p, C.c_int]),
 }
 
 _lib = None
diff --git a/shadernn_b200/csrc/capi.cpp b/shadernn_b200/csrc/capi.cpp
--- a/shadernn_b200/csrc/capi.cpp
+++ b/shadernn_b200/csrc/capi.cpp
@@ -147,6 +147,10 @@
 int snnb_debug_kblock_schedule(int ksize, int cblocks, int icp, int sc_cblocks, int tiles, int ksplit, int sms, int* rows, int capacity) {
     SNNB_REQUIRE(rows || capacity == 0, "snnb_debug_kblock_schedule: null buffer");
     return kblock_schedule(ksize, cblocks, icp, sc_cblocks, tiles, ksplit, sms, rows, capacity);
+}
+int snnb_debug_stem_pool_schedule(int N, int OH, int PH, int k, int grid, int* rows, int capacity) {
+    SNNB_REQUIRE(rows || capacity == 0, "snnb_debug_stem_pool_schedule: null buffer");
+    return stem_pool_schedule(N, OH, PH, k, grid, rows, capacity);
 }
 int snnb_tensor_planes(const snnb_tensor* t, void** hi, void** lo, int* cp) {
     SNNB_REQUIRE(t && hi && lo && cp, "snnb_tensor_planes: null argument");
diff --git a/shadernn_b200/csrc/engine/core.cpp b/shadernn_b200/csrc/engine/core.cpp
--- a/shadernn_b200/csrc/engine/core.cpp
+++ b/shadernn_b200/csrc/engine/core.cpp
@@ -54,6 +54,14 @@
     }
     if (!core->init(err)) return nullptr;
     return core;
+}
+
+static void feedExtent(const snnb_tensor* in, int outH, int outW, int k, int padY, const FeedPlan& fp, int& feedH, int& feedW) {
+    const int tilesX = (outW + 127) / 128;
+    const int needW  = 2 * (tilesX * 128 - 1) + 2 * fp.nch;
+    const int needH  = 2 * (outH - 1) + k - padY + padY;
+    feedW            = (std::max(in->w + fp.px, needW) + 1) & ~1;
+    feedH            = std::max(in->h + padY, needH);
 }
 
 static bool allZeroPadding(const PaddingSpec& p) {
@@ -119,6 +127,42 @@
         a.shortcut = &sc, a.sc_stride = (int) dc->_desc.stride;
         return conv2d_umma_fold_supported(ctx, a);
     };
+    const bool stemPoolFuse = options.fuse && options.convAlgo != SNNB_ALGO_SIMT && getenv("SNNB_NO_STEM_POOL") == nullptr && getenv("SNNB_NO_FEED") == nullptr;
+    std::unordered_map<GenericModelLayer*, GenericModelLayer*> stemPoolOf;
+    auto stemPoolable = [&](GenericModelLayer* c, GenericModelLayer* pool) {
+        if (c->typeName != "Conv2D" || c->fusedAway || c->nextLayers.size() != 1 || c->prevLayers.size() != 1) return false;
+        auto* cc = static_cast<Conv2DLayer*>(c);
+        auto* pl = static_cast<PoolingLayer*>(pool);
+        if (cc->fusedAct >= 0 || cc->shortcut || cc->foldedInto || pl->_desc.stride != 2 || !(pl->_desc.kernelSize == 2 || pl->_desc.kernelSize == 3)) return false;
+        GenericModelLayer* src = c->prevLayers[0];
+        while (alias.count(src)) src = alias[src];
+        const int mode = padModeId(cc->_desc.padding.mode);
+        if (!src->isInputLayer || !(mode == SNNB_PAD_NONE || mode == SNNB_PAD_CONSTANT)) return false;
+        uint32_t offs[4];
+        cc->_desc.padding.offsets((int) cc->_desc.kernelSize, true, offs);
+        const int k = (int) cc->_desc.kernelSize, padX = (int) offs[0], padY = (int) offs[2];
+        auto stand_in = [&](GenericModelLayer* X) {
+            snnb_tensor t;
+            const Dims& d = graph.outputDims[order[X]];
+            t.n = N, t.h = (int) d.height, t.w = (int) d.width, t.c = (int) d.depth, t.cp = round_up(t.c, 8);
+            t.hi = reinterpret_cast<__half*>(1), t.lo = twoPlanes ? t.hi : nullptr;
+            return t;
+        };
+        snnb_tensor in = stand_in(src), out = stand_in(c), po = stand_in(pool);
+        FeedPlan fp;
+        if (!make_feed_plan(k, (int) cc->_desc.stride, padX, in.c, fp)) return false;
+        in.feed_hi = in.feed_lo = in.hi, in.feed_px = fp.px, in.feed_py = padY;
+        feedExtent(&in, out.h, out.w, k, padY, fp, in.feed_h, in.feed_w);
+        snnb_weights probe;
+        probe.w_hi = probe.w_lo = probe.w_row_hi = probe.w_row_lo = probe.w_feed_hi = probe.w_feed_lo = reinterpret_cast<__half*>(1);
+        probe.row_stride = (int) cc->_desc.stride, probe.row_pad = padX, probe.feed_pad = padX;
+        ConvArgs a;
+        a.in = &in, a.residual = nullptr, a.out = &out, a.w = &probe;
+        a.k = k, a.stride = (int) cc->_desc.stride, a.pad_x = padX, a.pad_y = padY, a.pad_mode = mode;
+        a.act = cc->_desc.activation.id, a.alpha = cc->_desc.activation.alpha, a.precision = options.precision;
+        a.pool_out = &po, a.pool_k = (int) pl->_desc.kernelSize;
+        return conv2d_rowwin_pool_supported(ctx, a);
+    };
     if (options.fuse) {
         for (auto* L : graph.sorted) {
             if (L->typeName == "Pad" && L->nextLayers.size() == 1 && L->prevLayers.size() == 1) {
@@ -193,6 +237,12 @@
                     pool->fusedAway = true;
                 }
             }
+            if (stemPoolFuse && L->typeName == "MaxPooling2D" && !static_cast<PoolingLayer*>(L)->isAvg && L->prevLayers.size() == 1 &&
+                stemPoolable(L->prevLayers[0], L)) {
+                static_cast<Conv2DLayer*>(L->prevLayers[0])->poolK = (int) static_cast<PoolingLayer*>(L)->_desc.kernelSize;
+                stemPoolOf[L->prevLayers[0]] = L;
+                L->fusedAway = true;
+            }
             if (L->typeName == "Flatten" && L->inputDims.size() == 1 && L->inputDims[0].width * L->inputDims[0].height == 1 &&
                 static_cast<FlattenLayer*>(L)->activation.id == SNNB_ACT_NONE) {
                 L->fusedAway = true;
@@ -216,6 +266,7 @@
         GenericModelLayer* owner = resolve(L);
         if (owner != L && !(L->typeName == "Conv2D")) continue;
         if (L->typeName == "Conv2D" && static_cast<Conv2DLayer*>(L)->foldedInto) continue;
+        if (stemPoolOf.count(L)) continue;
         if (outOf.count(owner)) continue;
         const Dims& d = graph.outputDims[order[owner]];
         snnb_tensor* t = nullptr;
@@ -233,6 +284,16 @@
         }
         GenericModelLayer* owner = resolve(L);
         L->output                = outOf.count(owner) ? outOf[owner] : nullptr;
+        if (stemPoolOf.count(L)) {
+            auto* cl              = static_cast<Conv2DLayer*>(L);
+            const Dims& d         = graph.outputDims[order[L]];
+            cl->stemShape         = snnb_tensor();
+            cl->stemShape.ctx     = ctx, cl->stemShape.owns = false;
+            cl->stemShape.n = N, cl->stemShape.h = (int) d.height, cl->stemShape.w = (int) d.width, cl->stemShape.c = (int) d.depth;
+            cl->stemShape.cp      = round_up(cl->stemShape.c, 8);
+            cl->pooled            = outOf.at(stemPoolOf[L]);
+            L->output             = &cl->stemShape;
+        }
         if (L->fusedAway) continue;
         size_t nin = L->prevLayers.size();
         if (L->typeName == "Conv2D" && static_cast<Conv2DLayer*>(L)->fusedAct >= 0 && !static_cast<Conv2DLayer*>(L)->shortcut) {
@@ -270,16 +331,17 @@
                 FeedPlan fp;
                 if (!noFeed && !prepad && src->isInputLayer && !in->feed_hi && options.convAlgo != SNNB_ALGO_SIMT && !L->residual && !cl->shortcut && L->output->c <= 64 &&
                     (mode == SNNB_PAD_NONE || mode == SNNB_PAD_CONSTANT) && make_feed_plan(k, (int) cl->_desc.stride, padX, in->c, fp)) {
-                    const int tilesX = (L->output->w + 127) / 128;
-                    const int needW  = 2 * (tilesX * 128 - 1) + 2 * fp.nch;
-                    const int needH  = 2 * (L->output->h - 1) + k - padY + padY;
-                    const int feedW  = (std::max(in->w + fp.px, needW) + 1) & ~1;
-                    const int feedH  = std::max(in->h + padY, needH);
+                    int feedH, feedW;
+                    feedExtent(in, L->output->h, L->output->w, k, padY, fp, feedH, feedW);
                     if (tensor_alloc_feed(in, feedH, feedW, padY, fp.px)) {
                         err = get_error();
                         return false;
                     }
                     cl->feedInput = true;
+                }
+                if (cl->pooled && !cl->feedInput) {
+                    err = L->name + ": the fused max pool needs the input's stem feed; load the model with fuse=0";
+                    return false;
                 }
             }
         }
@@ -685,7 +747,21 @@
                  L->name.c_str());
     const size_t floats = L->output->pixels() * L->output->c;
     SNNB_REQUIRE(capacityFloats >= floats, "layerOutput: buffer too small (%zu < %zu floats)", capacityFloats, floats);
-    return snnb_tensor_download_nhwc(ctx, L->output, host);
+    return withLayerTensor(L, [&](const snnb_tensor* t) { return snnb_tensor_download_nhwc(ctx, t, host); });
+}
+
+int MixedInferenceCore::withLayerTensor(GenericModelLayer* L, const std::function<int(const snnb_tensor*)>& f) {
+    if (!(L->typeName == "Conv2D" && static_cast<Conv2DLayer*>(L)->pooled)) return f(L->output);
+    snnb_tensor* t = nullptr;
+    if (tensor_alloc(ctx, L->output->n, L->output->h, L->output->w, L->output->c, &t, options.precision != SNNB_PRECISION_FP16)) return 1;
+    ExecOptions eo;
+    eo.convAlgo = options.convAlgo, eo.precision = options.precision;
+    int rc = static_cast<Conv2DLayer*>(L)->runInto(ctx, eo, t);
+    if (!rc) rc = f(t);
+    const cudaError_t e = cudaStreamSynchronize(ctx->stream);
+    snnb_tensor_free(t);
+    SNNB_CUDA_OK(e);
+    return rc;
 }
 
 int MixedInferenceCore::timeLayers(std::vector<float>& ms) {
@@ -717,10 +793,10 @@
 
 int MixedInferenceCore::dumpOutputs(const std::string& dir) {
     for (auto& l : layers) {
-        if (!l->output || l->fusedAway) continue;
+        if (!l->output || (l->fusedAway && !(l->typeName == "MaxPooling2D" && l->output->hi))) continue;
         SNNB_REQUIRE(!(l->typeName == "Conv2D" && l->fusedAct >= 0), "dumpOutputs: %s was fused into its Add; load the model with fuse=0 to dump every layer", l->name.c_str());
         std::string path = dir + "/" + l->name + " pass[0].dump";
-        if (snnb_tensor_dump(ctx, l->output, path.c_str())) return 1;
+        if (withLayerTensor(l.get(), [&](const snnb_tensor* t) { return snnb_tensor_dump(ctx, t, path.c_str()); })) return 1;
     }
     return 0;
 }
diff --git a/shadernn_b200/csrc/engine/engine.h b/shadernn_b200/csrc/engine/engine.h
--- a/shadernn_b200/csrc/engine/engine.h
+++ b/shadernn_b200/csrc/engine/engine.h
@@ -1,6 +1,7 @@
 #pragma once
 
 #include <algorithm>
+#include <functional>
 #include <map>
 #include <memory>
 #include <string>
@@ -139,7 +140,11 @@
     Conv2DLayer* shortcut    = nullptr;
     Conv2DLayer* foldedInto  = nullptr;
     snnb_tensor* shortcutIn  = nullptr;
+    snnb_tensor* pooled = nullptr;
+    int poolK           = 0;
+    snnb_tensor stemShape;
     bool wantsPrepad(const snnb_tensor* in, const snnb_tensor* out, int convAlgo, int& ph, int& pw) const;
+    int runInto(snnb_context* ctx, const ExecOptions& opt, snnb_tensor* out);
     Transform getOutputScaleDimAdjustment() const override;
     void getOutputDims(uint32_t& w, uint32_t& h, uint32_t& d) const override;
     void packWeights(snnb::PackedHost& p) override;
@@ -294,6 +299,7 @@
     int submitImage(const snnb_image_io& io, int* ticket);
     int wait(int ticket);
     int layerOutput(int layerId, float* host, size_t capacityFloats);
+    int withLayerTensor(dp::GenericModelLayer* L, const std::function<int(const snnb_tensor*)>& f);
     int timeLayers(std::vector<float>& ms);
     int dumpOutputs(const std::string& dir);
 
diff --git a/shadernn_b200/csrc/engine/layers.cpp b/shadernn_b200/csrc/engine/layers.cpp
--- a/shadernn_b200/csrc/engine/layers.cpp
+++ b/shadernn_b200/csrc/engine/layers.cpp
@@ -96,7 +96,8 @@
     return true;
 }
 
-int Conv2DLayer::run(snnb_context* ctx, const ExecOptions& opt) {
+int Conv2DLayer::run(snnb_context* ctx, const ExecOptions& opt) { return runInto(ctx, opt, pooled ? nullptr : output); }
+int Conv2DLayer::runInto(snnb_context* ctx, const ExecOptions& opt, snnb_tensor* out) {
     uint32_t offs[4];
     _desc.padding.offsets((int) _desc.kernelSize, true, offs);
     if (prepadded) {
@@ -107,8 +108,9 @@
         return launch_conv2d_umma(ctx, a);
     }
     ConvArgs a;
-    a.in = inputs[0], a.residual = residual, a.out = output, a.w = &weights;
+    a.in = inputs[0], a.residual = residual, a.out = out ? out : output, a.w = &weights;
     a.k = (int) _desc.kernelSize, a.stride = (int) _desc.stride;
+    if (!out) a.pool_out = pooled, a.pool_k = poolK;
     a.pad_x = _desc.kernelSize == 1 ? 0 : (int) offs[0];
     a.pad_y = _desc.kernelSize == 1 ? 0 : (int) offs[2];
     a.pad_mode = padModeId(_desc.padding.mode);
@@ -118,8 +120,8 @@
     a.shortcut = shortcutIn, a.sc_stride = shortcut ? (int) shortcut->_desc.stride : 1;
     const int want = algo != SNNB_ALGO_AUTO ? algo : opt.convAlgo;
     if (want != SNNB_ALGO_SIMT && conv2d_umma_supported(a)) return launch_conv2d_umma(ctx, a);
-    if (shortcut) {
-        set_error("%s: a folded projection shortcut runs on the tensor-core kernel only; load the model with fuse=0 for another algorithm", name.c_str());
+    if (shortcut || a.pool_out) {
+        set_error("%s: a folded projection shortcut or max pool runs on the tensor-core kernel only; load the model with fuse=0 for another algorithm", name.c_str());
         return 2;
     }
     if (want == SNNB_ALGO_TCGEN05) {
diff --git a/shadernn_b200/csrc/kernels_umma.cu b/shadernn_b200/csrc/kernels_umma.cu
--- a/shadernn_b200/csrc/kernels_umma.cu
+++ b/shadernn_b200/csrc/kernels_umma.cu
@@ -203,6 +203,23 @@
     l               = um_f2h(a - hf.x, b - hf.y);
 }
 
+__device__ __forceinline__ void epi_act16(float (&v)[16], int act, float alpha, int c0, int OC) {
+    if (act == SNNB_ACT_RELU) {
+#pragma unroll
+        for (int j = 0; j < 16; ++j) v[j] = fmaxf(v[j], 0.0f);
+    } else if (act == SNNB_ACT_NONE) {
+    } else if (act == SNNB_ACT_RELU6) {
+#pragma unroll
+        for (int j = 0; j < 16; ++j) v[j] = fminf(fmaxf(v[j], 0.0f), 6.0f);
+    } else if (act == SNNB_ACT_LEAKY_RELU) {
+#pragma unroll
+        for (int j = 0; j < 16; ++j) v[j] = fminf(fmaxf(v[j], v[j] * alpha), __int_as_float(0x7f800000));
+    } else {
+#pragma unroll
+        for (int j = 0; j < 16; ++j) v[j] = (c0 + j < OC) ? umma_act(v[j], act, alpha) : 0.0f;
+    }
+}
+
 struct EpiArgs {
     const CUtensorMap *o_hi64, *o_lo64, *o_hiT, *o_loT;
     const CUtensorMap *r_hi64, *r_lo64, *r_hiT, *r_loT;
@@ -240,9 +257,6 @@
 __device__ __forceinline__ void epilogue_tile(const EpiArgs& e, uint32_t taddr, int oc0, int c1, int c2, int c3, int row, int half, bool leader, int lane,
                                               uint32_t& res_phase) {
     constexpr int MAXC  = NWARPS == 8 ? 2 : 4;
-    const bool fast_act = e.act == SNNB_ACT_NONE || e.act == SNNB_ACT_RELU || e.act == SNNB_ACT_RELU6 || e.act == SNNB_ACT_LEAKY_RELU;
-    const float slope   = (e.act == SNNB_ACT_RELU || e.act == SNNB_ACT_RELU6) ? 0.0f : (e.act == SNNB_ACT_LEAKY_RELU ? e.alpha : 1.0f);
-    const float hi_clip = e.act == SNNB_ACT_RELU6 ? 6.0f : __int_as_float(0x7f800000);
     const int nslabs    = (e.n_blk + 63) >> 6;
 #define EPI_STAMP(k)                                                                                      \
     do {                                                                                                  \
@@ -336,20 +350,7 @@
                             }
                         }
                     }
-                    if (e.act == SNNB_ACT_RELU) {
-#pragma unroll
-                        for (int j = 0; j < 16; ++j) v[j] = fmaxf(v[j], 0.0f);
-                    } else if (e.act == SNNB_ACT_NONE) {
-                    } else if (e.act == SNNB_ACT_RELU6) {
-#pragma unroll
-                        for (int j = 0; j < 16; ++j) v[j] = fminf(fmaxf(v[j], 0.0f), 6.0f);
-                    } else if (fast_act) {
-#pragma unroll
-                        for (int j = 0; j < 16; ++j) v[j] = fminf(fmaxf(v[j], v[j] * slope), hi_clip);
-                    } else {
-#pragma unroll
-                        for (int j = 0; j < 16; ++j) v[j] = (oc0 + c + j < e.OC) ? umma_act(v[j], e.act, e.alpha) : 0.0f;
-                    }
+                    epi_act16(v, e.act, e.alpha, oc0 + c, e.OC);
 #pragma unroll
                     for (int j = 0; j < 8; ++j) um_split2(v[2 * j], v[2 * j + 1], oh[kk][j], ol[kk][j]);
                 }
@@ -981,20 +982,197 @@
     uint32_t row_bytes;
     int stg_bufs;
     int feed_prows;
+    int PH, PW;
+    uint32_t pool_plane, pool_bytes;
 };
 
+template <class F> __host__ __device__ __forceinline__ void for_each_stem_row(int N, int OH, int PH, int k, int grid, int cta, F&& f) {
+    const long long P = (long long) N * PH, p1 = P * (cta + 1) / grid;
+    for (long long p = P * cta / grid; p < p1;) {
+        const int n = (int) (p / PH), a = (int) (p - (long long) n * PH);
+        const int b = (int) (a + (p1 - p) - 1 < PH - 1 ? a + (p1 - p) - 1 : PH - 1);
+        const int r1 = 2 * b + k - 1 < OH - 1 ? 2 * b + k - 1 : OH - 1;
+        for (int r = 2 * a; r <= r1; ++r) f(n, r, a, b);
+        p += b - a + 1;
+    }
+}
+__host__ __device__ __forceinline__ void stem_pool_rows(int r, int a, int b, int k, int& y0, int& y1) {
+    y0 = (r - k + 2) >> 1;
+    y0 = y0 > a ? y0 : a;
+    y1 = (r >> 1) < b ? (r >> 1) : b;
+}
+__host__ __device__ __forceinline__ bool stem_pool_last(int r, int y, int k, int OH) { return r == (2 * y + k - 1 < OH - 1 ? 2 * y + k - 1 : OH - 1); }
+
+struct PoolEpiArgs {
+    const CUtensorMap *o_hi, *o_lo;
+    const float* bias;
+    int n_blk, OC, act, has_lo, OW, OH, PH, PW;
+    float alpha;
+    uint32_t stg, plane, acc, xch;
+    uint32_t tmem_empty;
+};
+template <int POOL, int TERMS>
+__device__ __forceinline__ void epilogue_pool_row(const PoolEpiArgs& e, uint32_t taddr, int n, int r, int a, int b, int it, int& emitted, int q, int half, int lane,
+                                                  bool leader) {
+    const int nch = e.n_blk >> 4;
+    float v[2][16];
+    {
+        uint32_t rr[2][16], r2[2][16];
+#pragma unroll
+        for (int kk = 0; kk < 2; ++kk) {
+            const int ci = half + 2 * kk;
+            if (ci < nch) {
+                tmem_ld16(taddr + (uint32_t) (ci * 16), rr[kk]);
+                if (TERMS == 3) {
+                    tmem_ld16(taddr + (uint32_t) (e.n_blk + ci * 16), r2[kk]);
+                } else {
+#pragma unroll
+                    for (int j = 0; j < 16; ++j) r2[kk][j] = 0u;
+                }
+            }
+        }
+        tmem_ld_wait();
+        tc_fence_before();
+        __syncwarp();
+        if (lane == 0) mbar_arrive(e.tmem_empty);
+        const bool inside = 32 * q + lane < e.OW;
+#pragma unroll
+        for (int kk = 0; kk < 2; ++kk) {
+            const int c = (half + 2 * kk) * 16;
+            if (c >= e.n_blk) continue;
+#pragma unroll
+            for (int j4 = 0; j4 < 4; ++j4) {
+                const float4 bb = __ldg(reinterpret_cast<const float4*>(e.bias + c) + j4);
+                v[kk][4 * j4 + 0] = (__uint_as_float(rr[kk][4 * j4 + 0]) + __uint_as_float(r2[kk][4 * j4 + 0])) + bb.x;
+                v[kk][4 * j4 + 1] = (__uint_as_float(rr[kk][4 * j4 + 1]) + __uint_as_float(r2[kk][4 * j4 + 1])) + bb.y;
+                v[kk][4 * j4 + 2] = (__uint_as_float(rr[kk][4 * j4 + 2]) + __uint_as_float(r2[kk][4 * j4 + 2])) + bb.z;
+                v[kk][4 * j4 + 3] = (__uint_as_float(rr[kk][4 * j4 + 3]) + __uint_as_float(r2[kk][4 * j4 + 3])) + bb.w;
+            }
+            epi_act16(v[kk], e.act, e.alpha, c, e.OC);
+#pragma unroll
+            for (int j = 0; j < 16; ++j) v[kk][j] = inside ? v[kk][j] : -__int_as_float(0x7f800000);
+        }
+    }
+    const uint32_t xslot = e.xch + (uint32_t) ((((it & 1) * 2 + half) * 4 + q) * 128);
+    if (POOL == 3 && lane == 0) {
+#pragma unroll
+        for (int kk = 0; kk < 2; ++kk)
+            if ((half + 2 * kk) * 16 < e.n_blk) {
+#pragma unroll
+                for (int g = 0; g < 4; ++g)
+                    asm volatile("st.shared.v4.f32 [%0], {%1, %2, %3, %4};" ::"r"(xslot + (uint32_t) (kk * 64 + g * 16)), "f"(v[kk][4 * g]), "f"(v[kk][4 * g + 1]),
+                                 "f"(v[kk][4 * g + 2]), "f"(v[kk][4 * g + 3])
+                                 : "memory");
+            }
+    }
+    if (leader) {
+        if (elect_one()) bulk_wait_read1();
+        __syncwarp();
+    }
+    named_bar_sync(1, RW_EPI_WARPS * 32);
+#pragma unroll
+    for (int kk = 0; kk < 2; ++kk) {
+        if ((half + 2 * kk) * 16 >= e.n_blk) continue;
+        float nx[16];
+#pragma unroll
+        for (int j = 0; j < 16; ++j) nx[j] = -__int_as_float(0x7f800000);
+        if (POOL == 3 && lane == 30 && q < 3) {
+            const uint32_t src = xslot + 128u + (uint32_t) (kk * 64);
+#pragma unroll
+            for (int g = 0; g < 4; ++g)
+                asm volatile("ld.shared.v4.f32 {%0, %1, %2, %3}, [%4];" : "=f"(nx[4 * g]), "=f"(nx[4 * g + 1]), "=f"(nx[4 * g + 2]), "=f"(nx[4 * g + 3]) : "r"(src + 16u * g) : "memory");
+        }
+#pragma unroll
+        for (int j = 0; j < 16; ++j) {
+            const float t1 = __shfl_down_sync(0xffffffffu, v[kk][j], 1);
+            if (POOL == 3) {
+                const float t2 = __shfl_down_sync(0xffffffffu, v[kk][j], 2);
+                v[kk][j]       = fmaxf(fmaxf(v[kk][j], t1), lane == 30 ? nx[j] : t2);
+            } else {
+                v[kk][j] = fmaxf(v[kk][j], t1);
+            }
+        }
+    }
+    const int px      = 16 * q + (lane >> 1);
+    const bool owner  = !(lane & 1) && px < e.PW;
+    const uint32_t sw = (uint32_t) (px & 7);
+    const bool swz       = e.n_blk == 64;
+    const uint32_t pitch = swz ? 128u : (uint32_t) e.n_blk * 2u;
+    int y0, y1;
+    stem_pool_rows(r, a, b, POOL, y0, y1);
+    for (int y = y0; y <= y1; ++y) {
+        const bool first = r == 2 * y, last = stem_pool_last(r, y, POOL, e.OH);
+        if (last && y > y0) {
+            if (leader) {
+                if (elect_one()) bulk_wait_read1();
+                __syncwarp();
+            }
+            named_bar_sync(1, RW_EPI_WARPS * 32);
+        }
+        const uint32_t arow = e.acc + (uint32_t) (((n * e.PH + y) & 1) * e.PW + px) * 256u;
+        const uint32_t sbuf = e.stg + (uint32_t) (emitted & 1) * 2u * e.plane;
+        if (owner) {
+#pragma unroll
+            for (int kk = 0; kk < 2; ++kk) {
+                const int ci = half + 2 * kk;
+                if (ci * 16 >= e.n_blk) continue;
+#pragma unroll
+                for (int g2 = 0; g2 < 2; ++g2) {
+                    float m[8];
+#pragma unroll
+                    for (int g1 = 0; g1 < 2; ++g1) {
+                        const int g           = 2 * g2 + g1;
+                        const uint32_t addr   = arow + ((((uint32_t) (ci * 4 + g)) ^ sw) << 4);
+                        float o[4]            = {-100000.0f, -100000.0f, -100000.0f, -100000.0f};
+                        if (!first) asm volatile("ld.shared.v4.f32 {%0, %1, %2, %3}, [%4];" : "=f"(o[0]), "=f"(o[1]), "=f"(o[2]), "=f"(o[3]) : "r"(addr) : "memory");
+#pragma unroll
+                        for (int j = 0; j < 4; ++j) m[4 * g1 + j] = fmaxf(o[j], v[kk][4 * g + j]);
+                        if (!last)
+                            asm volatile("st.shared.v4.f32 [%0], {%1, %2, %3, %4};" ::"r"(addr), "f"(m[4 * g1]), "f"(m[4 * g1 + 1]), "f"(m[4 * g1 + 2]), "f"(m[4 * g1 + 3]) : "memory");
+                    }
+                    if (!last) continue;
+                    uint32_t oh[4], ol[4];
+#pragma unroll
+                    for (int j = 0; j < 4; ++j) {
+                        uint32_t h1, l1;
+                        um_split2(m[2 * j], m[2 * j + 1], h1, l1);
+                        const float2 fh = um_h2f(h1), fl = e.has_lo ? um_h2f(l1) : make_float2(0.0f, 0.0f);
+                        um_split2(fh.x + fl.x, fh.y + fl.y, oh[j], ol[j]);
+                    }
+                    const uint32_t addr = sbuf + (uint32_t) px * pitch + ((((uint32_t) (ci * 2 + g2)) ^ (swz ? sw : 0u)) << 4);
+                    asm volatile("st.shared.v4.b32 [%0], {%1, %2, %3, %4};" ::"r"(addr), "r"(oh[0]), "r"(oh[1]), "r"(oh[2]), "r"(oh[3]) : "memory");
+                    if (e.has_lo) asm volatile("st.shared.v4.b32 [%0], {%1, %2, %3, %4};" ::"r"(addr + e.plane), "r"(ol[0]), "r"(ol[1]), "r"(ol[2]), "r"(ol[3]) : "memory");
+                }
+            }
+        }
+        if (!last) continue;
+        fence_async_smem();
+        named_bar_sync(1, RW_EPI_WARPS * 32);
+        if (leader) {
+            if (elect_one()) {
+                tma_store_4d(e.o_hi, sbuf, 0, 0, y, n);
+                if (e.has_lo) tma_store_4d(e.o_lo, sbuf + e.plane, 0, 0, y, n);
+                bulk_commit();
+            }
+            __syncwarp();
+        }
+        ++emitted;
+    }
+}
+
 __device__ __forceinline__ uint64_t make_window_desc(uint32_t saddr) { return (uint64_t) ((saddr >> 4) & 0x3FFFu) | (1ull << 16) | (8ull << 32) | (1ull << 46); }
 
-template <int TERMS, int FKS>
+template <int TERMS, int FKS, int POOL = 0>
 __global__ void __launch_bounds__(RW_THREADS, 1)
 conv_rowwin_kernel(const __grid_constant__ CUtensorMap tmA_hi0, const __grid_constant__ CUtensorMap tmA_hi1, const __grid_constant__ CUtensorMap tmA_lo0,
                    const __grid_constant__ CUtensorMap tmA_lo1, const __grid_constant__ CUtensorMap tmB_hi, const __grid_constant__ CUtensorMap tmB_lo,
                    const __grid_constant__ CUtensorMap tmO_hi, const __grid_constant__ CUtensorMap tmO_lo, const RowWinParams p) {
+    static_assert(POOL == 0 || FKS > 0, "the fused pool needs feed mode");
     extern __shared__ uint8_t smem_raw[];
     const uint32_t smem_base = (smem_u32(smem_raw) + 1023u) & ~1023u;
     const uint32_t sB = smem_base;
     const uint32_t stg      = smem_base + p.b_bytes;
-    const uint32_t sA0      = stg + (uint32_t) p.stg_bufs * UM_STG_BYTES;
+    const uint32_t sA0      = stg + (POOL ? p.pool_bytes : (uint32_t) p.stg_bufs * UM_STG_BYTES);
     const uint32_t bar_base = sA0 + (uint32_t) p.stages * p.stage_bytes;
     const int RW_STAGES     = p.stages;
     auto full_bar       = [&](int s) { return bar_base + 8u * s; };
@@ -1060,11 +1238,8 @@
             if constexpr (FKS > 0) {
                 const uint32_t seg  = p.feed_seg_bytes;
                 const size_t pitch  = (size_t) p.feed_w * 4;
-                const int per_image = p.OH * p.tiles_x;
-                int rem = (int) blockIdx.x % per_image, n = (int) blockIdx.x / per_image;
                 uint32_t sA = sA0;
-                for (int tile = blockIdx.x; tile < total_tiles; tile += gridDim.x) {
-                    const int oy = p.tiles_x == 1 ? rem : rem / p.tiles_x, xt = p.tiles_x == 1 ? 0 : rem % p.tiles_x;
+                auto load_tile = [&](int n, int oy, int xt) {
                     const size_t off = (((size_t) n * p.feed_h + (oy * 2 - p.pad_y + p.feed_py)) * p.feed_w + 2 * xt * UM_BLOCK_M) * 4;
                     const __half* src_hi = p.feed_hi + off;
                     const __half* src_lo = p.feed_lo + off;
@@ -1090,8 +1265,17 @@
                         sA += p.stage_bytes;
                         if (++stage == RW_STAGES) stage = 0, phase ^= 1u, sA = sA0;
                     }
-                    rem += (int) gridDim.x;
-                    while (rem >= per_image) rem -= per_image, ++n;
+                };
+                if constexpr (POOL > 0) {
+                    for_each_stem_row(p.N, p.OH, p.PH, POOL, (int) gridDim.x, (int) blockIdx.x, [&](int n, int r, int, int) { load_tile(n, r, 0); });
+                } else {
+                    const int per_image = p.OH * p.tiles_x;
+                    int rem = (int) blockIdx.x % per_image, n = (int) blockIdx.x / per_image;
+                    for (int tile = blockIdx.x; tile < total_tiles; tile += gridDim.x) {
+                        load_tile(n, p.tiles_x == 1 ? rem : rem / p.tiles_x, p.tiles_x == 1 ? 0 : rem % p.tiles_x);
+                        rem += (int) gridDim.x;
+                        while (rem >= per_image) rem -= per_image, ++n;
+                    }
                 }
             } else
             for (int tile = blockIdx.x; tile < total_tiles; tile += gridDim.x) {
@@ -1143,7 +1327,7 @@
                 const uint32_t stage16  = p.stage_bytes >> 4, row16 = p.row_bytes >> 4;
                 const bool tracing      = p.trace != nullptr && blockIdx.x == 0;
                 uint64_t a_cur = wdesc0;
-                for (int tile = blockIdx.x; tile < total_tiles; tile += gridDim.x, ++it) {
+                auto issue_tile = [&]() {
                     const int acc = it & 1;
                     mbar_wait(tmem_empty_bar(acc), ((uint32_t) (it >> 1) & 1u) ^ 1u);
                     tc_fence_after();
@@ -1183,6 +1367,11 @@
                         if (tracing && tr < 256) p.trace[2 * 256 + tr] = clock64();
                         ++tr;
                     }
+                };
+                if constexpr (POOL > 0) {
+                    for_each_stem_row(p.N, p.OH, p.PH, POOL, (int) gridDim.x, (int) blockIdx.x, [&](int, int, int, int) { issue_tile(), ++it; });
+                } else {
+                    for (int tile = blockIdx.x; tile < total_tiles; tile += gridDim.x, ++it) issue_tile();
                 }
             } else
             for (int tile = blockIdx.x; tile < total_tiles; tile += gridDim.x, ++it) {
@@ -1226,38 +1415,57 @@
         const int q    = warp & 3;
         const int half = (warp - 2) >> 2;
         const int row  = q * 32 + lane;
-        EpiArgs e;
-        e.o_hi64 = &tmO_hi, e.o_lo64 = &tmO_lo, e.o_hiT = &tmO_hi, e.o_loT = &tmO_lo;
-        e.r_hi64 = e.r_lo64 = e.r_hiT = e.r_loT = &tmO_hi;
-        e.bias = p.bias, e.n_blk = p.n_blk, e.OC = p.OC, e.act = p.act, e.has_res = 0, e.rows_box = UM_BLOCK_M, e.alpha = p.alpha;
-        e.has_lo = TERMS >= 2;
-        e.stg = stg, e.res_bar = 0, e.bar_id = 1;
-        e.part_src = nullptr, e.part_splits = 0;
-        e.no_store = (p.ablate & 8) != 0;
-        e.two_stagings = p.stg_bufs == 2;
-        uint32_t res_phase = 0;
-        int it = 0;
-        for (int tile = blockIdx.x; tile < total_tiles; tile += gridDim.x, ++it) {
-            const int acc = it & 1;
-            const uint32_t acc_phase = (uint32_t) (it >> 1) & 1u;
-            const int xt = tile % p.tiles_x, oy = (tile / p.tiles_x) % p.OH, n = tile / (p.tiles_x * p.OH);
-            mbar_wait(tmem_full_bar(acc), acc_phase);
-            tc_fence_after();
-            if (warp == 2) UM_TRACE(3, it);
-            e.tmem_empty = tmem_empty_bar(acc);
-            e.trace = p.trace, e.trace_seq = it;
-            const uint32_t taddr = tmem_base + ((uint32_t) (q * 32) << 16) + (uint32_t) (acc * 2 * RW_MAX_N);
-            if (p.ablate & 1) {
-                tc_fence_before();
-                __syncwarp();
-                if (lane == 0) mbar_arrive(e.tmem_empty);
-                continue;
-            }
-            e.stg = stg + (uint32_t) ((it & 1) & (p.stg_bufs - 1)) * UM_STG_BYTES;
-            epilogue_tile<RW_EPI_WARPS, TERMS>(e, taddr, 0, xt * UM_BLOCK_M, oy, n, row, half, warp == 2, lane, res_phase);
-            if (warp == 2) UM_TRACE(4, it);
-        }
-        epilogue_drain(warp == 2);
+        if constexpr (POOL > 0) {
+            PoolEpiArgs e;
+            e.o_hi = &tmO_hi, e.o_lo = &tmO_lo, e.bias = p.bias;
+            e.n_blk = p.n_blk, e.OC = p.OC, e.act = p.act, e.has_lo = TERMS >= 2, e.OW = p.OW, e.OH = p.OH, e.PH = p.PH, e.PW = p.PW;
+            e.alpha = p.alpha;
+            e.stg = stg, e.plane = p.pool_plane, e.acc = stg + 4u * p.pool_plane, e.xch = e.acc + 2u * (uint32_t) p.PW * 256u;
+            int it = 0, emitted = 0;
+            for_each_stem_row(p.N, p.OH, p.PH, POOL, (int) gridDim.x, (int) blockIdx.x, [&](int n, int r, int a, int b) {
+                const int acc = it & 1;
+                mbar_wait(tmem_full_bar(acc), (uint32_t) (it >> 1) & 1u);
+                tc_fence_after();
+                e.tmem_empty = tmem_empty_bar(acc);
+                const uint32_t taddr = tmem_base + ((uint32_t) (q * 32) << 16) + (uint32_t) (acc * 2 * RW_MAX_N);
+                epilogue_pool_row<POOL, TERMS>(e, taddr, n, r, a, b, it, emitted, q, half, lane, warp == 2);
+                ++it;
+            });
+            epilogue_drain(warp == 2);
+        } else {
+            EpiArgs e;
+            e.o_hi64 = &tmO_hi, e.o_lo64 = &tmO_lo, e.o_hiT = &tmO_hi, e.o_loT = &tmO_lo;
+            e.r_hi64 = e.r_lo64 = e.r_hiT = e.r_loT = &tmO_hi;
+            e.bias = p.bias, e.n_blk = p.n_blk, e.OC = p.OC, e.act = p.act, e.has_res = 0, e.rows_box = UM_BLOCK_M, e.alpha = p.alpha;
+            e.has_lo = TERMS >= 2;
+            e.stg = stg, e.res_bar = 0, e.bar_id = 1;
+            e.part_src = nullptr, e.part_splits = 0;
+            e.no_store = (p.ablate & 8) != 0;
+            e.two_stagings = p.stg_bufs == 2;
+            uint32_t res_phase = 0;
+            int it = 0;
+            for (int tile = blockIdx.x; tile < total_tiles; tile += gridDim.x, ++it) {
+                const int acc = it & 1;
+                const uint32_t acc_phase = (uint32_t) (it >> 1) & 1u;
+                const int xt = tile % p.tiles_x, oy = (tile / p.tiles_x) % p.OH, n = tile / (p.tiles_x * p.OH);
+                mbar_wait(tmem_full_bar(acc), acc_phase);
+                tc_fence_after();
+                if (warp == 2) UM_TRACE(3, it);
+                e.tmem_empty = tmem_empty_bar(acc);
+                e.trace = p.trace, e.trace_seq = it;
+                const uint32_t taddr = tmem_base + ((uint32_t) (q * 32) << 16) + (uint32_t) (acc * 2 * RW_MAX_N);
+                if (p.ablate & 1) {
+                    tc_fence_before();
+                    __syncwarp();
+                    if (lane == 0) mbar_arrive(e.tmem_empty);
+                    continue;
+                }
+                e.stg = stg + (uint32_t) ((it & 1) & (p.stg_bufs - 1)) * UM_STG_BYTES;
+                epilogue_tile<RW_EPI_WARPS, TERMS>(e, taddr, 0, xt * UM_BLOCK_M, oy, n, row, half, warp == 2, lane, res_phase);
+                if (warp == 2) UM_TRACE(4, it);
+            }
+            epilogue_drain(warp == 2);
+        }
     }
 
     tc_fence_before();
@@ -1442,7 +1650,7 @@
 }
 
 static int conv_terms(const snnb_context* ctx, const ConvArgs& a) {
-    if (!a.in->lo || !a.out->lo) return 1;
+    if (!a.in->lo || !(a.pool_out ? a.pool_out : a.out)->lo) return 1;
     const int prec = a.precision >= 0 ? a.precision : ctx->precision;
     return prec == SNNB_PRECISION_FP16W ? 2 : (prec == SNNB_PRECISION_FP16 ? 1 : 3);
 }
@@ -1475,6 +1683,23 @@
     const int hx = (a.out->w + HL_TW - 1) / HL_TW, hy = (a.out->h + HL_TH - 1) / HL_TH;
     hp = plan_oc_ksplit(a.out->c, hx * hy * a.out->n, UM_BLOCK_M, HL_TW, 9 * cblocks, ctx->sm_count, terms, true);
     return hp.n_blk > 0 && hp.cost < plain_cost;
+}
+
+static uint32_t pool_plane_bytes(int PW) { return (uint32_t) round_up(PW * 128, 1024); }
+static uint32_t pool_region_bytes(int PW) { return 4u * pool_plane_bytes(PW) + 2u * (uint32_t) PW * 256u + 2048u; }
+static bool rowwin_pool_shape_ok(const ConvArgs& a) {
+    const snnb_tensor *o = a.out, *po = a.pool_out;
+    return (a.pool_k == 2 || a.pool_k == 3) && po && po->n == o->n && po->c == o->c && po->h >= 1 && po->w >= 1 && 2 * (po->h - 1) < o->h &&
+           2 * (po->w - 1) < o->w && o->w <= UM_BLOCK_M && o->c <= RW_MAX_N && !po->feed_only;
+}
+
+bool conv2d_rowwin_pool_supported(const snnb_context* ctx, const ConvArgs& a) {
+    FeedPlan fp;
+    if (!a.pool_out || a.residual || a.shortcut || !conv2d_umma_supported(a) || !rowwin_supported(a) || !feed_usable(a, fp) || !rowwin_pool_shape_ok(a)) return false;
+    const int terms = conv_terms(ctx, a), rps = (a.k + (a.k + 3) / 4 - 1) / ((a.k + 3) / 4);
+    const int b_bytes = round_up((terms == 3 ? 2 : 1) * ((a.k + fp.rows_per_panel - 1) / fp.rows_per_panel) * round_up(a.out->c, 16) * 128, 1024);
+    const int stage   = rps * (terms == 1 ? 1 : 2) * RW_ARR_BYTES;
+    return RW_SMEM_BYTES - 1024 - RW_BAR_BYTES - b_bytes - (int) pool_region_bytes(a.pool_out->w) >= 2 * stage;
 }
 
 bool conv2d_umma_fold_supported(const snnb_context* ctx, const ConvArgs& a) {
@@ -1493,16 +1718,21 @@
 
 typedef void (*RowWinKernel)(const CUtensorMap, const CUtensorMap, const CUtensorMap, const CUtensorMap, const CUtensorMap, const CUtensorMap, const CUtensorMap,
                              const CUtensorMap, const RowWinParams);
-template <int TERMS> static RowWinKernel rowwin_kernel_fks(int fks) {
+template <int TERMS, int POOL> static RowWinKernel rowwin_kernel_fks(int fks) {
     switch (fks) {
-    case 1: return conv_rowwin_kernel<TERMS, 1>;
-    case 2: return conv_rowwin_kernel<TERMS, 2>;
-    case 3: return conv_rowwin_kernel<TERMS, 3>;
-    case 4: return conv_rowwin_kernel<TERMS, 4>;
-    default: return conv_rowwin_kernel<TERMS, 0>;
-    }
-}
-static RowWinKernel rowwin_kernel_of(int terms, int fks) { return terms == 3 ? rowwin_kernel_fks<3>(fks) : (terms == 2 ? rowwin_kernel_fks<2>(fks) : rowwin_kernel_fks<1>(fks)); }
+    case 1: return conv_rowwin_kernel<TERMS, 1, POOL>;
+    case 2: return conv_rowwin_kernel<TERMS, 2, POOL>;
+    case 3: return conv_rowwin_kernel<TERMS, 3, POOL>;
+    case 4: return conv_rowwin_kernel<TERMS, 4, POOL>;
+    default: return POOL ? nullptr : conv_rowwin_kernel<TERMS, 0>;
+    }
+}
+template <int POOL> static RowWinKernel rowwin_kernel_pool(int terms, int fks) {
+    return terms == 3 ? rowwin_kernel_fks<3, POOL>(fks) : (terms == 2 ? rowwin_kernel_fks<2, POOL>(fks) : rowwin_kernel_fks<1, POOL>(fks));
+}
+static RowWinKernel rowwin_kernel_of(int terms, int fks, int pool) {
+    return pool == 3 ? rowwin_kernel_pool<3>(terms, fks) : (pool == 2 ? rowwin_kernel_pool<2>(terms, fks) : rowwin_kernel_pool<0>(terms, fks));
+}
 
 static bool feed_usable(const ConvArgs& a, FeedPlan& fp) {
     const snnb_tensor* in = a.in;
@@ -1521,11 +1751,13 @@
     FeedPlan fp;
     const bool feed = feed_usable(a, fp);
     SNNB_REQUIRE(feed || !in->feed_only, "launch_conv2d_rowwin: the input tensor only exists as a stem feed, which this launch cannot read");
+    const bool pool = a.pool_out != nullptr;
+    SNNB_REQUIRE(!pool || (feed && rowwin_pool_shape_ok(a)), "launch_conv2d_rowwin: the fused max pool needs a stem feed, OW <= 128, OC <= 64 and a 2x2 or 3x3 window");
     if (feed) {
         rp.parities = 1, rp.ksteps = fp.ksteps;
         for (int q = 0; q < fp.ksteps; ++q) rp.ks_parity[q] = 0, rp.ks_erel[q] = 2 * q;
     }
-    ctx->last_kernel = feed ? "conv_rowwin_kernel<feed>" : "conv_rowwin_kernel";
+    ctx->last_kernel = pool ? "conv_rowwin_kernel<feed+maxpool>" : (feed ? "conv_rowwin_kernel<feed>" : "conv_rowwin_kernel");
     RowWinParams p;
     p.out_hi = out->hi, p.out_lo = out->lo, p.bias = a.w->bias;
     p.N = out->n, p.OH = out->h, p.OW = out->w, p.OC = out->c, p.OCp = out->cp;
@@ -1551,7 +1783,10 @@
     static const int one_stg = getenv("SNNB_ROWWIN_ONE_STAGING") != nullptr;
     const int ring_room      = RW_SMEM_BYTES - 1024 - RW_BAR_BYTES - (int) p.b_bytes;
     p.stg_bufs    = (!one_stg && (ring_room - 2 * UM_STG_BYTES) / (int) p.stage_bytes >= 2) ? 2 : 1;
-    p.stages      = std::min(RW_MAX_STAGES, (ring_room - p.stg_bufs * UM_STG_BYTES) / (int) p.stage_bytes);
+    p.PH = pool ? a.pool_out->h : 0, p.PW = pool ? a.pool_out->w : 0;
+    p.pool_plane  = pool ? pool_plane_bytes(p.PW) : 0u;
+    p.pool_bytes  = pool ? pool_region_bytes(p.PW) : 0u;
+    p.stages      = std::min(RW_MAX_STAGES, (ring_room - (pool ? (int) p.pool_bytes : p.stg_bufs * UM_STG_BYTES)) / (int) p.stage_bytes);
     SNNB_REQUIRE(p.stages >= 2, "launch_conv2d_rowwin: weight panels of %u bytes leave no room for the activation ring", p.b_bytes);
 
     CUtensorMap tmA[4], tmB[2];
@@ -1581,22 +1816,24 @@
         }
     }
     CUtensorMap tmO[2];
-    if (encode_nhwc_box_maps(encode, out, p.n_blk, UM_BLOCK_M, 1, 1, p.n_blk == 64, tmO)) return 2;
+    if (encode_nhwc_box_maps(encode, pool ? a.pool_out : out, p.n_blk, pool ? p.PW : UM_BLOCK_M, 1, 1, p.n_blk == 64, tmO)) return 2;
     if (!(ctx->func_attr_mask & ATTR_ROWWIN)) {
         for (int t = 1; t <= 3; ++t)
-            for (int f = 0; f <= 4; ++f) SNNB_CUDA_OK(cudaFuncSetAttribute(rowwin_kernel_of(t, f), cudaFuncAttributeMaxDynamicSharedMemorySize, RW_SMEM_BYTES));
+            for (int f = 0; f <= 4; ++f)
+                for (int k : {0, 2, 3})
+                    if (RowWinKernel kf = rowwin_kernel_of(t, f, k)) SNNB_CUDA_OK(cudaFuncSetAttribute(kf, cudaFuncAttributeMaxDynamicSharedMemorySize, RW_SMEM_BYTES));
         ctx->func_attr_mask |= ATTR_ROWWIN;
     }
     const int total_tiles = p.N * p.OH * p.tiles_x;
     const int grid        = std::min(total_tiles, ctx->sm_count);
     p.trace = nullptr;
     if (trace_enabled() && trace_begin(ctx, &p.trace)) return 1;
-    auto* kern = rowwin_kernel_of(terms, feed ? fp.ksteps : 0);
+    auto* kern = rowwin_kernel_of(terms, feed ? fp.ksteps : 0, pool ? a.pool_k : 0);
     const cudaError_t le = launch_k_pdl(kern, dim3(grid), dim3(RW_THREADS), RW_SMEM_BYTES, ctx->stream, tmA[0], tmA[1], tmA[2], tmA[3], tmB[0], tmB[1], tmO[0], tmO[1], p);
     if (p.trace) {
         char hdr[256];
-        snprintf(hdr, sizeof hdr, "rowwin%s k%d s%d IC%d OC%d out %dx%dx%d n_blk %d tiles %d grid %d kh %d ksteps %d terms %d", feed ? "<feed>" : "", a.k, a.stride, a.in->c,
-                 a.out->c, a.out->n, a.out->h, a.out->w, p.n_blk, total_tiles, grid, p.kh, p.ksteps, terms);
+        snprintf(hdr, sizeof hdr, "rowwin%s k%d s%d IC%d OC%d out %dx%dx%d n_blk %d tiles %d grid %d kh %d ksteps %d terms %d", pool ? "<feed+maxpool>" : (feed ? "<feed>" : ""),
+                 a.k, a.stride, a.in->c, a.out->c, a.out->n, a.out->h, a.out->w, p.n_blk, total_tiles, grid, p.kh, p.ksteps, terms);
         if (trace_end(ctx, p.trace, hdr)) return 1;
     }
     cudaError_t e = le != cudaSuccess ? le : cudaGetLastError();
@@ -1615,6 +1852,7 @@
         SNNB_REQUIRE(!a.shortcut, "launch_conv2d_umma: a folded shortcut needs the plain tensor-core kernel, not the row-window kernel");
         return launch_conv2d_rowwin(ctx, a, encode);
     }
+    SNNB_REQUIRE(!a.pool_out, "launch_conv2d_umma: a fused max pool needs the row-window kernel in feed mode");
     SNNB_REQUIRE(!a.in->feed_only && !(a.shortcut && a.shortcut->feed_only), "launch_conv2d_umma: the input tensor only exists as a stem feed, which this launch cannot read");
     SNNB_REQUIRE(!(a.shortcut && a.residual), "launch_conv2d_umma: a folded shortcut and a residual operand are exclusive");
     SNNB_REQUIRE(!a.shortcut || ((a.sc_stride == 1 || a.sc_stride == 2) && a.shortcut->n == a.out->n), "launch_conv2d_umma: unsupported shortcut (stride %d)",
@@ -2011,6 +2249,29 @@
     return n;
 }
 
+int stem_pool_schedule(int N, int OH, int PH, int k, int grid, int* rows, int capacity) {
+    if (N < 1 || OH < 1 || PH < 1 || !(k == 2 || k == 3) || 2 * (PH - 1) >= OH || grid < 1) return -1;
+    struct Row {
+        int *rows, capacity, OH, k, cta, n;
+        __host__ __device__ void put(int kind, int img, int r) {
+            if (n < capacity) {
+                int* o = rows + 4 * (size_t) n;
+                o[0] = cta, o[1] = kind, o[2] = img, o[3] = r;
+            }
+            ++n;
+        }
+        __host__ __device__ void operator()(int img, int r, int a, int b) {
+            put(0, img, r);
+            int y0, y1;
+            stem_pool_rows(r, a, b, k, y0, y1);
+            for (int y = y0; y <= y1; ++y)
+                if (stem_pool_last(r, y, k, OH)) put(1, img, y);
+        }
+    } row {rows, capacity, OH, k, 0, 0};
+    for (row.cta = 0; row.cta < grid; ++row.cta) for_each_stem_row(N, OH, PH, k, grid, row.cta, row);
+    return row.n;
+}
+
 int kblock_schedule(int ksize, int cblocks, int icp, int sc_cblocks, int tiles, int ksplit, int sms, int* rows, int capacity) {
     if (ksize < 1 || cblocks < 1 || icp < 8 || sc_cblocks < 0 || tiles < 1 || ksplit < 0 || sms < 1) return -1;
     UmmaParams p {};
diff --git a/shadernn_b200/csrc/snnb_internal.h b/shadernn_b200/csrc/snnb_internal.h
--- a/shadernn_b200/csrc/snnb_internal.h
+++ b/shadernn_b200/csrc/snnb_internal.h
@@ -147,11 +147,15 @@
     bool stream_k = false;
     const snnb_tensor* shortcut = nullptr;
     int sc_stride = 1;
+    snnb_tensor* pool_out = nullptr;
+    int pool_k = 0;
 };
 int launch_conv2d_simt(snnb_context* ctx, const ConvArgs& a);
 int launch_conv2d_umma(snnb_context* ctx, const ConvArgs& a);
 bool conv2d_umma_supported(const ConvArgs& a);
 bool conv2d_umma_fold_supported(const snnb_context* ctx, const ConvArgs& a);
+bool conv2d_rowwin_pool_supported(const snnb_context* ctx, const ConvArgs& a);
+int stem_pool_schedule(int N, int OH, int PH, int k, int grid, int* rows, int capacity);
 int kblock_schedule(int ksize, int cblocks, int icp, int sc_cblocks, int tiles, int ksplit, int sms, int* rows, int capacity);
 int streamk_schedule(int tiles, int num_kb, int sms, int* rows, int capacity);
 int launch_depthwise(snnb_context* ctx, const ConvArgs& a);
```

Result: no change. 61890 (median of 6 runs) (+0.8%).
